# sigma0-dev/polymath

Hardware: AMD Instinct MI355X
Metric: prove_constraints_per_sec (higher is better)
Workload: dtype u32; 1 GPU; 2^20-100-constraint synthetic R1CS (random A*B=C gates), bls12_381, n=2^21, transcript=merlin; msm_pairs_per_proof=29359963, parallelism=one GPU

## Files before the change

polymath_amd/api.py:

```python
import ctypes as ct
import os

import numpy as np

HERE = os.path.dirname(os.path.abspath(__file__))
LIB_PATH = os.environ.get("POLYMATH_HIP_LIB") or os.path.join(HERE, "libpolymath_hip.so")

PM_BLS12_381, PM_BN254 = 0, 1
CURVE_IDS = {"bls12_381": PM_BLS12_381, "bn254": PM_BN254}
FQ_LIMBS64 = {PM_BLS12_381: 6, PM_BN254: 4}

STATUS = {0: "PM_OK", 1: "PM_ERR_INVALID_ARG", 2: "PM_ERR_LEN_MISMATCH", 3: "PM_ERR_DOMAIN_TOO_LARGE",
          4: "PM_ERR_REMAINDER_NONZERO", 5: "PM_ERR_DEGREE_BOUND", 6: "PM_ERR_HIP", 7: "PM_ERR_NO_DEVICE",
          8: "PM_ERR_STATE", 9: "PM_ERR_COMM"}
(X_POWERS, X_POWERS_Y_ALPHA, X_POWERS_Y_GAMMA, X_POWERS_Y_GAMMA_Z, X_POWERS_ZH_BY_Y_ALPHA,
 UJ_WJ_LCS_BY_Y_ALPHA) = range(6)
G1_OK, G1_BAD_FLAGS, G1_COORD_GE_P, G1_NOT_ON_CURVE, G1_NOT_IN_SUBGROUP, G1_NONCANONICAL_INF, G1_INF_SIGN = range(7)
G1_BYTES = {PM_BLS12_381: 48, PM_BN254: 32}
PROOF_BYTES = {PM_BLS12_381: 176, PM_BN254: 128}
VERIFY_REJECTED, VERIFY_ACCEPTED, VERIFY_MALFORMED = range(3)
VERIFY_TIMING_SLOTS = {"decode": 0, "terms": 1, "tree": 2, "host_glue": 3, "host_pairing": 4, "device_total": 7}
TIMING_SLOTS = ["witness_map", "ntt", "poly", "msm_sort", "msm_accumulate", "msm_reduce", "msm_total", "phase"]

u64p = ct.POINTER(ct.c_uint64)
# ... 242 lines not shown


def layout_indices(n, shard_count, shard_rank, coefficients=True):
    L = load_library()
    out = np.zeros(n // shard_count, dtype=np.uint64)
    st = L.pm_layout_indices(n, shard_count, shard_rank, int(coefficients), _p(out))
    if st:
        raise PolymathError(st, "pm_layout_indices")
    return out


class Comm:

    def __init__(self, handle, keep=None):
        self.L, self.h, self._keep = load_library(), handle, keep

    @classmethod
    def local_group(cls, world, serialize=False):
        L = load_library()
        arr = (ct.c_void_p * world)()
        st = L.pm_comm_local_create(world, arr)
        if st:
            raise PolymathError(st, "pm_comm_local_create")
        if serialize:
            st = L.pm_comm_local_set_serialize(ct.c_void_p(arr[0]), 1)
            if st:
                raise PolymathError(st, "pm_comm_local_set_serialize")
        return [cls(ct.c_void_p(arr[r])) for r in range(world)]

    @staticmethod
    def rccl_unique_id():
        L = load_library()
        buf = ct.create_string_buffer(128)
        st = L.pm_comm_rccl_unique_id(buf)
        if st:
            raise PolymathError(st, "pm_comm_rccl_unique_id (librccl not loadable?)")
        return buf.raw

    @classmethod
    def rccl(cls, unique_id, rank, world, device):
        L = load_library()
        h = ct.c_void_p()
        st = L.pm_comm_rccl_create(ct.c_char_p(unique_id), rank, world, device, ct.byref(h))
        if st:
            raise PolymathError(st, "pm_comm_rccl_create")
        return cls(h)

    @property
    def rank(self):
        return self.L.pm_comm_rank(self.h)

    @property
    def world(self):
        return self.L.pm_comm_world(self.h)

    def busy_ms(self, reset=True):
        return float(self.L.pm_comm_busy_ms(self.h, int(reset)))

    @property
    def kind(self):
        return self.L.pm_comm_kind(self.h).decode()

    @property
    def failed(self):
        return bool(self.L.pm_comm_failed(self.h))

    def last_error(self):
        return self.L.pm_comm_last_error(self.h).decode()

    def set_timeout_ms(self, ms):
        st = self.L.pm_comm_set_timeout_ms(self.h, int(ms))
        if st:
            raise PolymathError(st, "pm_comm_set_timeout_ms")

    def abort(self, why="aborted by the host"):
        self.L.pm_comm_abort(self.h, why.encode())

    def all_gather(self, arr):
        arr = np.ascontiguousarray(arr)
        out = np.zeros((self.world,) + arr.shape, dtype=arr.dtype)
        st = self.L.pm_comm_all_gather(self.h, arr.ctypes.data_as(ct.c_void_p), out.ctypes.data_as(ct.c_void_p), arr.nbytes)
        if st:
            raise PolymathError(st, self.L.pm_comm_last_error(self.h).decode())
        return out

    def all_to_all_device(self, d_send, d_recv, bytes_per_peer, stream=None):
        st = self.L.pm_comm_all_to_all(self.h, ct.c_void_p(d_send), ct.c_void_p(d_recv), bytes_per_peer, ct.c_void_p(stream or 0))
        if st:
            raise PolymathError(st, self.L.pm_comm_last_error(self.h).decode())

    def all_gather_device(self, d_send, d_recv, nbytes, stream=None):
        st = self.L.pm_comm_all_gather_device(self.h, ct.c_void_p(d_send), ct.c_void_p(d_recv), nbytes, ct.c_void_p(stream or 0))
        if st:
            raise PolymathError(st, self.L.pm_comm_last_error(self.h).decode())

    def close(self):
        if getattr(self, "h", None):
            self.L.pm_comm_destroy(self.h)
            self.h = None


class Context:

    def __init__(self, device=0):
        self.L = load_library()
        h = ct.c_void_p()
        st = self.L.pm_ctx_create(device, ct.byref(h))
        if st:
            raise PolymathError(st, "pm_ctx_create(device=%d)" % device)
        self.h = h
        self.device = device

    def close(self):
        if getattr(self, "h", None):
            self.L.pm_ctx_destroy(self.h)
            self.h = None

    def __del__(self):
        try:
            self.close()
        except Exception:
            pass

    def check(self, st):
        if st:
            raise PolymathError(st, self.L.pm_last_error(self.h).decode())

    def set_comm(self, comm):
        self.comm = comm
        self.check(self.L.pm_ctx_set_comm(self.h, comm.h if comm is not None else None))

    def set_option(self, name, value):
        key = OPTIONS[name] if isinstance(name, str) else int(name)
        if key == OPTIONS["tables"] and isinstance(value, str):
            value = TABLES_MODES[value]
        self.check(self.L.pm_ctx_set_option(self.h, key, int(value)))

    def get_option(self, name):
        key = OPTIONS[name] if isinstance(name, str) else int(name)
        v = ct.c_longlong(0)
        self.check(self.L.pm_ctx_get_option(self.h, key, ct.byref(v)))
        return int(v.value)

    def selftest_field(self, products_per_field=4096, seed=1):
        bad = (ct.c_uint64 * 4)()
        self.check(self.L.pm_selftest_field(self.h, products_per_field, seed, bad))
        return dict(zip(("bls12_381_fr", "bn254_fr", "bls12_381_fq", "bn254_fq"), (int(v) for v in bad)))

    def timings(self):
        arr = (ct.c_double * len(TIMING_SLOTS))()
        self.L.pm_last_timings(self.h, arr, len(TIMING_SLOTS))
        return dict(zip(TIMING_SLOTS, list(arr)))

    def ntt(self, curve, data, log_n, inverse=False):
        data = _c(data).copy()
        self.check(self.L.pm_ntt(self.h, CURVE_IDS[curve], _p(data), log_n, int(inverse)))
        return data

    def ntt_device(self, curve, dptr, log_n, inverse=False):
        self.check(self.L.pm_ntt_device(self.h, CURVE_IDS[curve], ct.c_void_p(dptr), log_n, int(inverse)))

    def msm(self, curve, bases, scalars):
        cid = CURVE_IDS[curve]
        bases, scalars = _c(bases), _c(scalars)
        out = np.zeros(2 * FQ_LIMBS64[cid], dtype=np.uint64)
        inf = ct.c_int(0)
        self.check(self.L.pm_msm_g1(self.h, cid, bases.ctypes.data_as(ct.c_void_p), max(bases.strides[0], 16 * FQ_LIMBS64[cid]) if bases.ndim > 1 else 16 * FQ_LIMBS64[cid],
                                    _p(scalars), scalars.shape[0], _p(out), ct.byref(inf)))
        return out, inf.value

    def g1_sum(self, curve, pts, infs=None):
        return g1_sum(curve, pts, infs)


class Bases:

    def __init__(self, ctx, curve, handle):
        self.ctx, self.curve, self.cid, self.h = ctx, curve, CURVE_IDS[curve], handle

    @classmethod
    def upload(cls, ctx, curve, bases):
        bases = _c(bases)
        h = ct.c_void_p()
        ctx.check(ctx.L.pm_bases_upload(ctx.h, CURVE_IDS[curve], bases.ctypes.data_as(ct.c_void_p), max(bases.strides[0], 16 * FQ_LIMBS64[CURVE_IDS[curve]]),
                                        bases.shape[0], ct.byref(h)))
        return cls(ctx, curve, h)

    @classmethod
    def multiples(cls, ctx, curve, length):
        h = ct.c_void_p()
        ctx.check(ctx.L.pm_bases_generate_multiples(ctx.h, CURVE_IDS[curve], length, ct.byref(h)))
        return cls(ctx, curve, h)

    def precompute(self):
        self.ctx.check(self.ctx.L.pm_bases_precompute(self.ctx.h, self.h))
        return self

    def __len__(self):
        return int(self.ctx.L.pm_bases_len(self.h))

    def download(self, offset=0, length=None):
        if length is None:
            length = len(self) - offset
        out = np.zeros((length, 2 * FQ_LIMBS64[self.cid]), dtype=np.uint64)
        self.ctx.check(self.ctx.L.pm_bases_download(self.ctx.h, self.h, offset, length, _p(out)))
        return out

    def msm(self, scalars, offset=0, length=None, device_ptr=None):
        out = np.zeros(2 * FQ_LIMBS64[self.cid], dtype=np.uint64)
        inf = ct.c_int(0)
        if device_ptr is not None:
            st = self.ctx.L.pm_msm_g1_resident(self.ctx.h, self.h, offset, ct.c_void_p(device_ptr), 1, length, _p(out), ct.byref(inf))
        else:
            scalars = _c(scalars)
            length = scalars.shape[0] if length is None else length
            st = self.ctx.L.pm_msm_g1_resident(self.ctx.h, self.h, offset, scalars.ctypes.data_as(ct.c_void_p), 0, length,
                                               _p(out), ct.byref(inf))
        self.ctx.check(st)
        return out, inf.value

    def free(self):
        if self.h:
            self.ctx.L.pm_bases_free(self.h)
            self.h = None

    def __del__(self):
        try:
            self.free()
        except Exception:
            pass


class CsrArrays:

    def __init__(self, rowptr, col, val):
        self.rowptr = np.ascontiguousarray(rowptr, dtype=np.uint64)
        self.col = np.ascontiguousarray(col if len(col) else [0], dtype=np.uint32)
        self.val = _c(val) if len(val) else np.zeros((1, 4), dtype=np.uint64)
        self.struct = PmCsr(len(self.rowptr) - 1, _p(self.rowptr), self.col.ctypes.data_as(u32p), _p(self.val))


class ProvingKey:

    def __init__(self, ctx, curve, handle, csrs):
        self.ctx, self.curve, self.cid, self.h, self._csrs = ctx, curve, CURVE_IDS[curve], handle, csrs
        n, m0, sigma = ct.c_uint64(), ct.c_uint64(), ct.c_uint64()
        omega = np.zeros(4, dtype=np.uint64)
        lens = np.zeros(6, dtype=np.uint64)
        ctx.check(ctx.L.pm_pk_info(self.h, ct.byref(n), ct.byref(m0), ct.byref(sigma), _p(omega), _p(lens)))
        self.n, self.m0, self.sigma, self.omega_limbs = n.value, m0.value, sigma.value, omega
        self.base_lens = [int(v) for v in lens]
        self.nq = FQ_LIMBS64[self.cid]

    @classmethod
    def generate(cls, ctx, curve, m0, mw, nr, a, b, c, x_trapdoor, z_trapdoor, shard_rank=0, shard_count=1, layout="pairs"):
        h = ct.c_void_p()
        ctx.check(ctx.L.pm_pk_generate_sharded(ctx.h, CURVE_IDS[curve], m0, mw, nr, ct.byref(a.struct), ct.byref(b.struct),
                                               ct.byref(c.struct), _p(_c(x_trapdoor)), _p(_c(z_trapdoor)), shard_rank, shard_count,
                                               LAYOUTS[layout], ct.byref(h)))
        pk = cls(ctx, curve, h, (a, b, c))
        pk.shard_rank, pk.shard_count, pk.layout = shard_rank, shard_count, LAYOUTS[layout]
        return pk

    @classmethod
    def load(cls, ctx, curve, n, m0, mw, nr, sigma, a, b, c, base_arrays, shard_rank=0, shard_count=1, layout="pairs"):
        arrs = [_c(x) for x in base_arrays]
        BA = (PmBaseArray * 6)()
        for k, x in enumerate(arrs):
            BA[k] = PmBaseArray(x.ctypes.data_as(ct.c_void_p), x.shape[0], x.strides[0])
        h = ct.c_void_p()
        ctx.check(ctx.L.pm_pk_load_sharded(ctx.h, CURVE_IDS[curve], n, m0, mw, nr, sigma, ct.byref(a.struct), ct.byref(b.struct),
                                           ct.byref(c.struct), BA, shard_rank, shard_count, LAYOUTS[layout], ct.byref(h)))
        pk = cls(ctx, curve, h, (a, b, c))
        pk.shard_rank, pk.shard_count, pk.layout = shard_rank, shard_count, LAYOUTS[layout]
        return pk

    @classmethod
    def load_bytes(cls, ctx, curve, data, validate=True, shard_rank=0, shard_count=1, layout="pairs"):
        keep, addr, nbytes = _byte_view(data)
        h = ct.c_void_p()
        ctx.check(ctx.L.pm_pk_load_bytes(ctx.h, CURVE_IDS[curve], ct.c_void_p(addr), nbytes, int(bool(validate)), shard_rank, shard_count,
                                         LAYOUTS[layout], ct.byref(h)))
        del keep
        pk = cls(ctx, curve, h, None)
        pk.shard_rank, pk.shard_count, pk.layout = shard_rank, shard_count, LAYOUTS[layout]
        return pk

    def view(self, ctx):
        v = ProvingKey.__new__(ProvingKey)
        v.__dict__.update(self.__dict__)
        v.ctx, v._view = ctx, True
        return v

    def msm_plan(self, which):
        pairs, win, bits, tb = ct.c_uint64(), ct.c_uint(), ct.c_uint(), ct.c_int()
        self.ctx.check(self.ctx.L.pm_pk_msm_plan(self.h, which, ct.byref(pairs), ct.byref(win), ct.byref(bits), ct.byref(tb)))
        return pairs.value, win.value, bits.value, bool(tb.value)

    def msm_pieces(self, which):
        n = ct.c_size_t(0)
        self.ctx.check(self.ctx.L.pm_pk_msm_pieces(self.h, which, None, None, 0, ct.byref(n)))
        lo, cnt = np.zeros(n.value, dtype=np.uint64), np.zeros(n.value, dtype=np.uint64)
        self.ctx.check(self.ctx.L.pm_pk_msm_pieces(self.h, which, _p(lo), _p(cnt), n.value, ct.byref(n)))
        return [(int(a), int(b)) for a, b in zip(lo, cnt)]

    def msm_windows(self, which):
# ... 92 lines not shown
```

polymath_amd/csrc/api.hip:

```cpp
#include <algorithm>
#include <atomic>
#include <cstdlib>
#include <cstring>
#include <exception>
#include <memory>
#include <new>
#include <thread>

#include "internal.h"
#include "comm.h"
#include "fq28.cuh"
#include "../host/hashes.hpp"

using namespace pm;

extern "C" void pm_host_keccak_f1600(uint64_t state[25]) { pmhost::keccak_f1600(state); }

int pm::host_threads_env() {
    static const int env_threads = [] { const char *e = getenv("PM_HOST_THREADS"); return e ? std::max(1, atoi(e)) : 0; }();
    return env_threads;
}

template <class F>
static void parallel_chunks(uint64_t count, F body) {
// ... 4 lines not shown
    if (env_threads) T = (unsigned)env_threads;
    if (T == 1) { body((uint64_t)0, count, 0u); return; }
    std::vector<std::thread> th;
    std::vector<std::exception_ptr> errs(T);
    auto guarded_body = [&](uint64_t lo, uint64_t hi, unsigned t) {
        try { body(lo, hi, t); } catch (...) { errs[t] = std::current_exception(); }
    };
    for (unsigned t = 1; t < T; ++t) {
        try {
            th.emplace_back([=, &guarded_body] { guarded_body(count * t / T, count * (t + 1) / T, t); });
        } catch (const std::system_error &) {
            guarded_body(count * t / T, count * (t + 1) / T, t);
        }
    }
    guarded_body((uint64_t)0, count / T, 0u);
    for (auto &x : th) x.join();
    for (auto &e : errs)
        if (e) std::rethrow_exception(e);
}

template <class C>
static void repack_bases(const void *src, size_t stride, size_t len, Affine<C> *dst) {
    const size_t PT = sizeof(Affine<C>);
    const uint8_t *s = (const uint8_t *)src;
    for (size_t i = 0; i < len; ++i) {
        memcpy(&dst[i], s + i * stride, PT);
        if (stride > PT && s[i * stride + PT] != 0) dst[i] = Affine<C>::infinity();
    }
}

#define PM_DISPATCH(curve, CALL_BLS, CALL_BN) \
    ((curve) == PM_BLS12_381 ? (CALL_BLS) : (curve) == PM_BN254 ? (CALL_BN) : (int)PM_ERR_INVALID_ARG)

static int set_device(pm_ctx *ctx) {
    PM_HIP(ctx, hipSetDevice(ctx->device));
    return PM_OK;
}

extern "C" int pm_device_count(void) {
    int n = 0;
    if (hipGetDeviceCount(&n) != hipSuccess) return 0;
    return n;
}

struct OptionSpec { const char *env; long long def, lo, hi; };
static const OptionSpec OPTION_SPECS[PM_NUM_OPTIONS] = {
     {"PM_MSM_OVERLAP", 1, 0, 1},
     {"PM_NTT_OVERLAP", 1, 0, 1},
     {"PM_TABLES", PM_TABLES_AUTO, PM_TABLES_OFF, PM_TABLES_NO_WIDE},
     {"PM_MSM_MAX_PIECE_LOG", 27, 4, 27},
     {"PM_MAX_SEG_LOG", 0, 0, 40},
     {"PM_INFLIGHT_CONTEXTS", 1, 1, 64},
     {"PM_MSM_SEG", 0, 0, 1 << 20},
     {"PM_TABLE_C", 0, 0, 24},
     {"PM_WIRE_CHUNK_LOG", 20, 4, 24},
};
static void options_defaults(pm_options *o) {
    for (int k = 0; k < PM_NUM_OPTIONS; ++k) {
        long long v = OPTION_SPECS[k].def;
        if (const char *e = getenv(OPTION_SPECS[k].env)) {
            if (k == PM_OPT_TABLES) v = e[0] == 'w' ? PM_TABLES_WIDE : e[0] == '0' ? PM_TABLES_OFF : PM_TABLES_AUTO;
            else v = atoll(e);
            if (v < OPTION_SPECS[k].lo || v > OPTION_SPECS[k].hi) v = OPTION_SPECS[k].def;
        }
        o->v[k] = v;
    }
    if (o->v[PM_OPT_TABLES] == PM_TABLES_AUTO) {
        const char *e = getenv("PM_WIDE");
        if (e && e[0] == '0') o->v[PM_OPT_TABLES] = PM_TABLES_NO_WIDE;
    }
}

extern "C" int pm_ctx_set_option(pm_ctx *ctx, int option, long long value) {
    if (!ctx || option < 0 || option >= PM_NUM_OPTIONS) return PM_ERR_INVALID_ARG;
    if (value < OPTION_SPECS[option].lo || value > OPTION_SPECS[option].hi) return PM_ERR_INVALID_ARG;
    ctx->opt.v[option] = value;
    if (ctx->aux) ctx->aux->opt.v[option] = value;
    return PM_OK;
}
extern "C" int pm_ctx_get_option(const pm_ctx *ctx, int option, long long *value) {
    if (!ctx || !value || option < 0 || option >= PM_NUM_OPTIONS) return PM_ERR_INVALID_ARG;
    *value = ctx->opt.v[option];
    return PM_OK;
}

extern "C" int pm_ctx_create(int device, pm_ctx **out) {
    if (!out) return PM_ERR_INVALID_ARG;
    *out = nullptr;
    int n = 0;
    if (hipGetDeviceCount(&n) != hipSuccess || n <= 0) return PM_ERR_NO_DEVICE;
    if (device < 0 || device >= n) return PM_ERR_INVALID_ARG;
    pm_ctx *ctx = new (std::nothrow) pm_ctx();
    if (!ctx) return PM_ERR_INVALID_ARG;
    ctx->device = device;
    options_defaults(&ctx->opt);
    ctx->pk = nullptr;
    ctx->phase = 0;
    ctx->aux = nullptr;
    ctx->comm = nullptr;
    ctx->tw_clock = 0;
    ctx->shard_roots_n = 0; ctx->shard_roots_N = 0; ctx->shard_roots_curve = -1;
    ctx->ntt_lds_attr[0] = ctx->ntt_lds_attr[1] = false;
    ctx->h_pinned = nullptr;
    ctx->msm_async = 0;
    ctx->keep_timings = false;
    ctx->lazy_timings = false;
    timing_reset(ctx);
    if (hipSetDevice(device) != hipSuccess || hipStreamCreateWithFlags(&ctx->stream, hipStreamNonBlocking) != hipSuccess) {
        delete ctx;
        return PM_ERR_HIP;
    }
    if (hipEventCreateWithFlags(&ctx->ev_sc_a, hipEventDisableTiming) != hipSuccess) {
        (void)hipStreamDestroy(ctx->stream);
        delete ctx;
        return PM_ERR_HIP;
    }
    *out = ctx;
    return PM_OK;
}

extern "C" void pm_ctx_destroy(pm_ctx *ctx) {
    if (!ctx) return;
    if (ctx->aux) pm_ctx_destroy(ctx->aux);
    (void)hipSetDevice(ctx->device);
    (void)hipStreamSynchronize(ctx->stream);
    timing_flush(ctx);
    MsmWorkspace &m = ctx->msm;
    for (DevBuf *b : {&m.set.sorted, &m.set.counts, &m.set.bucket_off, &m.set.task_off, &m.set.tasks, &m.set.partials, &m.set.task_cnt}) b->release();
    for (DevBuf *b : {&m.digits, &m.cursor, &m.wsum,
                      &m.region, &m.sub, &m.digits2, &m.len_bins, &m.block_cnt, &m.hot, &ctx->scratch, &ctx->flags, &ctx->xw, &ctx->ue, &ctx->we, &ctx->u, &ctx->w,
                      &ctx->wit_u, &ctx->u2, &ctx->sc_a, &ctx->sc_c, &ctx->quotient, &ctx->ztail, &ctx->ra, &ctx->sh_a, &ctx->sh_b, &ctx->sh_c, &ctx->halo,
                      &ctx->shard_roots, &ctx->ntt_tmp})
        b->release();
    for (auto &b : ctx->lvl) b.release();
    for (auto &b : ctx->fb_table) b.release();
    for (auto &t : ctx->tw) { t.fwd.release(); t.inv.release(); t.fwd_int.release(); t.inv_int.release(); }
    if (ctx->h_pinned) (void)hipHostFree(ctx->h_pinned);
    for (auto &t : ctx->pending_timers) { (void)hipEventDestroy(t.a); (void)hipEventDestroy(t.b); }
    for (hipEvent_t e : ctx->event_pool) (void)hipEventDestroy(e);
    (void)hipEventDestroy(ctx->ev_sc_a);
    (void)hipStreamDestroy(ctx->stream);
    delete ctx;
}

extern "C" const char *pm_last_error(const pm_ctx *ctx) { return ctx ? ctx->err.c_str() : "null context"; }

extern "C" int pm_last_timings(pm_ctx *ctx, double *ms_out, int n_slots) {
    if (!ctx || !ms_out) return PM_ERR_INVALID_ARG;
    if (!ctx->pending_timers.empty()) {
        if (hipSetDevice(ctx->device) != hipSuccess) return PM_ERR_HIP;
        timing_flush_now(ctx);
    }
    for (int i = 0; i < n_slots; ++i) ms_out[i] = i < T_NUM_SLOTS ? ctx->timing_ms[i] : 0.0;
    return PM_OK;
}

template <class C>
static int ntt_host(pm_ctx *ctx, uint64_t *data, unsigned log_n, int inverse) {
    typedef Fp<typename C::FrP> Fr;
    if (log_n > (unsigned)C::TWO_ADICITY) return PM_ERR_DOMAIN_TOO_LARGE;
    size_t bytes = sizeof(Fr) << log_n;
    PM_HIP(ctx, ctx->scratch.reserve(bytes));
    PM_HIP(ctx, hipMemcpyAsync(ctx->scratch.p, data, bytes, hipMemcpyHostToDevice, ctx->stream));
    timing_reset(ctx);
    PM_TRY(ntt_run<C>(ctx, ctx->scratch.as<Fr>(), log_n, inverse != 0));
    PM_HIP(ctx, hipMemcpyAsync(data, ctx->scratch.p, bytes, hipMemcpyDeviceToHost, ctx->stream));
    PM_HIP(ctx, hipStreamSynchronize(ctx->stream));
    timing_flush(ctx);
    return PM_OK;
}

extern "C" int pm_ntt(pm_ctx *ctx, int curve, uint64_t *data, unsigned log_n, int inverse) {
    if (!ctx || !data) return PM_ERR_INVALID_ARG;
    PM_TRY(set_device(ctx));
    return PM_DISPATCH(curve, ntt_host<BlsCurve>(ctx, data, log_n, inverse), ntt_host<BnCurve>(ctx, data, log_n, inverse));
}

template <class C>
static int ntt_dev(pm_ctx *ctx, uint64_t *d, unsigned log_n, int inverse) {
    timing_reset(ctx);
    PM_TRY(ntt_run<C>(ctx, (Fp<typename C::FrP> *)d, log_n, inverse != 0));
    PM_HIP(ctx, hipStreamSynchronize(ctx->stream));
    timing_flush(ctx);
    return PM_OK;
}

extern "C" int pm_ntt_device(pm_ctx *ctx, int curve, uint64_t *d_data, unsigned log_n, int inverse) {
    if (!ctx || !d_data) return PM_ERR_INVALID_ARG;
    PM_TRY(set_device(ctx));
    return PM_DISPATCH(curve, ntt_dev<BlsCurve>(ctx, d_data, log_n, inverse), ntt_dev<BnCurve>(ctx, d_data, log_n, inverse));
}

struct BasesDeleter {
    void operator()(pm_bases *b) const {
        if (!b) return;
        (void)hipSetDevice(b->device);
        if (b->d_points) (void)hipFree(b->d_points);
        if (b->d_inf) (void)hipFree(b->d_inf);
        if (b->d_table) (void)hipFree(b->d_table);
        delete b;
    }
};
typedef std::unique_ptr<pm_bases, BasesDeleter> BasesPtr;

template <class C>
static int bases_upload_impl(pm_ctx *ctx, const void *bases, size_t stride, size_t len, pm_bases **out) {
    if (stride < sizeof(Affine<C>)) return PM_ERR_INVALID_ARG;
    BasesPtr b(new pm_bases{C::ID, ctx->device, len, nullptr});
    if (len) {
        std::vector<Affine<C>> packed(len);
        repack_bases<C>(bases, stride, len, packed.data());
        PM_HIP(ctx, hipMalloc(&b->d_points, len * sizeof(Affine<C>)));
        PM_HIP(ctx, hipMemcpy(b->d_points, packed.data(), len * sizeof(Affine<C>), hipMemcpyHostToDevice));
        PM_TRY(bases_convert<C>(ctx, (Affine<C> *)b->d_points, len, true));
        PM_HIP(ctx, hipStreamSynchronize(ctx->stream));
    }
    *out = b.release();
    return PM_OK;
}

extern "C" int pm_bases_upload(pm_ctx *ctx, int curve, const void *bases, size_t base_stride, size_t len, pm_bases **out) {
    if (!ctx || !out || (len && !bases)) return PM_ERR_INVALID_ARG;
    PM_TRY(set_device(ctx));
    return PM_DISPATCH(curve, bases_upload_impl<BlsCurve>(ctx, bases, base_stride, len, out),
                       bases_upload_impl<BnCurve>(ctx, bases, base_stride, len, out));
}

template <class C>
static int bases_multiples_impl(pm_ctx *ctx, size_t len, pm_bases **out) {
    BasesPtr b(new pm_bases{C::ID, ctx->device, len, nullptr});
    if (len) {
        PM_HIP(ctx, hipMalloc(&b->d_points, len * sizeof(Affine<C>)));
        PM_TRY(bases_generate_multiples<C>(ctx, len, (Affine<C> *)b->d_points));
    }
    *out = b.release();
    return PM_OK;
}

extern "C" int pm_bases_generate_multiples(pm_ctx *ctx, int curve, size_t len, pm_bases **out) {
    if (!ctx || !out) return PM_ERR_INVALID_ARG;
    PM_TRY(set_device(ctx));
    return PM_DISPATCH(curve, bases_multiples_impl<BlsCurve>(ctx, len, out), bases_multiples_impl<BnCurve>(ctx, len, out));
}

template <class C>
static int download_points(pm_ctx *ctx, const void *d_src, size_t len, uint64_t *out_xy) {
    if (!len) return PM_OK;
    PM_HIP(ctx, ctx->scratch.reserve(len * sizeof(Affine<C>)));
    PM_HIP(ctx, hipMemcpyAsync(ctx->scratch.p, d_src, len * sizeof(Affine<C>), hipMemcpyDeviceToDevice, ctx->stream));
    PM_TRY(bases_convert<C>(ctx, ctx->scratch.as<Affine<C>>(), len, false));
    PM_HIP(ctx, hipMemcpyAsync(out_xy, ctx->scratch.p, len * sizeof(Affine<C>), hipMemcpyDeviceToHost, ctx->stream));
    PM_HIP(ctx, hipStreamSynchronize(ctx->stream));
    return PM_OK;
}

extern "C" int pm_bases_download(pm_ctx *ctx, const pm_bases *b, size_t offset, size_t len, uint64_t *out_xy) {
    if (!ctx || !b || !out_xy || offset + len > b->len) return PM_ERR_INVALID_ARG;
    PM_TRY(set_device(ctx));
    size_t pt = b->curve == PM_BLS12_381 ? sizeof(Affine<BlsCurve>) : sizeof(Affine<BnCurve>);
    const void *src = (const uint8_t *)b->d_points + offset * pt;
    return PM_DISPATCH(b->curve, download_points<BlsCurve>(ctx, src, len, out_xy), download_points<BnCurve>(ctx, src, len, out_xy));
}

template <class C>
static int bases_precompute_impl(pm_ctx *ctx, pm_bases *b) {
    if (b->tables.c || !b->len) return PM_OK;
    MsmTables tb = tables_plan(b->len, 1, b->len, (unsigned)C::FrP::BITS, (unsigned)ctx->opt.v[PM_OPT_TABLE_WINDOW_BITS]);
    if (!tb.c) return PM_OK;
    void *d_table = nullptr, *d_flags = nullptr;
    int st = PM_OK;
    if (hipMalloc(&d_table, b->len * tb.nwin * sizeof(TablePoint<C>)) != hipSuccess || hipMalloc(&d_flags, b->len) != hipSuccess) {
        ctx->err = "pm_bases_precompute: out of device memory for the window tables";
        st = PM_ERR_HIP;
    }
    if (st == PM_OK) st = infinity_flags<C>(ctx, (const Affine<C> *)b->d_points, b->len, (unsigned char *)d_flags);
    if (st == PM_OK) st = tables_build<C>(ctx, (const Affine<C> *)b->d_points, (TablePoint<C> *)d_table, b->len, tb);
    if (st != PM_OK) {
        if (d_table) (void)hipFree(d_table);
        if (d_flags) (void)hipFree(d_flags);
        return st;
    }
    b->d_table = d_table;
    b->d_inf = d_flags;
    tb.inf = (const unsigned char *)d_flags;
    tb.table = d_table;
    b->tables = tb;
    return PM_OK;
}

extern "C" int pm_bases_precompute(pm_ctx *ctx, pm_bases *b) {
    if (!ctx || !b) return PM_ERR_INVALID_ARG;
    PM_TRY(set_device(ctx));
    return PM_DISPATCH(b->curve, bases_precompute_impl<BlsCurve>(ctx, b), bases_precompute_impl<BnCurve>(ctx, b));
}

extern "C" size_t pm_bases_len(const pm_bases *b) { return b ? b->len : 0; }

extern "C" void pm_bases_free(pm_bases *b) { BasesDeleter()(b); }

template <class C>
static int msm_resident_impl(pm_ctx *ctx, const pm_bases *bases, size_t off, const uint64_t *scalars, int on_device,
                             size_t len, uint64_t *out_xy, int *out_inf) {
    typedef Fp<typename C::FrP> Fr;
    const Fr *d_sc = (const Fr *)scalars;
    if (!on_device && len) {
        PM_HIP(ctx, ctx->scratch.reserve(len * sizeof(Fr)));
// ... 819 lines not shown
```

polymath_amd/csrc/internal.h:

```cpp
#pragma once
#include <hip/hip_runtime.h>
#include <stdint.h>
#include <stdlib.h>

#include <chrono>
#include <condition_variable>
#include <cstdio>
#include <functional>
#include <mutex>
#include <string>
#include <thread>
#include <vector>

#include "../../include/polymath_hip.h"
#include "../host/layout.hpp"
#include "ec.cuh"

namespace pm {

struct pm_error_sink {
    std::string msg;
};

#define PM_HIP(ctx, expr)                                                                        \
    do {                                                                                         \
        hipError_t _e = (expr);                                                                  \
        if (_e != hipSuccess) {                                                                  \
            (ctx)->err = std::string(#expr) + ": " + hipGetErrorString(_e) + " @" + __FILE__ + ":" + \
                         std::to_string(__LINE__);                                               \
            return PM_ERR_HIP;                                                                   \
        }                                                                                        \
    } while (0)

#define PM_TRY(expr)                  \
    do {                              \
        int _s = (expr);              \
        if (_s != PM_OK) return _s;   \
    } while (0)

struct DevBuf {
    void *p = nullptr;
    size_t bytes = 0;
    hipError_t reserve(size_t need) {
        if (need <= bytes) return hipSuccess;
        if (p) {
            hipError_t e = hipFree(p);
            if (e != hipSuccess) return e;
            p = nullptr;
            bytes = 0;
        }
        size_t want = need + need / 8;
        hipError_t e = hipMalloc(&p, want);
        if (e != hipSuccess) {
            e = hipMalloc(&p, need);
            want = need;
        }
        if (e == hipSuccess) bytes = want;
        return e;
    }
    void release() {
        if (p) (void)hipFree(p);
        p = nullptr;
        bytes = 0;
    }
    template <class T>
    T *as() const { return (T *)p; }
};

enum TimingSlot {
    T_WITNESS_MAP = 0,
    T_NTT = 1,
    T_POLY = 2,
    T_MSM_SORT = 3,
    T_MSM_ACCUMULATE = 4,
    T_MSM_REDUCE = 5,
    T_MSM_TOTAL = 6,
    T_PHASE = 7,
    T_NUM_SLOTS = 8
};

struct MsmSet {
    DevBuf sorted, counts, bucket_off, task_off, tasks, partials, task_cnt;
};
struct MsmWorkspace {
    MsmSet set;
    DevBuf digits, cursor, wsum, region, sub, digits2, len_bins, block_cnt, hot;
};

struct MsmTables {
    unsigned c = 0, nwin = 0;
    unsigned off[33] = {0};
    unsigned char width[32] = {0};
    size_t stride = 0;
    size_t base_index = 0;
    const unsigned char *inf = nullptr;
    const void *table = nullptr;
    bool wide = false;
};

struct TwiddleCache {
    int curve = -1;
    unsigned log_n = 0;
    unsigned long long stamp = 0;
    DevBuf fwd, inv;
    DevBuf fwd_int, inv_int;
};

}

struct pm_bases {
    int curve;
    int device;
    size_t len;
    void *d_points;
    void *d_inf;
    void *d_table;
    pm::MsmTables tables;
};

struct pm_pk {
    int curve, device;
    uint64_t n, m0, mw, nr, sigma;
    unsigned log_n;
    uint64_t omega[4];
    int shard_rank, shard_count;
    uint64_t *d_rowptr[3];
    uint32_t *d_col[3];
    uint64_t *d_val[3];
    uint64_t nnz[3];
    void *d_bases;
    uint64_t base_len[PM_NUM_BASE_VECS];
    uint64_t seg_off[PM_NUM_BASE_VECS];
    uint64_t total_points;
    uint64_t res_lo[3], res_hi[3], res_dev_off[3];
    uint64_t msm_lo[3], msm_len[3];
    int layout;
    std::vector<pmlayout::Piece> pieces[3];
    uint64_t res_cnt[3];
    std::vector<pmlayout::Segment> segs;
    uint64_t max_seg;
    uint64_t max_piece = (uint64_t)1 << 27;
    struct SegRef { uint64_t a, b; uint32_t rank, idx; };
    std::vector<SegRef> all_segs;
    size_t seg_slots;
    void *d_segs;
    void *d_all_segs = nullptr;
    pm::MsmTables tables[3];
    void *d_tab[3], *d_tab_inf[3];
};

struct pm_worker {
    std::thread th;
    std::mutex mu;
    std::condition_variable cv;
    std::function<void()> job;
    bool has_job = false, done = true, stop = false;
    bool submit(std::function<void()> fn) {
        std::unique_lock<std::mutex> lk(mu);
        if (!th.joinable()) {
            try {
                th = std::thread([this] {
                    std::unique_lock<std::mutex> l(mu);
                    for (;;) {
                        cv.wait(l, [this] { return has_job || stop; });
                        if (stop) return;
                        std::function<void()> f = std::move(job);
                        has_job = false;
                        l.unlock();
                        f();
                        l.lock();
                        done = true;
                        cv.notify_all();
                    }
                });
            } catch (const std::system_error &) {
                return false;
            }
        }
        job = std::move(fn);
        has_job = true;
        done = false;
        cv.notify_all();
        return true;
    }
    void wait() {
        std::unique_lock<std::mutex> lk(mu);
        cv.wait(lk, [this] { return done; });
    }
    ~pm_worker() {
        {
            std::unique_lock<std::mutex> lk(mu);
            cv.wait(lk, [this] { return done; });
            stop = true;
            cv.notify_all();
        }
        if (th.joinable()) th.join();
    }
};

struct pm_options {
    long long v[PM_NUM_OPTIONS];
};

struct PendingTimer {
    int slot;
    hipEvent_t a, b;
};

struct pm_ctx {
    int device;
    pm_options opt;
    std::vector<PendingTimer> pending_timers;
    std::vector<hipEvent_t> event_pool;
    hipStream_t stream;
    std::string err;
    double timing_ms[pm::T_NUM_SLOTS];
    hipEvent_t ev_sc_a;
    pm::MsmWorkspace msm;
    pm::TwiddleCache tw[8];
    unsigned long long tw_clock;
    pm::DevBuf scratch, flags, ntt_tmp;
    void *h_pinned;
    int msm_async;
    bool ntt_lds_attr[2];
    pm_comm *comm;
    pm_worker worker;
    pm_ctx *aux;
    pm::DevBuf fb_table[2];
    const pm_pk *pk;
    int phase;
    std::vector<uint8_t> seg_all;
    uint64_t x1_host[4];
    uint64_t ra_host[8];
    bool keep_timings;
    bool lazy_timings;
    pm::DevBuf xw, ue, we, u, w, wit_u, u2, sc_a, sc_c, quotient, ztail, lvl[6], ra;
    pm::DevBuf sh_a, sh_b, sh_c, halo, shard_roots;
    uint64_t shard_roots_n;
    uint32_t shard_roots_N;
    int shard_roots_curve;
};

namespace pm {

struct HostProfile {
    bool on;
    const char *phase;
    int rank;
    std::chrono::steady_clock::time_point t0, last;
    std::vector<std::pair<const char *, double>> parts;
    HostProfile(const char *ph, int r) : phase(ph), rank(r) {
        static const bool enabled = [] { const char *e = getenv("PM_PROFILE_HOST"); return e && e[0] == '1'; }();
        on = enabled;
        if (on) t0 = last = std::chrono::steady_clock::now();
    }
    void mark(const char *label) {
        if (!on) return;
        const auto now = std::chrono::steady_clock::now();
        parts.emplace_back(label, std::chrono::duration<double, std::milli>(now - last).count());
        last = now;
    }
    ~HostProfile() {
        if (!on) return;
        std::string line = std::string("[pm host rank ") + std::to_string(rank) + "] " + phase + ":";
        char buf[96];
        for (auto &p : parts) { snprintf(buf, sizeof buf, " %s=%.3f", p.first, p.second); line += buf; }
        snprintf(buf, sizeof buf, " | total=%.3f ms\n", std::chrono::duration<double, std::milli>(last - t0).count());
        line += buf;
        fputs(line.c_str(), stderr);
    }
};

int host_threads_env();

template <class C>
int ntt_run(pm_ctx *ctx, Fp<typename C::FrP> *d_data, unsigned log_n, bool inverse);
template <class C>
int twiddles_get(pm_ctx *ctx, unsigned log_n, bool inv_dir, const Fp<typename C::FrP> **out);

template <class C>
int msm_run(pm_ctx *ctx, const Affine<C> *d_bases, const Fp<typename C::FrP> *d_scalars, size_t len,
            Affine<C> *h_out, int *h_inf, const MsmTables *tables = nullptr);

template <class C>
int msm_begin(pm_ctx *ctx, const Affine<C> *d_bases, const Fp<typename C::FrP> *d_scalars, size_t len, const MsmTables *tables);
template <class C>
int msm_end(pm_ctx *ctx, Affine<C> *h_out, int *h_inf);
template <class C>
int msm_resident_begin(pm_ctx *ctx, const pm_pk *pk, int which, const Fp<typename C::FrP> *d_scalars, uint64_t lo = 0, uint64_t count = 0);
template <class C>
int msm_resident_end(pm_ctx *ctx, uint64_t *out_xy, int *out_inf);

template <class C>
int reduce_two_level(pm_ctx *ctx, size_t NB, XYZZ<C> **out, unsigned nsets = 1, size_t bucket0 = 0);

constexpr unsigned SORT_REGION_BITS = 15, SORT_MAX_REGIONS = 1024;

struct WideSets {
    size_t wide_b, narrow_b;
    unsigned n_wide, n_narrow;
    size_t total() const { return n_wide * wide_b + n_narrow * narrow_b; }
};
inline WideSets wide_sets(unsigned nwin, unsigned c) {
    WideSets s;
    s.wide_b = (size_t)1 << (c - 1);
    const bool halve = 256 % nwin != 0 && (s.wide_b >> 1) >= ((size_t)1 << SORT_REGION_BITS);
    s.narrow_b = halve ? s.wide_b >> 1 : s.wide_b;
    s.n_wide = halve ? 256 % nwin : nwin;
    s.n_narrow = nwin - s.n_wide;
    return s;
}

inline size_t msm_max_piece(const pm_ctx *ctx) {
    const long long lg = ctx->opt.v[PM_OPT_MSM_MAX_PIECE_LOG];
    return (size_t)1 << (lg < 4 ? 4 : lg > 27 ? 27 : lg);
}

void msm_plan_query(size_t len, unsigned scalar_bits, unsigned *nwin, unsigned *c);
MsmTables tables_plan(size_t total_pairs, unsigned n_msm, size_t resident_points, unsigned scalar_bits, unsigned force_c = 0);
MsmTables wide_plan(size_t piece, unsigned force_c = 0);
template <class C>
struct TablePoint;
template <class C>
int tables_build(pm_ctx *ctx, const Affine<C> *d_points, TablePoint<C> *d_table, size_t count, const MsmTables &t);
template <class C>
int infinity_flags(pm_ctx *ctx, const Affine<C> *d_points, size_t count, unsigned char *d_flags);

template <class C>
int bases_generate_multiples(pm_ctx *ctx, size_t len, Affine<C> *d_out);

template <class C>
int fixed_base_batch(pm_ctx *ctx, const Fp<typename C::FrP> *d_scalars, size_t len, Affine<C> *d_out);

template <class C>
int bases_convert(pm_ctx *ctx, Affine<C> *d_points, size_t len, bool to_internal);

template <class C>
int g1_decode_device(pm_ctx *ctx, const uint8_t *d_in, size_t count, bool validate, Affine<C> *d_out, uint8_t *d_status,
                     unsigned long long *d_first_bad, uint64_t base_index);
template <class C>
int g1_encode_device(pm_ctx *ctx, const Affine<C> *d_pts, size_t count, uint8_t *d_out);
const char *g1_status_text(int curve, int status);
struct WireLayout {
    size_t vk_len = 0;
    uint64_t n = 0, vk_m0 = 0, sigma = 0, omega[4] = {0, 0, 0, 0};
    uint64_t m0 = 0, mw = 0, nr = 0;
    std::vector<uint64_t> rowptr[3], val[3];
    std::vector<uint32_t> col[3];
    uint64_t vec_off[PM_NUM_BASE_VECS] = {0}, vec_len[PM_NUM_BASE_VECS] = {0};
};
template <class C>
int pk_wire_parse(const uint8_t *data, size_t len, WireLayout &out, std::string &err);

template <class C>
int lcs_scalars(pm_ctx *ctx, const pm_pk *pk, const Fp<typename C::FrP> &x, const Fp<typename C::FrP> &omega, const Fp<typename C::FrP> &kscale,
                const Fp<typename C::FrP> &y_gamma, const Fp<typename C::FrP> &y_to_minus_alpha, DevBuf &lagrange, DevBuf &work,
                Fp<typename C::FrP> *d_lcs);

template <class C>
int powers_fill(pm_ctx *ctx, Fp<typename C::FrP> *d_out, size_t count, const Fp<typename C::FrP> &scale,
                const Fp<typename C::FrP> &x);

template <class C>
int msm_resident(pm_ctx *ctx, const pm_pk *pk, int which, const Fp<typename C::FrP> *d_scalars, uint64_t *out_xy, int *out_inf);

template <class C>
int prove_phase1_impl(pm_ctx *ctx, const pm_pk *pk, const uint64_t *x, const uint64_t *w, const uint64_t *r_a,
                      uint64_t *a_xy, int *a_inf, uint64_t *c_xy, int *c_inf, bool assignment_on_device);
template <class C>
int prove_phase2_impl(pm_ctx *ctx, const uint64_t *x1, uint64_t *u_at_x1);
template <class C>
int prove_phase3_impl(pm_ctx *ctx, const uint64_t *x1, const uint64_t *x2, const uint64_t *a_at_x1,
                      const uint64_t *c_at_x1, uint64_t *d_xy, int *d_inf);

template <class C>
int prove_phase1_sharded(pm_ctx *ctx, const pm_pk *pk, const uint64_t *x, const uint64_t *w, const uint64_t *r_a, uint64_t *a_xy, int *a_inf,
                         uint64_t *c_xy, int *c_inf, bool assignment_on_device);
template <class C>
int prove_phase2_sharded(pm_ctx *ctx, const uint64_t *x1, uint64_t *u_at_x1);
template <class C>
int prove_phase3_sharded(pm_ctx *ctx, const uint64_t *x1, const uint64_t *x2, const uint64_t *a_at_x1, const uint64_t *c_at_x1, uint64_t *d_xy,
                         int *d_inf);

inline pm_ctx *ctx_aux(pm_ctx *ctx) {
    if (!ctx->aux && pm_ctx_create(ctx->device, &ctx->aux) != PM_OK) ctx->aux = nullptr;
    if (ctx->aux) ctx->aux->opt = ctx->opt;
    return ctx->aux;
}

constexpr size_t PINNED_SLOTS_BYTES = 4096, PINNED_STAGE_BYTES = 32768;
constexpr size_t PINNED_MSM_SUM = 0,
                 PINNED_MSM_POINT = 1024,
                 PINNED_MSM_INF = 2048,
                 PINNED_REMAINDER = 3072,
                 PINNED_FLAGS = PINNED_SLOTS_BYTES;
template <class T>
inline T *pinned_slot(pm_ctx *ctx, size_t offset) { return (T *)((uint8_t *)ctx->h_pinned + offset); }
inline void *ctx_pinned(pm_ctx *ctx) {
    if (!ctx->h_pinned && hipHostMalloc(&ctx->h_pinned, PINNED_SLOTS_BYTES + PINNED_STAGE_BYTES, hipHostMallocDefault) != hipSuccess) ctx->h_pinned = nullptr;
    return ctx->h_pinned;
}

inline void timing_reset(pm_ctx *ctx) {
    for (int i = 0; i < T_NUM_SLOTS; ++i) ctx->timing_ms[i] = 0;
    for (auto &t : ctx->pending_timers) { ctx->event_pool.push_back(t.a); ctx->event_pool.push_back(t.b); }
    ctx->pending_timers.clear();
}

struct StageTimer {
    pm_ctx *ctx;
    int slot;
    hipEvent_t a, b;
    bool ok;
    static bool take(pm_ctx *c, hipEvent_t *e) {
        if (!c->event_pool.empty()) { *e = c->event_pool.back(); c->event_pool.pop_back(); return true; }
        return hipEventCreate(e) == hipSuccess;
    }
    hipStream_t stream;
    StageTimer(pm_ctx *c, int s, hipStream_t on = nullptr) : ctx(c), slot(s), ok(false), stream(on ? on : c->stream) {
        if (!take(c, &a)) return;
        if (!take(c, &b)) { c->event_pool.push_back(a); return; }
        ok = hipEventRecord(a, stream) == hipSuccess;
        if (!ok) { c->event_pool.push_back(a); c->event_pool.push_back(b); }
    }
    void stop() {
        if (!ok) return;
        ok = false;
        (void)hipEventRecord(b, stream);
        ctx->pending_timers.push_back(PendingTimer{slot, a, b});
// ... 37 lines not shown
```

polymath_amd/csrc/msm.hip:

```cpp
#include <cstdlib>
#include <cstring>

#include "internal.h"
#include "fq28.cuh"

namespace pm {

constexpr uint32_t DIGIT_NONE = 0xFFFFFFFFu;

struct MsmPlan {
    unsigned c, nwin, nbuckets;
    unsigned seg;
    size_t len;
    unsigned chunk, nchunks;
    size_t max_tasks;
};

static MsmPlan make_plan(size_t len, unsigned scalar_bits, unsigned task_len = 0) {
    MsmPlan p;
    p.len = len;
    double best = 1e300;
    unsigned bc = 4;
    for (unsigned c = 4; c <= 16; ++c) {
        unsigned w = (scalar_bits + 1 + c - 1) / c;
        double cost = (double)w * ((double)len + 6.0 * (double)(1u << (c - 1)));
        if (cost < best) { best = cost; bc = c; }
    }
    p.c = bc;
    p.nwin = (scalar_bits + 1 + bc - 1) / bc;
    p.nbuckets = 1u << (bc - 1);
    size_t avg = len / p.nbuckets + 1;
    size_t seg = 2 * avg;
    if (seg < 64) seg = 64;
    p.seg = (unsigned)seg;
    p.chunk = 1u << 15;
    if (len < p.chunk) p.chunk = (unsigned)(len ? len : 1);
    p.nchunks = (unsigned)((len + p.chunk - 1) / p.chunk);
    if (task_len) p.seg = task_len;
    p.max_tasks = (size_t)p.nwin * p.nbuckets + ((size_t)p.nwin * len) / p.seg + 1;
    return p;
}

void msm_plan_query(size_t len, unsigned scalar_bits, unsigned *nwin, unsigned *c) {
    MsmPlan p = make_plan(len ? len : 1, scalar_bits);
    *nwin = p.nwin;
    *c = p.c;
}

template <class C>
__global__ void k_digits(const Fp<typename C::FrP> *scalars, const Affine<C> *bases, uint32_t *digits, size_t len,
                         unsigned c, unsigned nwin) {
    typedef typename C::FrP P;
    size_t i = (size_t)blockIdx.x * blockDim.x + threadIdx.x;
    if (i >= len) return;
    Fp<P> k = from_mont<P>(scalars[i]);
    const uint32_t *bx = (const uint32_t *)&bases[i];
    uint32_t any = 0;
#pragma unroll
    for (int t = 0; t < 2 * C::FqP::N; ++t) any |= bx[t];
    const bool skip = (any == 0);
    uint32_t carry = 0;
    const uint32_t half = 1u << (c - 1), full = 1u << c, mask = full - 1;
    for (unsigned w = 0; w < nwin; ++w) {
        unsigned lo = w * c, limb = lo >> 5, off = lo & 31;
        uint32_t v = 0;
        if (limb < (unsigned)P::N) {
            uint64_t two = k.l[limb];
            if (limb + 1 < (unsigned)P::N) two |= (uint64_t)k.l[limb + 1] << 32;
            v = (uint32_t)(two >> off) & mask;
        }
        uint32_t d = v + carry;
        uint32_t out;
        if (d > half) {
            uint32_t m = full - d;
            out = m ? (((m - 1) << 1) | 1u) : DIGIT_NONE;
            carry = 1;
        } else {
            out = d ? ((d - 1) << 1) : DIGIT_NONE;
            carry = 0;
        }
        digits[(size_t)w * len + i] = skip ? DIGIT_NONE : out;
    }
}

__global__ __launch_bounds__(1024) void k_hist(const uint32_t *digits, uint32_t *counts, size_t len, unsigned chunk,
                                               unsigned nbuckets) {
    extern __shared__ __attribute__((aligned(16))) unsigned char smem_raw[];
    uint32_t *h = (uint32_t *)smem_raw;
    const unsigned w = blockIdx.y;
    for (unsigned b = threadIdx.x; b < nbuckets; b += blockDim.x) h[b] = 0;
    __syncthreads();
    size_t lo = (size_t)blockIdx.x * chunk, hi = lo + chunk;
    if (hi > len) hi = len;
    const uint32_t *d = digits + (size_t)w * len;
    for (size_t i = lo + threadIdx.x; i < hi; i += blockDim.x) {
        uint32_t v = d[i];
        if (v != DIGIT_NONE) atomicAdd(&h[v >> 1], 1u);
    }
    __syncthreads();
    uint32_t *cw = counts + (size_t)w * nbuckets;
    for (unsigned b = threadIdx.x; b < nbuckets; b += blockDim.x) {
        uint32_t v = h[b];
        if (v) atomicAdd(&cw[b], v);
    }
}

constexpr unsigned SCAN_PER = 16, SCAN_TILE = 256 * SCAN_PER;

__global__ __launch_bounds__(256) void k_scan_tiles(const uint32_t *counts, uint32_t *bucket_off, uint32_t *task_off,
                                                    uint32_t *tile_tot, size_t G, unsigned seg) {
    __shared__ uint32_t s_a[256], s_b[256];
    const unsigned tid = threadIdx.x;
    const size_t base = (size_t)blockIdx.x * SCAN_TILE + (size_t)tid * SCAN_PER;
    uint32_t c[SCAN_PER], nt[SCAN_PER];
    uint32_t sa = 0, sb = 0;
#pragma unroll
    for (unsigned k = 0; k < SCAN_PER; ++k) {
        c[k] = base + k < G ? counts[base + k] : 0u;
        nt[k] = (c[k] + seg - 1) / seg;
        sa += c[k];
        sb += nt[k];
    }
    s_a[tid] = sa;
    s_b[tid] = sb;
    __syncthreads();
    for (unsigned off = 1; off < 256; off <<= 1) {
        uint32_t va = 0, vb = 0;
        if (tid >= off) { va = s_a[tid - off]; vb = s_b[tid - off]; }
        __syncthreads();
        s_a[tid] += va;
        s_b[tid] += vb;
        __syncthreads();
    }
    uint32_t ra = s_a[tid] - sa, rb = s_b[tid] - sb;
#pragma unroll
    for (unsigned k = 0; k < SCAN_PER; ++k) {
        if (base + k < G) { bucket_off[base + k] = ra; task_off[base + k] = rb; }
        ra += c[k];
        rb += nt[k];
    }
    if (tid == 255) { tile_tot[2 * blockIdx.x] = s_a[255]; tile_tot[2 * blockIdx.x + 1] = s_b[255]; }
}

__global__ __launch_bounds__(1024) void k_scan_totals(uint32_t *tile_tot, unsigned ntiles, uint32_t *bucket_off,
                                                      uint32_t *task_off, size_t G) {
    __shared__ uint32_t s_a[1024], s_b[1024];
    const unsigned tid = threadIdx.x;
    uint32_t carry_a = 0, carry_b = 0;
    for (unsigned base = 0; base < ntiles; base += 1024) {
        unsigned i = base + tid;
        uint32_t a = i < ntiles ? tile_tot[2 * i] : 0u, b = i < ntiles ? tile_tot[2 * i + 1] : 0u;
        s_a[tid] = a;
        s_b[tid] = b;
        __syncthreads();
        for (unsigned off = 1; off < 1024; off <<= 1) {
            uint32_t va = 0, vb = 0;
            if (tid >= off) { va = s_a[tid - off]; vb = s_b[tid - off]; }
            __syncthreads();
            s_a[tid] += va;
            s_b[tid] += vb;
            __syncthreads();
        }
        if (i < ntiles) { tile_tot[2 * i] = carry_a + s_a[tid] - a; tile_tot[2 * i + 1] = carry_b + s_b[tid] - b; }
        carry_a += s_a[1023];
        carry_b += s_b[1023];
        __syncthreads();
    }
    if (tid == 0) { bucket_off[G] = carry_a; task_off[G] = carry_b; }
}

__global__ __launch_bounds__(256) void k_scan_add(uint32_t *bucket_off, uint32_t *task_off, const uint32_t *tile_tot, size_t G) {
    const size_t base = (size_t)blockIdx.x * SCAN_TILE + (size_t)threadIdx.x * SCAN_PER;
    const uint32_t oa = tile_tot[2 * blockIdx.x], ob = tile_tot[2 * blockIdx.x + 1];
#pragma unroll
    for (unsigned k = 0; k < SCAN_PER; ++k)
        if (base + k < G) { bucket_off[base + k] += oa; task_off[base + k] += ob; }
}

__global__ __launch_bounds__(1024) void k_scatter(const uint32_t *digits, const uint32_t *bucket_off, uint32_t *cursor,
                                                  uint32_t *sorted, size_t len, unsigned chunk, unsigned nbuckets) {
    extern __shared__ __attribute__((aligned(16))) unsigned char smem_raw[];
    uint32_t *h = (uint32_t *)smem_raw;
    const unsigned w = blockIdx.y;
    for (unsigned b = threadIdx.x; b < nbuckets; b += blockDim.x) h[b] = 0;
    __syncthreads();
    size_t lo = (size_t)blockIdx.x * chunk, hi = lo + chunk;
    if (hi > len) hi = len;
    const uint32_t *d = digits + (size_t)w * len;
    for (size_t i = lo + threadIdx.x; i < hi; i += blockDim.x) {
        uint32_t v = d[i];
        if (v != DIGIT_NONE) atomicAdd(&h[v >> 1], 1u);
    }
    __syncthreads();
    const size_t gbase = (size_t)w * nbuckets;
    for (unsigned b = threadIdx.x; b < nbuckets; b += blockDim.x) {
        uint32_t v = h[b];
        if (v) h[b] = bucket_off[gbase + b] + atomicAdd(&cursor[gbase + b], v);
    }
    __syncthreads();
    for (size_t i = lo + threadIdx.x; i < hi; i += blockDim.x) {
        uint32_t v = d[i];
        if (v != DIGIT_NONE) {
            uint32_t pos = atomicAdd(&h[v >> 1], 1u);
            sorted[pos] = ((uint32_t)i << 1) | (v & 1u);
        }
    }
}

constexpr unsigned TASK_MAX_BINS = 8192;

template <bool SCATTER>
__global__ __launch_bounds__(1024) void k_task_bins(const uint32_t *counts, const uint32_t *bucket_off, const uint32_t *task_off, size_t G,
                                                    unsigned seg, unsigned lshift, unsigned nbins, uint32_t *len_cnt, const uint32_t *len_off,
                                                    uint32_t *len_cursor, uint4 *tasks) {
    extern __shared__ __attribute__((aligned(16))) unsigned char smem_raw[];
    uint32_t *h = (uint32_t *)smem_raw;
    for (unsigned b = threadIdx.x; b < nbins; b += blockDim.x) h[b] = 0;
    __syncthreads();
    const size_t g = (size_t)blockIdx.x * blockDim.x + threadIdx.x;
    uint32_t t0 = 0, n = 0, rank_full = 0, rank_last = 0, cnt = 0;
    unsigned bin = 0;
    if (g < G) {
        t0 = task_off[g];
        n = task_off[g + 1] - t0;
        if (n) {
            cnt = counts[g];
            const uint32_t L = cnt - (n - 1) * seg;
            bin = (seg - L) >> lshift;
            if (n > 1) rank_full = atomicAdd(&h[0], n - 1);
            rank_last = atomicAdd(&h[bin], 1u);
        }
    }
    __syncthreads();
    if (!SCATTER) {
        for (unsigned b = threadIdx.x; b < nbins; b += blockDim.x) {
            const uint32_t v = h[b];
            if (v) atomicAdd(&len_cnt[b], v);
        }
    } else {
        for (unsigned b = threadIdx.x; b < nbins; b += blockDim.x) {
            const uint32_t v = h[b];
            if (v) h[b] = len_off[b] + atomicAdd(&len_cursor[b], v);
        }
        __syncthreads();
        if (n) {
            const uint32_t at = h[0] + rank_full, first = bucket_off[g];
            for (uint32_t k = 0; k + 1 < n; ++k)
                tasks[at + k] = make_uint4(t0 + k, first + k * seg, first + (k + 1) * seg, 0u);
            tasks[h[bin] + rank_last] = make_uint4(t0 + n - 1, first + (n - 1) * seg, first + cnt, 0u);
        }
    }
}

template <class C, bool TABLE>
__device__ __forceinline__ void accumulate_task(const uint32_t *sorted, const uint4 d, const void *points, XYZZ<C> *partials) {
    typedef typename C::FqRR RR;
    XYZZ28<C> acc;
    acc.X = acc.Y = acc.ZZ = acc.ZZZ = f28_zero<RR>();
    uint4 quad = make_uint4(0u, 0u, 0u, 0u);
    uint32_t quad_at = 0xffffffffu;
    for (uint32_t e = d.y; e < d.z; ++e) {
        if ((e & ~3u) != quad_at) {
            quad_at = e & ~3u;
            quad = *(const uint4 *)(sorted + quad_at);
        }
        const unsigned q = e & 3u;
        const uint32_t v = q == 0 ? quad.x : q == 1 ? quad.y : q == 2 ? quad.z : quad.w;
        const bool neg = (v & 1u) != 0;
        if (TABLE) {
            const TablePoint<C> tp = ((const TablePoint<C> *)points)[v >> 1];
            F28<RR> x2, y2;
#pragma unroll
            for (int i = 0; i < RR::N; ++i) { x2.l[i] = tp.x[i]; y2.l[i] = tp.y[i]; }
            if (!xyzz28_madd_limbs<C>(acc, x2, y2, neg)) acc = xyzz28_madd_exceptional<C>(acc, table_point_to_affine<C>(tp), neg);
        } else {
            const Affine<C> p = ((const Affine<C> *)points)[v >> 1];
            if (!xyzz28_madd<C>(acc, p, neg)) acc = xyzz28_madd_exceptional<C>(acc, p, neg);
        }
    }
    partials[d.x] = xyzz28_store<C>(acc);
}

template <class C, bool TABLE>
__global__ __launch_bounds__(128) void k_accumulate(const uint32_t *sorted, const uint32_t *task_off, const uint4 *tasks,
                                                    const void *points, XYZZ<C> *partials, size_t G, uint32_t *ticket) {
    const uint32_t total = task_off[G];
    const unsigned lane = threadIdx.x & 63u;
    for (;;) {
        uint32_t base = 0;
        if (lane == 0) base = atomicAdd(ticket, 64u);
        base = __builtin_amdgcn_readfirstlane(base);
        if (base >= total) break;
        const uint32_t i = base + lane;
        if (i < total) accumulate_task<C, TABLE>(sorted, tasks[i], points, partials);
    }
}

constexpr unsigned RED_K = 4;

template <class C>
__device__ __forceinline__ void lds_tree_sum(XYZZ28<C> *sh) {
    __syncthreads();
    for (unsigned off = blockDim.x >> 1; off > 0; off >>= 1) {
        if (threadIdx.x < off) {
            const XYZZ28<C> b = sh[threadIdx.x + off];
            xyzz28_add_into_full<C>(&sh[threadIdx.x], b);
        }
        __syncthreads();
    }
}

constexpr uint32_t FOLD_MIN = 8, FOLD_BLOCK_MIN = 1024;

__global__ void k_task_counts(const uint32_t *task_off, size_t G, uint32_t *task_cnt, uint32_t *hot_a, uint32_t *hot_b,
                              uint32_t *hot_counts , uint32_t cap) {
    size_t g = (size_t)blockIdx.x * blockDim.x + threadIdx.x;
    if (g >= G) return;
    const uint32_t n = task_off[g + 1] - task_off[g];
    task_cnt[g] = n;
    if (n > FOLD_BLOCK_MIN) {
        const uint32_t i = atomicAdd(&hot_counts[0], 1u);
        if (i < cap) hot_a[i] = (uint32_t)g;
    } else if (n > FOLD_MIN) {
        const uint32_t i = atomicAdd(&hot_counts[1], 1u);
        if (i < cap) hot_b[i] = (uint32_t)g;
    }
}

template <class C, unsigned LANES>
__global__ __launch_bounds__(256) __attribute__((amdgpu_waves_per_eu(2, 2))) void k_task_fold(XYZZ<C> *partials, const uint32_t *task_off, uint32_t *task_cnt,
                                                   const uint32_t *hot, const uint32_t *hot_count, uint32_t cap) {
    extern __shared__ __attribute__((aligned(16))) unsigned char smem_raw[];
    XYZZ28<C> *sh = (XYZZ28<C> *)smem_raw;
    typedef typename C::FqRR RR;
    uint32_t listed = *hot_count;
    if (listed > cap) listed = cap;
    constexpr unsigned GROUPS = 256 / LANES;
    const unsigned group = threadIdx.x / LANES, lane = threadIdx.x % LANES;
    for (uint32_t h0 = blockIdx.x * GROUPS; h0 < listed; h0 += gridDim.x * GROUPS) {
        const uint32_t h = h0 + group;
        XYZZ28<C> *acc = &sh[threadIdx.x];
        acc->X = acc->Y = acc->ZZ = acc->ZZZ = f28_zero<RR>();
        uint32_t first = 0, n = 0;
        if (h < listed) {
            first = task_off[hot[h]];
            n = task_off[hot[h] + 1] - first;
            for (uint32_t i = lane; i < n; i += LANES) xyzz28_add_into_full<C>(acc, xyzz28_load<C>(partials[first + i]));
        }
        __syncthreads();
        for (unsigned off = LANES >> 1; off > 0; off >>= 1) {
            if (lane < off) {
                const XYZZ28<C> b = sh[threadIdx.x + off];
                xyzz28_add_into_full<C>(&sh[threadIdx.x], b);
            }
            __syncthreads();
        }
        if (h < listed && lane == 0) {
            partials[first] = xyzz28_store<C>(sh[threadIdx.x]);
            task_cnt[hot[h]] = 1;
        }
        __syncthreads();
    }
}

template <class C>
__global__ __launch_bounds__(256) __attribute__((amdgpu_waves_per_eu(2, 2))) void k_bucket_reduce(const XYZZ<C> *partials, const uint32_t *task_off, const uint32_t *task_cnt, unsigned nbuckets,
                                                       unsigned lanes_per_window, unsigned bpw, XYZZ<C> *out) {
    extern __shared__ __attribute__((aligned(16))) unsigned char smem_raw[];
    XYZZ28<C> *sh = (XYZZ28<C> *)smem_raw;
    typedef typename C::FqRR RR;
    const unsigned w = blockIdx.x / bpw, bw = blockIdx.x % bpw;
    const unsigned j = bw * blockDim.x + threadIdx.x;
    XYZZ28<C> run;
    run.X = run.Y = run.ZZ = run.ZZZ = f28_zero<RR>();
    XYZZ28<C> *acc = &sh[threadIdx.x];
    *acc = run;
    if (j < lanes_per_window) {
        const size_t gbase = (size_t)w * nbuckets + (size_t)j * RED_K;
        for (int i = (int)RED_K - 1; i >= 0; --i) {
            if ((size_t)j * RED_K + i >= nbuckets) continue;
            for (uint32_t q = task_off[gbase + i], qe = q + task_cnt[gbase + i]; q < qe; ++q) xyzz28_add_full<C>(run, xyzz28_load<C>(partials[q]));
            xyzz28_add_into_full<C>(acc, run);
        }
        const uint32_t s = j * RED_K;
        if (s) {
            XYZZ28<C> m = run;
            for (int b = 30 - __clz((int)s); b >= 0; --b) {
                xyzz28_dbl<C>(m);
                if ((s >> b) & 1) xyzz28_add_full<C>(m, run);
            }
            xyzz28_add_into_full<C>(acc, m);
        }
    }
    lds_tree_sum<C>(sh);
    if (threadIdx.x == 0) out[blockIdx.x] = xyzz28_store<C>(sh[0]);
}

template <class C>
__global__ __launch_bounds__(64) __attribute__((amdgpu_waves_per_eu(2, 2))) void k_sum_parts(const XYZZ<C> *parts, unsigned count, XYZZ<C> *out) {
    __shared__ XYZZ28<C> sh[64];
    typedef typename C::FqRR RR;
    XYZZ28<C> *acc = &sh[threadIdx.x];
    acc->X = acc->Y = acc->ZZ = acc->ZZZ = f28_zero<RR>();
    for (unsigned i = threadIdx.x; i < count; i += 64) xyzz28_add_into_full<C>(acc, xyzz28_load<C>(parts[(size_t)blockIdx.x * count + i]));
    lds_tree_sum<C>(sh);
    if (threadIdx.x == 0) out[blockIdx.x] = xyzz28_store<C>(sh[0]);
}

constexpr unsigned LO_BITS = SORT_REGION_BITS;

__device__ __forceinline__ uint32_t block_inclusive_scan(uint32_t v, uint32_t *wt) {
    const unsigned lane = threadIdx.x & 63, wave = threadIdx.x >> 6;
#pragma unroll
    for (unsigned o = 1; o < 64; o <<= 1) {
        const uint32_t n = __shfl_up(v, o, 64);
        if (lane >= o) v += n;
    }
    if (lane == 63) wt[wave] = v;
    __syncthreads();
    if (wave == 0) {
        uint32_t w = lane < (blockDim.x >> 6) ? wt[lane] : 0u;
#pragma unroll
        for (unsigned o = 1; o < 16; o <<= 1) {
            const uint32_t n = __shfl_up(w, o, 64);
            if (lane >= o) w += n;
        }
        wt[lane] = w;
    }
    __syncthreads();
    if (wave) v += wt[wave - 1];
    return v;
}

template <class P>
__device__ __forceinline__ Fp<P> canon_scalar(const Fp<P> *scalars, const unsigned char *inf, size_t i) {
    Fp<P> k = from_mont<P>(scalars[i]);
    if (inf[i]) k = Fp<P>::zero();
    return k;
}

__host__ __device__ constexpr unsigned win_width(unsigned nwin, unsigned w) { return 256 / nwin + (w < 256 % nwin ? 1u : 0u); }
__host__ __device__ constexpr unsigned win_off(unsigned nwin, unsigned w) { return w * (256 / nwin) + (w < 256 % nwin ? w : 256 % nwin); }
__host__ __device__ constexpr uint32_t win_base(unsigned nwin, unsigned w, uint32_t wide_b, uint32_t narrow_b) {
    return w <= 256 % nwin ? w * wide_b : (256 % nwin) * wide_b + (w - 256 % nwin) * narrow_b;
}

template <class P>
__device__ __forceinline__ bool digit_at(const Fp<P> &k, unsigned lo, unsigned c, uint32_t &carry, uint32_t &bucket, uint32_t &neg) {
    const uint32_t half = 1u << (c - 1), full = 1u << c, mask = full - 1;
    const unsigned limb = lo >> 5, off = lo & 31;
    uint32_t v = 0;
    if (limb < (unsigned)P::N) {
        uint64_t two = k.l[limb];
        if (limb + 1 < (unsigned)P::N) two |= (uint64_t)k.l[limb + 1] << 32;
        v = (uint32_t)(two >> off) & mask;
    }
    const uint32_t d = v + carry;
    const bool over = d > half;
    const uint32_t m = over ? full - d : d;
    carry = over ? 1u : 0u;
    neg = carry;
    bucket = m - 1;
    return m != 0;
}

template <class P, unsigned NWIN>
__global__ __launch_bounds__(1024) void k_tbl_count(const Fp<P> *scalars, const unsigned char *inf, size_t len, unsigned regions,
                                                   uint32_t *block_cnt, uint32_t win_buckets, uint32_t narrow_buckets) {
    __shared__ uint32_t cnt[SORT_MAX_REGIONS];
    for (unsigned r = threadIdx.x; r < regions; r += blockDim.x) cnt[r] = 0;
    __syncthreads();
    const size_t i = (size_t)blockIdx.x * blockDim.x + threadIdx.x;
    if (i < len) {
        const Fp<P> k = canon_scalar<P>(scalars, inf, i);
        uint32_t carry = 0, b, neg;
#pragma unroll
        for (unsigned w = 0; w < NWIN; ++w)
            if (digit_at<P>(k, win_off(NWIN, w), win_width(NWIN, w), carry, b, neg)) atomicAdd(&cnt[(b + win_base(NWIN, w, win_buckets, narrow_buckets)) >> LO_BITS], 1u);
    }
    __syncthreads();
    for (unsigned r = threadIdx.x; r < regions; r += blockDim.x) block_cnt[(size_t)blockIdx.x * regions + r] = cnt[r];
}

struct BlockScanShape { unsigned G, span, rows, per; };
static BlockScanShape block_scan_shape(unsigned nblocks, unsigned regions) {
    BlockScanShape h;
    h.rows = 1024 / regions < 16 ? 1024 / regions : 16;
    if (h.rows < 1) h.rows = 1;
    h.G = (nblocks + 15) / 16 < 256 ? (nblocks + 15) / 16 : 256;
    if (h.G < 1) h.G = 1;
    h.span = (nblocks + h.G - 1) / h.G;
    h.per = (h.span + h.rows - 1) / h.rows;
    return h;
}
__device__ __forceinline__ void block_scan_range(unsigned g, unsigned j, BlockScanShape h, unsigned nblocks, unsigned &lo, unsigned &hi) {
    const unsigned end = (g + 1) * h.span < nblocks ? (g + 1) * h.span : nblocks;
    lo = g * h.span + j * h.per;
    hi = lo + h.per < end ? lo + h.per : end;
}
__global__ __launch_bounds__(1024) void k_block_sums(const uint32_t *block_cnt, unsigned nblocks, unsigned regions, BlockScanShape h, uint32_t *partial) {
    __shared__ uint32_t s[1024];
    const unsigned t = threadIdx.x, j = t / regions, r = t % regions;
    if (j < h.rows) {
        unsigned lo, hi;
        block_scan_range(blockIdx.x, j, h, nblocks, lo, hi);
        uint32_t sum = 0;
        for (unsigned b = lo; b < hi; ++b) sum += block_cnt[(size_t)b * regions + r];
        s[t] = sum;
    }
    __syncthreads();
    if (t < regions) {
        uint32_t tot = 0;
        for (unsigned jj = 0; jj < h.rows; ++jj) tot += s[jj * regions + t];
        partial[(size_t)blockIdx.x * regions + t] = tot;
    }
}
__global__ __launch_bounds__(1024) void k_block_offsets(uint32_t *block_cnt, unsigned nblocks, unsigned regions, BlockScanShape h, const uint32_t *partial,
                                                        uint32_t *region_count) {
    __shared__ uint32_t s[1024], base[1024];
    const unsigned t = threadIdx.x, j = t / regions, r = t % regions, g = blockIdx.x;
    if (j < h.rows) {
        uint32_t acc = 0;
        for (unsigned q = j; q < g; q += h.rows) acc += partial[(size_t)q * regions + r];
        s[t] = acc;
    }
    __syncthreads();
    if (t < regions) {
        uint32_t tot = 0;
        for (unsigned jj = 0; jj < h.rows; ++jj) tot += s[jj * regions + t];
        base[t] = tot;
    }
    __syncthreads();
    unsigned lo = 0, hi = 0;
    if (j < h.rows) {
        block_scan_range(g, j, h, nblocks, lo, hi);
        uint32_t sum = 0;
        for (unsigned b = lo; b < hi; ++b) sum += block_cnt[(size_t)b * regions + r];
        s[t] = sum;
    }
    __syncthreads();
    if (j < h.rows) {
        uint32_t run = base[r];
        for (unsigned jj = 0; jj < j; ++jj) run += s[jj * regions + r];
        for (unsigned b = lo; b < hi; ++b) {
            const uint32_t v = block_cnt[(size_t)b * regions + r];
            block_cnt[(size_t)b * regions + r] = run;
            run += v;
        }
    }
    if (g == gridDim.x - 1 && t < regions) {
        uint32_t tot = base[t];
        for (unsigned jj = 0; jj < h.rows; ++jj) tot += s[jj * regions + t];
        region_count[t] = tot;
    }
}

__global__ __launch_bounds__(1024) void k_region_offsets(const uint32_t *region_count, uint32_t *region_off, uint32_t *region_cursor,
                                                         unsigned regions) {
    __shared__ uint32_t s[1024];
    const unsigned t = threadIdx.x;
    uint32_t v = t < regions ? region_count[t] : 0u;
    s[t] = v;
    __syncthreads();
    for (unsigned off = 1; off < 1024; off <<= 1) {
        uint32_t a = t >= off ? s[t - off] : 0u;
        __syncthreads();
        s[t] += a;
        __syncthreads();
    }
    if (t < regions) { region_off[t] = s[t] - v; region_cursor[t] = 0; }
    if (t == 1023) region_off[regions] = s[1023];
}

template <class P, unsigned NWIN>
__global__ __launch_bounds__(1024) void k_tbl_partition(const Fp<P> *scalars, const unsigned char *inf, size_t len,
                                                       unsigned regions, const uint32_t *region_off, const uint32_t *block_off, size_t tbl_stride, size_t base_index, uint16_t *keys,
                                                       uint32_t *vals, uint32_t win_buckets, uint32_t narrow_buckets) {
    extern __shared__ __attribute__((aligned(16))) unsigned char smem_raw[];
    uint32_t *cnt = (uint32_t *)smem_raw, *delta = cnt + SORT_MAX_REGIONS;
    uint32_t *st_val = delta + 1024, *st_key = st_val + (size_t)blockDim.x * NWIN;
    __shared__ uint32_t tot, wt[64];
    const unsigned t = threadIdx.x, BD = blockDim.x;
    for (unsigned r = t; r < regions; r += BD) cnt[r] = 0;
    __syncthreads();
    const size_t i = (size_t)blockIdx.x * BD + t;
    uint32_t rank[NWIN];
    Fp<P> k = Fp<P>::zero();
    if (i < len) {
        k = canon_scalar<P>(scalars, inf, i);
        uint32_t carry = 0, b, neg;
#pragma unroll
        for (unsigned w = 0; w < NWIN; ++w)
            if (digit_at<P>(k, win_off(NWIN, w), win_width(NWIN, w), carry, b, neg)) rank[w] = atomicAdd(&cnt[(b + win_base(NWIN, w, win_buckets, narrow_buckets)) >> LO_BITS], 1u);
    }
    __syncthreads();
    {
        const uint32_t c = t < regions ? cnt[t] : 0u;
        const uint32_t incl = block_inclusive_scan(c, wt);
        if (t < regions) {
            const uint32_t ex = incl - c;
            cnt[t] = ex;
            delta[t] = region_off[t] + block_off[(size_t)blockIdx.x * regions + t] - ex;
        }
        if (t == BD - 1) tot = incl;
    }
    __syncthreads();
    if (i < len) {
        uint32_t carry = 0, b, neg;
#pragma unroll
        for (unsigned w = 0; w < NWIN; ++w)
            if (digit_at<P>(k, win_off(NWIN, w), win_width(NWIN, w), carry, b, neg)) {
                b += win_base(NWIN, w, win_buckets, narrow_buckets);
                const uint32_t rg = b >> LO_BITS, slot = cnt[rg] + rank[w];
                st_key[slot] = (rg << 16) | (b & ((1u << LO_BITS) - 1));
                st_val[slot] = (uint32_t)(((size_t)w * tbl_stride + base_index + i) << 1) | neg;
            }
    }
    __syncthreads();
    const uint32_t total = tot;
    for (uint32_t s = t; s < total; s += BD) {
        const uint32_t kv = st_key[s], pos = delta[kv >> 16] + s;
        keys[pos] = (uint16_t)kv;
        vals[pos] = st_val[s];
    }
}

enum { RS_HIST = 0, RS_MID = 1, RS_FINAL = 2 };
constexpr unsigned ST_MAX_BINS_HIST = 256;
constexpr unsigned RS_CHUNK_LOG = 15, RS_PER_LANE = (1u << RS_CHUNK_LOG) / 1024;

template <int MODE>
__global__ __launch_bounds__(1024) void k_region_pass(const uint16_t *keys, const uint32_t *vals, const uint32_t *seg_off,
                                                      unsigned nseg, unsigned bin_shift, unsigned nbins, unsigned chunk,
                                                      uint32_t *counts, const uint32_t *out_off, uint32_t *cursor,
                                                      uint32_t *sorted, uint16_t * , uint32_t * ) {
    static_assert(MODE == RS_HIST || MODE == RS_FINAL, "the middle level runs staged (k_region_pass_staged<RS_MID>)");
    extern __shared__ __attribute__((aligned(16))) unsigned char smem_raw[];
    uint32_t *h = (uint32_t *)smem_raw;
    const uint32_t total = seg_off[nseg];
    const uint32_t lo = blockIdx.x * chunk;
    if (lo >= total) return;
    uint32_t hi = lo + chunk;
    if (hi > total) hi = total;
    unsigned ra = 0, rb = nseg;
    while (rb - ra > 1) {
        unsigned mid = (ra + rb) >> 1;
        if (seg_off[mid] <= lo) ra = mid; else rb = mid;
    }
    for (unsigned r = ra; r < nseg; ++r) {
        const uint32_t s0 = seg_off[r] > lo ? seg_off[r] : lo;
        const uint32_t s1 = seg_off[r + 1] < hi ? seg_off[r + 1] : hi;
        if (s0 >= hi) break;
        if (s0 >= s1) continue;
        for (unsigned b = threadIdx.x; b < nbins; b += blockDim.x) h[b] = 0;
        __syncthreads();
        const size_t gbase = (size_t)r * nbins;
        if (MODE == RS_HIST) {
            for (uint32_t e = s0 + threadIdx.x; e < s1; e += blockDim.x) atomicAdd(&h[keys[e] >> bin_shift], 1u);
            __syncthreads();
            for (unsigned b = threadIdx.x; b < nbins; b += blockDim.x) {
                uint32_t v = h[b];
                if (v) atomicAdd(&counts[gbase + b], v);
            }
        } else {
            uint32_t rank[RS_PER_LANE];
            uint16_t key[RS_PER_LANE];
#pragma unroll
            for (unsigned q = 0; q < RS_PER_LANE; ++q) {
                const uint32_t e = s0 + q * blockDim.x + threadIdx.x;
                if (e < s1) {
                    key[q] = keys[e];
                    rank[q] = atomicAdd(&h[key[q] >> bin_shift], 1u);
                }
            }
            __syncthreads();
            for (unsigned b = threadIdx.x; b < nbins; b += blockDim.x) {
                uint32_t v = h[b];
                if (v) h[b] = out_off[gbase + b] + atomicAdd(&cursor[gbase + b], v);
            }
            __syncthreads();
#pragma unroll
            for (unsigned q = 0; q < RS_PER_LANE; ++q) {
                const uint32_t e = s0 + q * blockDim.x + threadIdx.x;
                if (e < s1) sorted[h[key[q] >> bin_shift] + rank[q]] = vals[e];
            }
        }
        __syncthreads();
    }
}

__global__ __launch_bounds__(1024) void k_hist_small(const uint16_t *keys, const uint32_t *seg_off, unsigned nseg, unsigned bin_shift,
                                                     unsigned nbins, unsigned chunk, uint32_t *counts) {
    __shared__ uint32_t h[16][ST_MAX_BINS_HIST];
    const uint32_t total = seg_off[nseg];
    const uint32_t lo = blockIdx.x * chunk;
    if (lo >= total) return;
    uint32_t hi = lo + chunk;
    if (hi > total) hi = total;
    unsigned ra = 0, rb = nseg;
    while (rb - ra > 1) {
        unsigned mid = (ra + rb) >> 1;
        if (seg_off[mid] <= lo) ra = mid; else rb = mid;
    }
    const unsigned wave = threadIdx.x >> 6;
    for (unsigned r = ra; r < nseg; ++r) {
        const uint32_t s0 = seg_off[r] > lo ? seg_off[r] : lo;
        const uint32_t s1 = seg_off[r + 1] < hi ? seg_off[r + 1] : hi;
        if (s0 >= hi) break;
        if (s0 >= s1) continue;
        for (unsigned b = threadIdx.x; b < 16 * ST_MAX_BINS_HIST; b += blockDim.x) (&h[0][0])[b] = 0;
        __syncthreads();
        const uint32_t b0 = (s0 + 7u) & ~7u, b1 = s1 & ~7u;
        if (b0 < b1) {
            for (uint32_t e = s0 + threadIdx.x; e < b0; e += blockDim.x) atomicAdd(&h[wave][keys[e] >> bin_shift], 1u);
            for (uint32_t e = b0 + threadIdx.x * 8u; e < b1; e += blockDim.x * 8u) {
                const uint4 v = *(const uint4 *)(keys + e);
                const uint32_t w4[4] = {v.x, v.y, v.z, v.w};
#pragma unroll
                for (int q = 0; q < 4; ++q) {
                    atomicAdd(&h[wave][(w4[q] & 0xffffu) >> bin_shift], 1u);
                    atomicAdd(&h[wave][(w4[q] >> 16) >> bin_shift], 1u);
                }
            }
            for (uint32_t e = b1 + threadIdx.x; e < s1; e += blockDim.x) atomicAdd(&h[wave][keys[e] >> bin_shift], 1u);
// ... 50 lines not shown
            uint32_t kw[ST_PER_LANE / 2], vw[ST_PER_LANE];
#pragma unroll
            for (unsigned g = 0; g < ST_PER_LANE / 8; ++g) {
                const uint4 kv = *(const uint4 *)(keys + e0 + 8 * g);
                kw[4 * g] = kv.x; kw[4 * g + 1] = kv.y; kw[4 * g + 2] = kv.z; kw[4 * g + 3] = kv.w;
            }
#pragma unroll
            for (unsigned g = 0; g < ST_PER_LANE / 4; ++g) {
                const uint4 va = *(const uint4 *)(vals + e0 + 4 * g);
                vw[4 * g] = va.x; vw[4 * g + 1] = va.y; vw[4 * g + 2] = va.z; vw[4 * g + 3] = va.w;
            }
#pragma unroll
            for (unsigned q = 0; q < ST_PER_LANE; ++q) {
                const uint32_t e = e0 + q;
                key[q] = (uint16_t)(kw[q >> 1] >> (16 * (q & 1)));
                val[q] = vw[q];
                if (e >= s0 && e < s1) {
                    vm |= 1u << q;
                    rank[q] = atomicAdd(&h[key[q] >> bin_shift], 1u);
                }
            }
        }
        __syncthreads();
        {
            const uint32_t c = t < nbins ? h[t] : 0u;
            const uint32_t incl = block_inclusive_scan(c, wt);
            if (t < nbins) {
                const uint32_t ex = incl - c;
                const size_t g = (size_t)r * nbins + t;
                const uint32_t gpos = c ? out_off[g] + atomicAdd(&cursor[g], c) : 0u;
                delta[t] = gpos - ex;
                h[t] = ex;
            }
        }
        __syncthreads();
#pragma unroll
        for (unsigned q = 0; q < ST_PER_LANE; ++q) {
            if ((vm >> q) & 1u) {
                const uint32_t slot = h[key[q] >> bin_shift] + rank[q];
                st_key[slot] = key[q];
                st_val[slot] = val[q];
            }
        }
        __syncthreads();
        for (uint32_t i = t; i < cnt; i += ST_THREADS) {
            const uint16_t k = st_key[i];
            const uint32_t pos = delta[k >> bin_shift] + i;
            if (MODE == RS_FINAL) {
                sorted[pos] = st_val[i];
            } else {
                keys_out[pos] = k & low_mask;
                vals_out[pos] = st_val[i];
            }
        }
        __syncthreads();
    }
}

__global__ __launch_bounds__(1024) void k_scan_small(const uint32_t *cnt, uint32_t *off, uint32_t *zero, unsigned n) {
    __shared__ uint32_t s[1024];
    __shared__ uint32_t carry;
    const unsigned t = threadIdx.x;
    if (t == 0) carry = 0;
    __syncthreads();
    for (unsigned base = 0; base < n; base += 1024) {
        const unsigned i = base + t;
        const uint32_t v = i < n ? cnt[i] : 0u;
        s[t] = v;
        __syncthreads();
        for (unsigned o = 1; o < 1024; o <<= 1) {
            uint32_t a = t >= o ? s[t - o] : 0u;
            __syncthreads();
            s[t] += a;
            __syncthreads();
        }
        if (i < n) { off[i] = carry + s[t] - v; zero[i] = 0; }
        __syncthreads();
        if (t == 1023) carry += s[1023];
        __syncthreads();
    }
    if (t == 0) off[n] = carry;
}

struct BucketPlan {
    bool tables, wide;
    unsigned nwin, c;
    size_t len, E;
    size_t NB1, NBn, NB;
    unsigned n_wide_sets, n_narrow_sets;
    uint32_t win_buckets, narrow_buckets;
    size_t seg, max_tasks;
    unsigned chunk, nchunks;
    unsigned lo_buckets, regions, pbd;
    size_t plds, keys_bytes;
    bool two_level;
    unsigned red_lanes, red_block, bpw;
    unsigned nsums;
    unsigned char width[64];
};

constexpr unsigned PARTITION_LANES = 512, PARTITION_WIDE_LANES = 1024, PARTITION_WIDE_FROM = 512;

static int bucket_plan(const MsmTables *tb, size_t len, unsigned scalar_bits, long long task_len, BucketPlan &p) {
    p = BucketPlan();
    p.len = len;
    p.tables = tb && tb->c;
    if (!p.tables) {
        const MsmPlan w = make_plan(len, scalar_bits, task_len > 0 ? (unsigned)task_len : 0u);
        p.nwin = w.nwin; p.c = w.c; p.seg = w.seg; p.max_tasks = w.max_tasks; p.chunk = w.chunk; p.nchunks = w.nchunks;
        p.NB1 = w.nbuckets;
        p.n_wide_sets = w.nwin;
        for (unsigned i = 0; i < w.nwin; ++i) p.width[i] = (unsigned char)w.c;
    } else {
        p.wide = tb->wide;
        p.nwin = tb->nwin; p.c = tb->c;
        if (p.nwin < 10 || p.nwin > 32) return PM_ERR_INVALID_ARG;
        for (unsigned w = 0; w < p.nwin; ++w)
            if (tb->off[w] != win_off(p.nwin, w) || tb->width[w] != win_width(p.nwin, w)) return PM_ERR_INVALID_ARG;
        p.NB1 = (size_t)1 << (p.c - 1);
        p.n_wide_sets = 1;
        if (p.wide) {
            const WideSets s = wide_sets(p.nwin, p.c);
            p.NBn = s.narrow_b; p.n_wide_sets = s.n_wide; p.n_narrow_sets = s.n_narrow;
            p.win_buckets = (uint32_t)p.NB1; p.narrow_buckets = (uint32_t)p.NBn;
            for (unsigned w = 0; w < p.nwin; ++w) p.width[w] = tb->width[w];
        }
    }
    p.NB = p.n_wide_sets * p.NB1 + p.n_narrow_sets * p.NBn;
    p.E = (size_t)p.nwin * len;
    p.nsums = p.n_wide_sets + p.n_narrow_sets;
    p.red_lanes = (unsigned)((p.NB1 + RED_K - 1) / RED_K);
    p.red_block = 64;
    while (p.red_block < p.red_lanes && p.red_block < 256) p.red_block <<= 1;
    p.bpw = (p.red_lanes + p.red_block - 1) / p.red_block;
    if (!p.tables) return PM_OK;

    p.lo_buckets = (unsigned)(p.NB < ((size_t)1 << LO_BITS) ? p.NB : ((size_t)1 << LO_BITS));
    p.regions = (unsigned)(p.NB / p.lo_buckets);
    if ((size_t)p.regions * p.lo_buckets != p.NB) return PM_ERR_INVALID_ARG;
    p.pbd = p.regions >= PARTITION_WIDE_FROM ? PARTITION_WIDE_LANES : p.nwin <= 16 ? PARTITION_LANES : 256;
    if (p.regions > p.pbd || p.regions > SORT_MAX_REGIONS) return PM_ERR_INVALID_ARG;
    p.plds = 2 * SORT_MAX_REGIONS * 4 + (size_t)p.pbd * p.nwin * 8;
    p.two_level = p.NB1 >= 4096;
    if (p.wide && !p.two_level) return PM_ERR_INVALID_ARG;
    p.seg = 2 * (p.E / p.NB + 1);
    if (p.seg < 64) p.seg = 64;
    if (task_len > 0) p.seg = (size_t)task_len;
    p.max_tasks = p.NB + p.E / p.seg + 1;
    p.keys_bytes = (p.E * 2 + 15) & ~(size_t)15;
    return PM_OK;
}


template <class C>
static int reserve_set(pm_ctx *ctx, MsmSet &S, const BucketPlan &p) {
    PM_HIP(ctx, S.sorted.reserve(p.E * 4 + 16));
    PM_HIP(ctx, S.counts.reserve(2 * p.NB * 4));
    PM_HIP(ctx, S.bucket_off.reserve((p.NB + 1) * 4));
    PM_HIP(ctx, S.task_off.reserve((p.NB + 1) * 4));
    PM_HIP(ctx, S.partials.reserve(p.max_tasks * sizeof(XYZZ<C>)));
    PM_HIP(ctx, S.task_cnt.reserve(p.NB * 4));
    PM_HIP(ctx, ctx->msm.cursor.reserve(((p.NB + SCAN_TILE - 1) / SCAN_TILE + 1) * 8));
    return PM_OK;
}

static int bucket_scan(pm_ctx *ctx, MsmSet &S, const BucketPlan &p) {
    uint32_t *tile_tot = ctx->msm.cursor.as<uint32_t>(), *bucket_off = S.bucket_off.as<uint32_t>(), *task_off = S.task_off.as<uint32_t>();
    const unsigned ntiles = (unsigned)((p.NB + SCAN_TILE - 1) / SCAN_TILE);
    hipLaunchKernelGGL(k_scan_tiles, dim3(ntiles), dim3(256), 0, ctx->stream, S.counts.as<uint32_t>(), bucket_off, task_off, tile_tot, p.NB,
                       (unsigned)p.seg);
    PM_HIP(ctx, hipGetLastError());
    hipLaunchKernelGGL(k_scan_totals, dim3(1), dim3(1024), 0, ctx->stream, tile_tot, ntiles, bucket_off, task_off, p.NB);
    PM_HIP(ctx, hipGetLastError());
    hipLaunchKernelGGL(k_scan_add, dim3(ntiles), dim3(256), 0, ctx->stream, bucket_off, task_off, tile_tot, p.NB);
    PM_HIP(ctx, hipGetLastError());
    return PM_OK;
}

template <class C>
static int fold_hot_buckets(pm_ctx *ctx, MsmSet &S, const BucketPlan &p) {
    MsmWorkspace &ws = ctx->msm;
    const size_t G = p.NB;
    size_t cap = p.max_tasks > G ? p.max_tasks - G + 1 : 1;
    cap = cap / FOLD_MIN + 1;
    PM_HIP(ctx, ws.hot.reserve((2 * cap + 2) * 4));
    uint32_t *hot_counts = ws.hot.as<uint32_t>(), *hot_a = hot_counts + 2, *hot_b = hot_a + cap;
    PM_HIP(ctx, hipMemsetAsync(hot_counts, 0, 8, ctx->stream));
    hipLaunchKernelGGL(k_task_counts, dim3((unsigned)((G + 255) / 256)), dim3(256), 0, ctx->stream, S.task_off.as<uint32_t>(), G,
                       S.task_cnt.as<uint32_t>(), hot_a, hot_b, hot_counts, (uint32_t)cap);
    PM_HIP(ctx, hipGetLastError());
    hipLaunchKernelGGL((k_task_fold<C, 256>), dim3(256), dim3(256), 256 * sizeof(XYZZ28<C>), ctx->stream, S.partials.as<XYZZ<C>>(),
                       S.task_off.as<uint32_t>(), S.task_cnt.as<uint32_t>(), hot_a, hot_counts, (uint32_t)cap);
    PM_HIP(ctx, hipGetLastError());
    hipLaunchKernelGGL((k_task_fold<C, 64>), dim3(1024), dim3(256), 256 * sizeof(XYZZ28<C>), ctx->stream, S.partials.as<XYZZ<C>>(),
                       S.task_off.as<uint32_t>(), S.task_cnt.as<uint32_t>(), hot_b, hot_counts + 1, (uint32_t)cap);
    PM_HIP(ctx, hipGetLastError());
    return PM_OK;
}

static int task_order(pm_ctx *ctx, MsmSet &S, const BucketPlan &p) {
    MsmWorkspace &ws = ctx->msm;
    const size_t G = p.NB, seg = p.seg;
    const uint32_t *counts = S.counts.as<uint32_t>();
    unsigned lshift = 0;
    while (((seg - 1) >> lshift) + 1 > TASK_MAX_BINS) ++lshift;
    const unsigned nbins = (unsigned)(((seg - 1) >> lshift) + 1);
    PM_HIP(ctx, S.tasks.reserve(p.max_tasks * sizeof(uint4)));
    PM_HIP(ctx, ws.len_bins.reserve((3 * (size_t)nbins + 5) * 4));
    uint32_t *ticket = ws.len_bins.as<uint32_t>(), *len_cnt = ticket + 1, *len_off = len_cnt + nbins, *len_cursor = len_off + nbins + 1;
    PM_HIP(ctx, hipMemsetAsync(ticket, 0, ((size_t)nbins + 1) * 4, ctx->stream));
    const unsigned blocks = (unsigned)((G + 1023) / 1024);
    hipLaunchKernelGGL(k_task_bins<false>, dim3(blocks), dim3(1024), nbins * 4, ctx->stream, counts, S.bucket_off.as<uint32_t>(),
                       S.task_off.as<uint32_t>(), G, (unsigned)seg, lshift, nbins, len_cnt, (const uint32_t *)nullptr, (uint32_t *)nullptr,
                       (uint4 *)nullptr);
    PM_HIP(ctx, hipGetLastError());
    hipLaunchKernelGGL(k_scan_small, dim3(1), dim3(1024), 0, ctx->stream, len_cnt, len_off, len_cursor, nbins);
    PM_HIP(ctx, hipGetLastError());
    hipLaunchKernelGGL(k_task_bins<true>, dim3(blocks), dim3(1024), nbins * 4, ctx->stream, counts, S.bucket_off.as<uint32_t>(),
                       S.task_off.as<uint32_t>(), G, (unsigned)seg, lshift, nbins, (uint32_t *)nullptr, len_off, len_cursor,
                       S.tasks.as<uint4>());
    PM_HIP(ctx, hipGetLastError());
    return PM_OK;
}

template <class C, bool TABLE>
static int accumulate(pm_ctx *ctx, MsmSet &S, const BucketPlan &p, const void *points) {
    int per_cu = 0, cus = 0;
    PM_HIP(ctx, hipOccupancyMaxActiveBlocksPerMultiprocessor(&per_cu, (const void *)k_accumulate<C, TABLE>, 128, 0));
    PM_HIP(ctx, hipDeviceGetAttribute(&cus, hipDeviceAttributeMultiprocessorCount, ctx->device));
    size_t blocks = (size_t)(per_cu > 0 ? per_cu : 1) * (size_t)(cus > 0 ? cus : 1);
    if (blocks > (p.max_tasks + 127) / 128) blocks = (p.max_tasks + 127) / 128;
    hipLaunchKernelGGL((k_accumulate<C, TABLE>), dim3((unsigned)blocks), dim3(128), 0, ctx->stream, S.sorted.as<uint32_t>(),
                       S.task_off.as<uint32_t>(), S.tasks.as<uint4>(), points, S.partials.as<XYZZ<C>>(), p.NB, ctx->msm.len_bins.as<uint32_t>());
    PM_HIP(ctx, hipGetLastError());
    return PM_OK;
}

template <class C>
static int reduce_single_level(pm_ctx *ctx, MsmSet &S, const BucketPlan &p, XYZZ<C> **out) {
    const unsigned sets = p.n_wide_sets;
    PM_HIP(ctx, ctx->msm.wsum.reserve(((size_t)sets * p.bpw + sets) * sizeof(XYZZ<C>)));
    XYZZ<C> *parts = ctx->msm.wsum.as<XYZZ<C>>(), *sums = parts + (size_t)sets * p.bpw;
    hipLaunchKernelGGL(k_bucket_reduce<C>, dim3(sets * p.bpw), dim3(p.red_block), p.red_block * sizeof(XYZZ28<C>), ctx->stream,
                       S.partials.as<XYZZ<C>>(), S.task_off.as<uint32_t>(), S.task_cnt.as<uint32_t>(), (unsigned)p.NB1, p.red_lanes, p.bpw, parts);
    PM_HIP(ctx, hipGetLastError());
    hipLaunchKernelGGL(k_sum_parts<C>, dim3(sets), dim3(64), 0, ctx->stream, parts, p.bpw, sums);
    PM_HIP(ctx, hipGetLastError());
    *out = sums;
    return PM_OK;
}

template <class C>
static XYZZ<C> host_horner(const XYZZ<C> *sums , unsigned nsums, const unsigned char *width) {
    XYZZ<C> acc = XYZZ<C>::identity();
    for (int w = (int)nsums - 1; w >= 0; --w) {
        for (unsigned k = 0; k < width[w]; ++k) acc = xyzz_dbl<C>(acc);
        acc = xyzz_add<C>(acc, xyzz_internal_to_std<C>(sums[w]));
    }
    return acc;
}
template <class C>
static void host_finish(const XYZZ<C> &acc, Affine<C> *out, int *inf) {
    *inf = acc.is_identity() ? 1 : 0;
    *out = xyzz_to_affine<C>(acc);
}

template <class C>
static int sort_windows(pm_ctx *ctx, MsmSet &S, const BucketPlan &p, const Affine<C> *d_bases, const Fp<typename C::FrP> *d_scalars) {
    MsmWorkspace &ws = ctx->msm;
    PM_HIP(ctx, ws.digits.reserve(p.E * 4));
    uint32_t *counts = S.counts.as<uint32_t>(), *cursor = counts + p.NB, *digits = ws.digits.as<uint32_t>();
    const unsigned nbuckets = (unsigned)p.NB1;
    PM_HIP(ctx, hipMemsetAsync(counts, 0, 2 * p.NB * 4, ctx->stream));
    hipLaunchKernelGGL(k_digits<C>, dim3((unsigned)((p.len + 255) / 256)), dim3(256), 0, ctx->stream, d_scalars, d_bases, digits, p.len, p.c, p.nwin);
    PM_HIP(ctx, hipGetLastError());
    const size_t lds = (size_t)nbuckets * 4;
    if (lds > 48 * 1024) {
        PM_HIP(ctx, hipFuncSetAttribute((const void *)k_hist, hipFuncAttributeMaxDynamicSharedMemorySize, (int)lds));
        PM_HIP(ctx, hipFuncSetAttribute((const void *)k_scatter, hipFuncAttributeMaxDynamicSharedMemorySize, (int)lds));
    }
    hipLaunchKernelGGL(k_hist, dim3(p.nchunks, p.nwin), dim3(1024), lds, ctx->stream, digits, counts, p.len, p.chunk, nbuckets);
    PM_HIP(ctx, hipGetLastError());
    PM_TRY(bucket_scan(ctx, S, p));
    hipLaunchKernelGGL(k_scatter, dim3(p.nchunks, p.nwin), dim3(1024), lds, ctx->stream, digits, S.bucket_off.as<uint32_t>(), cursor,
                       S.sorted.as<uint32_t>(), p.len, p.chunk, nbuckets);
    PM_HIP(ctx, hipGetLastError());
    return PM_OK;
}

struct SortBuffers {
    uint16_t *keys;
    uint32_t *vals, *region_count, *region_off, *region_cursor;
};

template <class P, unsigned NWIN = 10>
static int sort_first_level(pm_ctx *ctx, const BucketPlan &p, const MsmTables &tb, const Fp<P> *d_scalars, const SortBuffers &b) {
    if (p.nwin != NWIN) {
        if constexpr (NWIN < 32) return sort_first_level<P, NWIN + 1>(ctx, p, tb, d_scalars, b);
        return PM_ERR_INVALID_ARG;
    }
    hipStream_t st = ctx->stream;
    const unsigned char *inf = tb.inf + tb.base_index;
    const unsigned pblocks = (unsigned)((p.len + p.pbd - 1) / p.pbd);
    const BlockScanShape bsh = block_scan_shape(pblocks, p.regions);
    PM_HIP(ctx, ctx->msm.block_cnt.reserve(((size_t)pblocks + bsh.G) * p.regions * 4));
    uint32_t *block_cnt = ctx->msm.block_cnt.as<uint32_t>(), *block_partial = block_cnt + (size_t)pblocks * p.regions;
    PM_HIP(ctx, hipMemsetAsync(b.region_count, 0, (size_t)p.regions * 4, st));
    hipLaunchKernelGGL((k_tbl_count<P, NWIN>), dim3(pblocks), dim3(p.pbd), 0, st, d_scalars, inf, p.len, p.regions, block_cnt, p.win_buckets,
                       p.narrow_buckets);
    hipLaunchKernelGGL(k_block_sums, dim3(bsh.G), dim3(1024), 0, st, block_cnt, pblocks, p.regions, bsh, block_partial);
    hipLaunchKernelGGL(k_block_offsets, dim3(bsh.G), dim3(1024), 0, st, block_cnt, pblocks, p.regions, bsh, block_partial, b.region_count);
    hipLaunchKernelGGL(k_region_offsets, dim3(1), dim3(1024), 0, st, b.region_count, b.region_off, b.region_cursor, p.regions);
    PM_HIP(ctx, hipFuncSetAttribute((const void *)k_tbl_partition<P, NWIN>, hipFuncAttributeMaxDynamicSharedMemorySize, (int)p.plds));
    hipLaunchKernelGGL((k_tbl_partition<P, NWIN>), dim3(pblocks), dim3(p.pbd), p.plds, st, d_scalars, inf, p.len, p.regions, b.region_off, block_cnt,
                       p.wide ? (size_t)0 : tb.stride, tb.base_index, b.keys, b.vals, p.win_buckets, p.narrow_buckets);
    PM_HIP(ctx, hipGetLastError());
    return PM_OK;
}

constexpr unsigned SUB_BINS = 128, FIN_BINS = 256, FIN_BITS = 8;

static int sort_three_levels(pm_ctx *ctx, MsmSet &S, const BucketPlan &p, const SortBuffers &b) {
    MsmWorkspace &ws = ctx->msm;
    hipStream_t st = ctx->stream;
    const unsigned nsub = p.regions * SUB_BINS, chunk = 1u << RS_CHUNK_LOG;
    PM_HIP(ctx, ws.sub.reserve((3 * (size_t)nsub + 4) * 4));
    PM_HIP(ctx, ws.digits2.reserve(p.keys_bytes + p.E * 4 + 128));
    uint32_t *counts = S.counts.as<uint32_t>(), *cursor = counts + p.NB;
    uint32_t *sub_count = ws.sub.as<uint32_t>(), *sub_off = sub_count + nsub, *sub_cursor = sub_off + nsub + 1;
    uint16_t *keys2 = (uint16_t *)ws.digits2.p;
    uint32_t *vals2 = (uint32_t *)((uint8_t *)ws.digits2.p + p.keys_bytes);
    const unsigned sblocks = (unsigned)((p.E + chunk - 1) / chunk), stblocks = (unsigned)((p.E + ST_CHUNK - 1) / ST_CHUNK);
    PM_HIP(ctx, hipMemsetAsync(sub_count, 0, (size_t)nsub * 4, st));
    hipLaunchKernelGGL(k_hist_small, dim3(sblocks), dim3(1024), 0, st, b.keys, b.region_off, p.regions, FIN_BITS, SUB_BINS, chunk, sub_count);
    PM_HIP(ctx, hipGetLastError());
    hipLaunchKernelGGL(k_scan_small, dim3(1), dim3(1024), 0, st, sub_count, sub_off, sub_cursor, nsub);
    PM_HIP(ctx, hipGetLastError());
    hipLaunchKernelGGL(k_region_pass_staged<RS_MID>, dim3(stblocks), dim3(ST_THREADS), 0, st, b.keys, b.vals, b.region_off, p.regions,
                       FIN_BITS, SUB_BINS, sub_off, sub_cursor, (uint32_t *)nullptr, keys2, vals2);
    PM_HIP(ctx, hipGetLastError());
    hipLaunchKernelGGL(k_hist_small, dim3(sblocks), dim3(1024), 0, st, keys2, sub_off, nsub, 0u, FIN_BINS, chunk, counts);
    PM_HIP(ctx, hipGetLastError());
    PM_TRY(bucket_scan(ctx, S, p));
    hipLaunchKernelGGL(k_region_pass_staged<RS_FINAL>, dim3(stblocks), dim3(ST_THREADS), 0, st, keys2, vals2, sub_off, nsub, 0u,
                       FIN_BINS, S.bucket_off.as<uint32_t>(), cursor, S.sorted.as<uint32_t>(), (uint16_t *)nullptr, (uint32_t *)nullptr);
    PM_HIP(ctx, hipGetLastError());
    return PM_OK;
}

static int sort_one_region(pm_ctx *ctx, MsmSet &S, const BucketPlan &p, const SortBuffers &b) {
    hipStream_t st = ctx->stream;
    const unsigned chunk = 1u << RS_CHUNK_LOG, sblocks = (unsigned)((p.E + chunk - 1) / chunk);
    const size_t lds = (size_t)p.lo_buckets * 4;
    uint32_t *counts = S.counts.as<uint32_t>(), *cursor = counts + p.NB;
    hipLaunchKernelGGL(k_region_pass<RS_HIST>, dim3(sblocks), dim3(1024), lds, st, b.keys, b.vals, b.region_off, p.regions, 0u,
                       p.lo_buckets, chunk, counts, (const uint32_t *)nullptr, (uint32_t *)nullptr, (uint32_t *)nullptr,
                       (uint16_t *)nullptr, (uint32_t *)nullptr);
    PM_HIP(ctx, hipGetLastError());
    PM_TRY(bucket_scan(ctx, S, p));
    hipLaunchKernelGGL(k_region_pass<RS_FINAL>, dim3(sblocks), dim3(1024), lds, st, b.keys, b.vals, b.region_off, p.regions, 0u,
                       p.lo_buckets, chunk, (uint32_t *)nullptr, S.bucket_off.as<uint32_t>(), cursor, S.sorted.as<uint32_t>(),
                       (uint16_t *)nullptr, (uint32_t *)nullptr);
    PM_HIP(ctx, hipGetLastError());
    return PM_OK;
}

template <class C>
static int sort_tables(pm_ctx *ctx, MsmSet &S, const BucketPlan &p, const MsmTables &tb, const Fp<typename C::FrP> *d_scalars) {
    MsmWorkspace &ws = ctx->msm;
    PM_HIP(ctx, ws.digits.reserve(p.keys_bytes + p.E * 4 + 128));
    PM_HIP(ctx, ws.region.reserve((3 * (size_t)p.regions + 4) * 4));
    SortBuffers b;
    b.keys = (uint16_t *)ws.digits.p;
    b.vals = (uint32_t *)((uint8_t *)ws.digits.p + p.keys_bytes);
    b.region_count = ws.region.as<uint32_t>();
    b.region_off = b.region_count + p.regions;
    b.region_cursor = b.region_off + p.regions + 1;
    PM_HIP(ctx, hipMemsetAsync(S.counts.as<uint32_t>(), 0, 2 * p.NB * 4, ctx->stream));
    PM_TRY((sort_first_level<typename C::FrP>(ctx, p, tb, d_scalars, b)));
    return p.lo_buckets == (1u << LO_BITS) ? sort_three_levels(ctx, S, p, b) : sort_one_region(ctx, S, p, b);
}

template <class C>
static int msm_enqueue(pm_ctx *ctx, const BucketPlan &p, const MsmTables *tb, const Affine<C> *d_bases, const Fp<typename C::FrP> *d_scalars,
                       XYZZ<C> *h_sums) {
    MsmSet &S = ctx->msm.set;
    if (p.wide && !d_bases) return PM_ERR_INVALID_ARG;
    PM_TRY(reserve_set<C>(ctx, S, p));
    {
        StageTimer t(ctx, T_MSM_SORT);
        PM_TRY(p.tables ? sort_tables<C>(ctx, S, p, *tb, d_scalars) : sort_windows<C>(ctx, S, p, d_bases, d_scalars));
        PM_TRY(task_order(ctx, S, p));
    }
    {
        StageTimer t(ctx, T_MSM_ACCUMULATE);
        if (p.tables && !p.wide) PM_TRY((accumulate<C, true>(ctx, S, p, tb->table)));
        else PM_TRY((accumulate<C, false>(ctx, S, p, (const void *)d_bases)));
    }
    StageTimer t(ctx, T_MSM_REDUCE);
    PM_TRY(fold_hot_buckets<C>(ctx, S, p));
    XYZZ<C> *d_sums = nullptr;
    if (!p.two_level) {
        PM_TRY(reduce_single_level<C>(ctx, S, p, &d_sums));
    } else {
        PM_TRY(reduce_two_level<C>(ctx, p.NB1, &d_sums, p.n_wide_sets));
    }
    PM_HIP(ctx, hipMemcpyAsync(h_sums, d_sums, p.n_wide_sets * sizeof(XYZZ<C>), hipMemcpyDeviceToHost, ctx->stream));
    if (p.n_narrow_sets) {
        PM_TRY(reduce_two_level<C>(ctx, p.NBn, &d_sums, p.n_narrow_sets, (size_t)p.n_wide_sets * p.NB1));
        PM_HIP(ctx, hipMemcpyAsync(h_sums + p.n_wide_sets, d_sums, p.n_narrow_sets * sizeof(XYZZ<C>), hipMemcpyDeviceToHost, ctx->stream));
    }
    return PM_OK;
}

template <class C>
int msm_run(pm_ctx *ctx, const Affine<C> *d_bases, const Fp<typename C::FrP> *d_scalars, size_t len, Affine<C> *h_out,
            int *h_inf, const MsmTables *tables) {
    const bool tbl = tables && tables->c;
    const size_t max_piece = msm_max_piece(ctx);
    XYZZ<C> acc = XYZZ<C>::identity();
    std::vector<XYZZ<C>> sums;
    for (size_t off = 0; off < len; off += max_piece) {
        StageTimer t_total(ctx, T_MSM_TOTAL);
        const size_t cnt = len - off < max_piece ? len - off : max_piece;
        MsmTables tb;
        if (tbl) {
            tb = *tables;
            tb.base_index += off;
        }
        BucketPlan p;
        PM_TRY(bucket_plan(tbl ? &tb : nullptr, cnt, (unsigned)C::FrP::BITS, ctx->opt.v[PM_OPT_MSM_TASK_LEN], p));
        sums.resize(p.nsums);
        PM_TRY(msm_enqueue<C>(ctx, p, tbl ? &tb : nullptr, tbl ? d_bases : d_bases + off, d_scalars + off, sums.data()));
        PM_HIP(ctx, hipStreamSynchronize(ctx->stream));
        acc = xyzz_add<C>(acc, host_horner<C>(sums.data(), p.nsums, p.width));
    }
    host_finish<C>(acc, h_out, h_inf);
    return PM_OK;
}

template <class C>
int msm_begin(pm_ctx *ctx, const Affine<C> *d_bases, const Fp<typename C::FrP> *d_scalars, size_t len, const MsmTables *tables) {
    ctx->msm_async = 0;
    const bool tbl = tables && tables->c && !tables->wide;
    if (!ctx_pinned(ctx)) { ctx->err = "pinned result slot allocation failed"; return PM_ERR_HIP; }
    if (len == 0 || !tbl || len > msm_max_piece(ctx)) {
        PM_TRY(msm_run<C>(ctx, d_bases, d_scalars, len, pinned_slot<Affine<C>>(ctx, PINNED_MSM_POINT), pinned_slot<int>(ctx, PINNED_MSM_INF), tables));
        ctx->msm_async = 2;
        return PM_OK;
    }
    StageTimer t_total(ctx, T_MSM_TOTAL);
    BucketPlan p;
    PM_TRY(bucket_plan(tables, len, (unsigned)C::FrP::BITS, ctx->opt.v[PM_OPT_MSM_TASK_LEN], p));
    PM_TRY(msm_enqueue<C>(ctx, p, tables, d_bases, d_scalars, pinned_slot<XYZZ<C>>(ctx, PINNED_MSM_SUM)));
    ctx->msm_async = 1;
    return PM_OK;
}

template <class C>
int msm_end(pm_ctx *ctx, Affine<C> *h_out, int *h_inf) {
    if (ctx->msm_async == 2) {
        *h_out = *pinned_slot<const Affine<C>>(ctx, PINNED_MSM_POINT);
        *h_inf = *pinned_slot<const int>(ctx, PINNED_MSM_INF);
    } else if (ctx->msm_async == 1) {
        PM_HIP(ctx, hipStreamSynchronize(ctx->stream));
        const unsigned char width0 = 0;
        host_finish<C>(host_horner<C>(pinned_slot<const XYZZ<C>>(ctx, PINNED_MSM_SUM), 1, &width0), h_out, h_inf);
    } else {
        return PM_ERR_STATE;
    }
    ctx->msm_async = 0;
    return PM_OK;
}

template int msm_begin<BlsCurve>(pm_ctx *, const Affine<BlsCurve> *, const Fp<BlsFrP> *, size_t, const MsmTables *);
template int msm_begin<BnCurve>(pm_ctx *, const Affine<BnCurve> *, const Fp<BnFrP> *, size_t, const MsmTables *);
template int msm_end<BlsCurve>(pm_ctx *, Affine<BlsCurve> *, int *);
template int msm_end<BnCurve>(pm_ctx *, Affine<BnCurve> *, int *);
template int msm_run<BlsCurve>(pm_ctx *, const Affine<BlsCurve> *, const Fp<BlsFrP> *, size_t, Affine<BlsCurve> *, int *, const MsmTables *);
template int msm_run<BnCurve>(pm_ctx *, const Affine<BnCurve> *, const Fp<BnFrP> *, size_t, Affine<BnCurve> *, int *, const MsmTables *);

}
```

polymath_amd/csrc/ntt.hip:

```cpp
#include <cstring>
#include <type_traits>

#include "internal.h"
#include "fq28.cuh"

namespace pm {

template <class P>
struct PowTable {
    Fp<P> w[33];
};

template <class RR>
struct alignas(8) Tw28 {
    uint32_t l[RR::N];
};

template <class P, class RR>
__global__ void k_twiddles(Fp<P> *out, Fp<P> *out_int, Tw28<RR> *out28, size_t count, PowTable<P> tab, unsigned nbits) {
    size_t j = (size_t)blockIdx.x * blockDim.x + threadIdx.x;
    if (j >= count) return;
    Fp<P> acc = Fp<P>::one();
    for (unsigned k = 0; k < nbits; ++k)
        if ((j >> k) & 1) acc = mul<P>(acc, tab.w[k]);
// ... 232 lines not shown
            stage(std::true_type{});
        else
            stage(std::false_type{});
        __syncthreads();
    }
}

template <class P, class RR>
__device__ __forceinline__ void l28_emit(const F28<RR> &v, Fp<P> *dst, const F28<RR> &scale28, int do_scale, bool short_pass) {
    Fp<P> out;
    if (do_scale)
        l28_pack_canonical<RR>(l28_canonical<RR, 0>(f28_mul<RR>(v, scale28)), out.l);
    else if (short_pass)
        l28_pack_canonical<RR>(l28_canonical<RR, 4>(f28_weak_norm<RR>(v)), out.l);
    else
        l28_pack_canonical<RR>(l28_canonical<RR, 5>(f28_weak_norm<RR>(v)), out.l);
    *dst = out;
}

template <class P, class RR, unsigned TH>
__global__ __launch_bounds__(TH) __attribute__((amdgpu_waves_per_eu(4, 4))) void k_ntt_pass28(const Fp<P> *a, Fp<P> *dst, const Tw28<RR> *tw, unsigned log_n, unsigned s0, unsigned ns,
                                                             unsigned log_cols, Fp<P> scale_int, int do_scale, int pair_stages) {
    extern __shared__ __attribute__((aligned(16))) unsigned char smem_raw[];
    uint32_t *t = (uint32_t *)smem_raw;
    constexpr unsigned tile = L28_EPL * TH;
    const unsigned cols = 1u << log_cols;
    const size_t lo_groups = ((size_t)1 << s0) >> log_cols, g = blockIdx.x;
    const size_t hi = g / lo_groups, lo0 = (g % lo_groups) << log_cols, base = (hi << (s0 + ns)) + lo0;
    for (unsigned e8 = threadIdx.x; e8 < tile; e8 += L28_EPL * TH) {
        Fp<P> v[L28_EPL];
#pragma unroll
        for (unsigned q = 0; q < L28_EPL; ++q) {
            const unsigned e = e8 + q * TH, r = e >> log_cols, c = e & (cols - 1);
            if (e < tile) v[q] = a[base + ((size_t)r << s0) + c];
        }
#pragma unroll
        for (unsigned q = 0; q < L28_EPL; ++q) {
            const unsigned e = e8 + q * TH;
            if (e < tile) l28_store<RR, tile>(t, e, f28_unpack<RR>(v[q].l));
        }
    }
    __syncthreads();
    l28_stages<P, RR, false, TH>(t, tw, log_n, s0, ns, log_cols, lo0, pair_stages != 0);
    const F28<RR> sc = f28_unpack<RR>(scale_int.l);
    for (unsigned e = threadIdx.x; e < tile; e += TH) {
        const unsigned r = e >> log_cols, c = e & (cols - 1);
        l28_emit<P, RR>(l28_load<RR, tile>(t, e), &dst[base + ((size_t)r << s0) + c], sc, do_scale, ns <= 7);
    }
}

template <class P, class RR, unsigned TH>
__global__ __launch_bounds__(TH) __attribute__((amdgpu_waves_per_eu(4, 4))) void k_ntt_first_pass28(const Fp<P> *src, Fp<P> *dst, const Tw28<RR> *tw, unsigned log_n, unsigned ns,
                                                                   unsigned log_cols, int pair_stages) {
    extern __shared__ __attribute__((aligned(16))) unsigned char smem_raw[];
    uint32_t *t = (uint32_t *)smem_raw;
    constexpr unsigned tile = L28_EPL * TH;
    const unsigned cols = 1u << log_cols, rows = 1u << ns, H = log_n - ns, cm = cols - 1;
    const size_t g = blockIdx.x;
    for (unsigned e8 = threadIdx.x; e8 < tile; e8 += L28_EPL * TH) {
        Fp<P> v[L28_EPL];
#pragma unroll
        for (unsigned q = 0; q < L28_EPL; ++q) {
            const unsigned e = e8 + q * TH, rb = e >> log_cols, c = e & cm;
            if (e < tile) v[q] = src[((size_t)rb << H) + (g << log_cols) + c];
        }
#pragma unroll
        for (unsigned q = 0; q < L28_EPL; ++q) {
            const unsigned e = e8 + q * TH, rb = e >> log_cols, c = e & cm, r = __brev(rb) >> (32 - ns);
            if (e < tile) l28_store<RR, tile>(t, r * cols + ((c + r) & cm), f28_unpack<RR>(v[q].l));
        }
    }
    __syncthreads();
    l28_stages<P, RR, true, TH>(t, tw, log_n, 0, ns, log_cols, 0, pair_stages != 0);
    const F28<RR> none = f28_zero<RR>();
    for (unsigned e = threadIdx.x; e < tile; e += TH) {
        const unsigned c = e >> ns, r = e & (rows - 1);
        const size_t hi = __brevll((unsigned long long)((g << log_cols) + c)) >> (64 - H);
        l28_emit<P, RR>(l28_load<RR, tile>(t, r * cols + ((c + r) & cm)), &dst[(hi << ns) + r], none, 0, ns <= 7);
    }
}

template <class P>
__global__ void k_scale(Fp<P> *a, size_t n, Fp<P> s) {
    size_t i = (size_t)blockIdx.x * blockDim.x + threadIdx.x;
    if (i < n) a[i] = mul<P>(a[i], s);
}

static bool ntt_l28_domain(unsigned log_n) {
    const unsigned tile_log = log_n > 24 ? (unsigned)LOG_TILE + 1 : (unsigned)LOG_TILE;
    return log_n >= tile_log + 3;
}

template <class C>
static int twiddles_slot(pm_ctx *ctx, unsigned log_n, TwiddleCache **out) {
    typedef typename C::FrP P;
    typedef typename C::FrRR RR;
    typedef typename C::FrNttRR NttRR;
    typedef Fp<P> Fr;
    const int cid = C::ID;
    TwiddleCache *slot = nullptr;
    for (auto &t : ctx->tw)
        if (t.curve == cid && t.log_n == log_n) slot = &t;
    if (slot) slot->stamp = ++ctx->tw_clock;
    if (!slot) {
        slot = &ctx->tw[0];
        for (auto &t : ctx->tw)
            if (t.stamp < slot->stamp) slot = &t;
        slot->stamp = ++ctx->tw_clock;
        slot->curve = cid;
        slot->log_n = log_n;
        const bool l28 = ntt_l28_domain(log_n);
        size_t half = log_n ? ((size_t)1 << (log_n - 1)) : 1;
        const size_t int_bytes = half * (l28 ? sizeof(Tw28<NttRR>) : sizeof(Fr));
        PM_HIP(ctx, slot->fwd.reserve(half * sizeof(Fr)));
        PM_HIP(ctx, slot->inv.reserve(half * sizeof(Fr)));
        PM_HIP(ctx, slot->fwd_int.reserve(int_bytes));
        PM_HIP(ctx, slot->inv_int.reserve(int_bytes));
        Fr root;
        for (int i = 0; i < P::N; ++i) root.l[i] = C::ROOT_MONT[i];
        for (unsigned i = log_n; i < (unsigned)C::TWO_ADICITY; ++i) root = sqr<P>(root);
        Fr rinv = inverse<P>(root);
        for (int dir = 0; dir < 2; ++dir) {
            PowTable<P> tab;
            Fr w = dir ? rinv : root;
            for (unsigned k = 0; k < 33; ++k) {
                tab.w[k] = w;
                w = sqr<P>(w);
            }
            Fr *dst = dir ? slot->inv.as<Fr>() : slot->fwd.as<Fr>();
            DevBuf &ib = dir ? slot->inv_int : slot->fwd_int;
            unsigned blocks = (unsigned)((half + 255) / 256);
            if (l28)
                hipLaunchKernelGGL((k_twiddles<P, NttRR>), dim3(blocks), dim3(256), 0, ctx->stream, dst, (Fr *)nullptr, ib.as<Tw28<NttRR>>(), half,
                                   tab, log_n ? log_n - 1 : 0);
            else
                hipLaunchKernelGGL((k_twiddles<P, RR>), dim3(blocks), dim3(256), 0, ctx->stream, dst, ib.as<Fr>(), (Tw28<RR> *)nullptr, half, tab,
                                   log_n ? log_n - 1 : 0);
            PM_HIP(ctx, hipGetLastError());
        }
    }
    *out = slot;
    return PM_OK;
}

template <class C>
int twiddles_get(pm_ctx *ctx, unsigned log_n, bool inv_dir, const Fp<typename C::FrP> **out) {
    TwiddleCache *slot = nullptr;
    PM_TRY(twiddles_slot<C>(ctx, log_n, &slot));
    *out = inv_dir ? slot->inv.as<Fp<typename C::FrP>>() : slot->fwd.as<Fp<typename C::FrP>>();
    return PM_OK;
}

template <class C>
int ntt_run(pm_ctx *ctx, Fp<typename C::FrP> *d, unsigned log_n, bool inv_dir) {
    typedef typename C::FrP P;
    typedef Fp<P> Fr;
    if (log_n > (unsigned)C::TWO_ADICITY) return PM_ERR_DOMAIN_TOO_LARGE;
    if (log_n == 0) return PM_OK;
    StageTimer timer(ctx, T_NTT);
    const size_t n = (size_t)1 << log_n;
    TwiddleCache *slot = nullptr;
    PM_TRY(twiddles_slot<C>(ctx, log_n, &slot));
    const DevBuf &twb = inv_dir ? slot->inv_int : slot->fwd_int;
    const Fr *tw = twb.as<Fr>();
    const unsigned tile_log = log_n > 24 ? (unsigned)LOG_TILE + 1 : (unsigned)LOG_TILE;
    const Fr ninv = inv_dir ? inverse<P>(from_u64<P>((uint64_t)n)) : Fr::one();
    if (ntt_l28_domain(log_n)) {
        PM_HIP(ctx, ctx->ntt_tmp.reserve(n * sizeof(Fr)));
        Fr *tmp = ctx->ntt_tmp.as<Fr>();
        typedef typename C::FrNttRR RR;
        const Tw28<RR> *tw28 = twb.as<Tw28<RR>>();
        const unsigned p8 = (log_n + 7) / 8, p9 = (log_n + 8) / 9, npass = p9 < p8 ? p9 : p8;
        const unsigned ns_max = log_n / npass + (log_n % npass ? 1 : 0);
#ifndef PM_NTT_TH_SMALL_MAX_NS
#define PM_NTT_TH_SMALL_MAX_NS 8
#endif
        const bool small = ns_max <= PM_NTT_TH_SMALL_MAX_NS;
        const unsigned tile_log28 = small ? 10 : 11;
        if (!ctx->ntt_lds_attr[C::ID]) {
            PM_HIP(ctx, hipFuncSetAttribute((const void *)k_ntt_pass28<P, RR, 512>, hipFuncAttributeMaxDynamicSharedMemorySize, (int)(((size_t)1 << 11) * RR::N * 4)));
            PM_HIP(ctx, hipFuncSetAttribute((const void *)k_ntt_first_pass28<P, RR, 512>, hipFuncAttributeMaxDynamicSharedMemorySize, (int)(((size_t)1 << 11) * RR::N * 4)));
            ctx->ntt_lds_attr[C::ID] = true;
        }
        Fr scale_int;
        for (int i = 0; i < P::N; ++i) scale_int.l[i] = RR::STD2INT[i];
        scale_int = mul<P>(ninv, scale_int);
        const int pair_stages = 1;
        unsigned s0 = 0;
        for (unsigned k = 0; k < npass; ++k) {
            const unsigned ns = log_n / npass + (k < log_n % npass ? 1 : 0);
            unsigned log_cols = tile_log28 - ns;
            if (k && s0 < log_cols) return PM_ERR_STATE;
            const bool last = s0 + ns == log_n;
            if (k == 0) {
                const dim3 grid((unsigned)(n >> (ns + log_cols)));
                const size_t lds = ((size_t)1 << (ns + log_cols)) * RR::N * 4;
                if (small)
                    hipLaunchKernelGGL((k_ntt_first_pass28<P, RR, 256>), grid, dim3(256), lds, ctx->stream, (const Fr *)d, tmp, tw28, log_n, ns, log_cols, pair_stages);
                else
                    hipLaunchKernelGGL((k_ntt_first_pass28<P, RR, 512>), grid, dim3(512), lds, ctx->stream, (const Fr *)d, tmp, tw28, log_n, ns, log_cols, pair_stages);
            } else {
                if (s0 < log_cols) log_cols = s0;
                const dim3 grid((unsigned)(n >> (ns + log_cols)));
                const size_t lds = ((size_t)1 << (ns + log_cols)) * RR::N * 4;
                if (small)
                    hipLaunchKernelGGL((k_ntt_pass28<P, RR, 256>), grid, dim3(256), lds, ctx->stream, (const Fr *)tmp, last ? d : tmp, tw28, log_n, s0, ns,
                                       log_cols, scale_int, last && inv_dir ? 1 : 0, pair_stages);
                else
                    hipLaunchKernelGGL((k_ntt_pass28<P, RR, 512>), grid, dim3(512), lds, ctx->stream, (const Fr *)tmp, last ? d : tmp, tw28, log_n, s0, ns,
                                       log_cols, scale_int, last && inv_dir ? 1 : 0, pair_stages);
            }
            PM_HIP(ctx, hipGetLastError());
            s0 += ns;
        }
        return PM_OK;
    }
    hipLaunchKernelGGL(k_bitrev<P>, dim3((unsigned)((n + 255) / 256)), dim3(256), 0, ctx->stream, d, log_n);
    PM_HIP(ctx, hipGetLastError());
    unsigned s0 = 0;
    while (s0 < log_n) {
        unsigned ns = log_n - s0 < tile_log ? log_n - s0 : tile_log;
        unsigned log_cols = 11 - ns < 3 ? 11 - ns : 3;
        if (s0 < log_cols) log_cols = s0;
        size_t tiles = n >> (ns + log_cols);
        size_t lds = ((size_t)1 << (ns + log_cols)) * sizeof(Fr);
        hipLaunchKernelGGL((k_ntt_pass<P, typename C::FrRR>), dim3((unsigned)tiles), dim3(256), lds, ctx->stream, (const Fr *)d, d, tw, log_n, s0, ns,
                           log_cols, ninv, 0);
        PM_HIP(ctx, hipGetLastError());
        s0 += ns;
    }
    if (inv_dir) {
        hipLaunchKernelGGL(k_scale<P>, dim3((unsigned)((n + 255) / 256)), dim3(256), 0, ctx->stream, d, n, ninv);
        PM_HIP(ctx, hipGetLastError());
    }
    return PM_OK;
}

template int twiddles_get<BlsCurve>(pm_ctx *, unsigned, bool, const Fp<BlsFrP> **);
template int twiddles_get<BnCurve>(pm_ctx *, unsigned, bool, const Fp<BnFrP> **);
template int ntt_run<BlsCurve>(pm_ctx *, Fp<BlsFrP> *, unsigned, bool);
template int ntt_run<BnCurve>(pm_ctx *, Fp<BnFrP> *, unsigned, bool);

}
```

polymath_amd/csrc/prove.hip:

```cpp
#include <cstring>

#include <thread>

#include "internal.h"
#include "fq28.cuh"
#include "prove_common.cuh"

namespace pm {

template <class P>
__global__ void k_witness_rows(CsrDev A, CsrDev B, CsrDev Cm, const Fp<P> *xw, Fp<P> *ue, Fp<P> *we, Fp<P> *y,
                               uint64_t m0, uint64_t nr) {
    uint64_t r = (uint64_t)blockIdx.x * blockDim.x + threadIdx.x;
    if (r >= nr) return;
    Fp<P> az = csr_row_dot<P>(A.rowptr, A.col, A.val, xw, r);
    Fp<P> bz = csr_row_dot<P>(B.rowptr, B.col, B.val, xw, r);
    Fp<P> cz = csr_row_dot<P>(Cm.rowptr, Cm.col, Cm.val, xw, r);
    Fp<P> d = sub<P>(az, bz), d2 = sqr<P>(d);
    Fp<P> c4 = dbl<P>(dbl<P>(cz));
    y[m0 + r] = d2;
    ue[2 * m0 + r] = add<P>(az, bz);
    we[2 * m0 + r] = add<P>(c4, d2);
    ue[2 * m0 + nr + r] = d;
    we[2 * m0 + nr + r] = d2;
// ... 281 lines not shown
template <class P>
__global__ void k_div_top(const Fp<P> *in, uint64_t count, Fp<P> xp, Fp<P> *H) {
    if (threadIdx.x || blockIdx.x) return;
    Fp<P> acc = Fp<P>::zero();
    H[count] = acc;
    for (uint64_t k = count; k-- > 0;) {
        acc = add<P>(mul<P>(acc, xp), in[k]);
        H[k] = acc;
    }
}

template <class P>
__global__ void k_div_expandN(const Fp<P> *in, uint64_t count, Fp<P> xp, unsigned L, uint64_t nchunks, const Fp<P> *Hup,
                              Fp<P> *H) {
    uint64_t t = (uint64_t)blockIdx.x * blockDim.x + threadIdx.x;
    if (t >= nchunks) return;
    uint64_t lo = t * L, hi = lo + L;
    if (hi > count) hi = count;
    Fp<P> acc = Hup[t + 1];
    for (uint64_t k = hi; k-- > lo;) {
        acc = add<P>(mul<P>(acc, xp), in[k]);
        H[k] = acc;
    }
    if (t == nchunks - 1) H[count] = Fp<P>::zero();
}

template <class P>
__global__ void k_div_expand0(NumParams np, NumConsts<P> nc, NumMul28<typename Radix28<P>::RR> m28, const Fp<P> *u, const Fp<P> *wit_u, const Fp<P> *u2,
                              unsigned L, uint64_t nchunks, const Fp<P> *Hup, Fp<P> *q, unsigned *flags) {
    typedef typename Radix28<P>::RR RR;
    uint64_t t = (uint64_t)blockIdx.x * blockDim.x + threadIdx.x;
    if (t >= nchunks) return;
    uint64_t lo = t * L, hi = lo + L;
    if (hi > np.len) hi = np.len;
    F28<RR> acc = f28_unpack<RR>(Hup[t + 1].l);
    {
        const uint64_t s = np.sigma, n = np.n;
        const bool zeros = (lo >= 2 && hi <= 2 * s) || (lo >= 2 * s + 3 && hi <= 3 * s) || (lo >= 3 * s + n && hi <= 5 * s) ||
                           (lo >= 5 * s + n + 1 && hi <= 8 * s);
        if (zeros) {
            for (uint64_t k = hi; k-- > lo;) {
                acc = f28_mul<RR>(acc, m28.x1);
                Fp<P> out;
                f28_pack_reduced<RR>(acc, out.l);
                q[k - 1] = out;
            }
            return;
        }
    }
    for (uint64_t k = hi; k-- > lo;) {
        acc = f28_canonical_lazy<RR, 3>(horner28_step<P, RR>(acc, k, np, nc, m28, u, wit_u, u2));
        Fp<P> out;
        f28_pack_canonical<RR>(acc, out.l);
        if (k > 0) q[k - 1] = out;
        else if (!out.is_zero()) atomicOr(flags, 8u);
    }
}

template <class C>
int msm_resident(pm_ctx *ctx, const pm_pk *pk, int which, const Fp<typename C::FrP> *d_scalars, uint64_t *out_xy, int *out_inf) {
    const Affine<C> *bases = (const Affine<C> *)pk->d_bases + pk->res_dev_off[which];
    Affine<C> r;
    int inf = 1;
    if (pk->tables[which].c) {
        MsmTables tb = pk->tables[which];
        tb.base_index = 0;
        PM_TRY(msm_run<C>(ctx, tb.wide ? bases : (const Affine<C> *)nullptr, d_scalars, (size_t)pk->res_cnt[which], &r, &inf, &tb));
    } else {
        PM_TRY(msm_run<C>(ctx, bases, d_scalars, (size_t)pk->res_cnt[which], &r, &inf));
    }
    store_affine_host<C>(r, inf, out_xy, out_inf);
    return PM_OK;
}

template <class C>
int msm_resident_begin(pm_ctx *ctx, const pm_pk *pk, int which, const Fp<typename C::FrP> *d_scalars, uint64_t lo, uint64_t count) {
    const Affine<C> *bases = (const Affine<C> *)pk->d_bases + pk->res_dev_off[which];
    if (count == 0) { lo = 0; count = pk->res_cnt[which]; }
    if (lo + count > pk->res_cnt[which]) return PM_ERR_INVALID_ARG;
    if (pk->tables[which].c) {
        MsmTables tb = pk->tables[which];
        tb.base_index = (size_t)lo;
        return msm_begin<C>(ctx, tb.wide ? bases : (const Affine<C> *)nullptr, d_scalars + lo, (size_t)count, &tb);
    }
    return msm_begin<C>(ctx, bases + lo, d_scalars + lo, (size_t)count, (const MsmTables *)nullptr);
}
template <class C>
int msm_resident_end(pm_ctx *ctx, uint64_t *out_xy, int *out_inf) {
    Affine<C> r;
    int inf = 1;
    PM_TRY(msm_end<C>(ctx, &r, &inf));
    store_affine_host<C>(r, inf, out_xy, out_inf);
    return PM_OK;
}

template <class C>
static int msm_shard(pm_ctx *ctx, const pm_pk *pk, int which, const Fp<typename C::FrP> *d_scalars, uint64_t *out_xy,
                     int *out_inf) {
    return msm_resident<C>(ctx, pk, which, d_scalars + pk->res_lo[which], out_xy, out_inf);
}

template <class C>
int prove_phase1_impl(pm_ctx *ctx, const pm_pk *pk, const uint64_t *x, const uint64_t *w, const uint64_t *r_a,
                      uint64_t *a_xy, int *a_inf, uint64_t *c_xy, int *c_inf, bool assignment_on_device) {
    typedef typename C::FrP P;
    typedef Fp<P> Fr;
    const uint64_t n = pk->n, m0 = pk->m0, mw = pk->mw, nr = pk->nr;
    const uint64_t Lz = 2 * m0 + mw + nr;
    if (pk->log_n + 1 > (unsigned)C::TWO_ADICITY) return PM_ERR_DOMAIN_TOO_LARGE;
    hipStream_t st = ctx->stream;
    if (!ctx->keep_timings) timing_reset(ctx);
    ctx->pk = pk;
    ctx->phase = 0;
    TimingGuard timing_guard{ctx};
    StageTimer t_phase(ctx, T_PHASE);
    const uint64_t len_c = Lz + (n - 1) + (n + 1) + 3 + 2, len_a = n + 3;
    PM_HIP(ctx, ctx->xw.reserve((m0 + mw) * sizeof(Fr)));
    PM_HIP(ctx, ctx->ue.reserve(n * sizeof(Fr)));
    PM_HIP(ctx, ctx->we.reserve(n * sizeof(Fr)));
    PM_HIP(ctx, ctx->u.reserve(n * sizeof(Fr)));
    PM_HIP(ctx, ctx->w.reserve(n * sizeof(Fr)));
    PM_HIP(ctx, ctx->wit_u.reserve(n * sizeof(Fr)));
    PM_HIP(ctx, ctx->u2.reserve(2 * n * sizeof(Fr)));
    PM_HIP(ctx, ctx->sc_c.reserve(len_c * sizeof(Fr)));
    PM_HIP(ctx, ctx->sc_a.reserve(len_a * sizeof(Fr)));
    PM_HIP(ctx, ctx->ra.reserve(2 * sizeof(Fr)));
    PM_HIP(ctx, ctx->flags.reserve(64));
    Fr *xw = ctx->xw.as<Fr>(), *ue = ctx->ue.as<Fr>(), *we = ctx->we.as<Fr>(), *u = ctx->u.as<Fr>(), *wv = ctx->w.as<Fr>();
    Fr *wit_u = ctx->wit_u.as<Fr>(), *u2 = ctx->u2.as<Fr>(), *sc_c = ctx->sc_c.as<Fr>(), *sc_a = ctx->sc_a.as<Fr>();
    Fr *ra = ctx->ra.as<Fr>();
    unsigned *flags = ctx->flags.as<unsigned>();
    PM_HIP(ctx, hipMemsetAsync(flags, 0, 64, st));
    const hipMemcpyKind kind = assignment_on_device ? hipMemcpyDeviceToDevice : hipMemcpyHostToDevice;
    PM_HIP(ctx, hipMemcpyAsync(xw, x, m0 * sizeof(Fr), kind, st));
    if (mw) PM_HIP(ctx, hipMemcpyAsync(xw + m0, w, mw * sizeof(Fr), kind, st));
    PM_HIP(ctx, hipMemcpyAsync(ra, r_a, 2 * sizeof(Fr), hipMemcpyHostToDevice, st));
    memcpy(ctx->ra_host, r_a, 2 * sizeof(Fr));
    {
        StageTimer t(ctx, T_WITNESS_MAP);
        CsrDev A{pk->d_rowptr[0], pk->d_col[0], pk->d_val[0]}, B{pk->d_rowptr[1], pk->d_col[1], pk->d_val[1]},
            Cm{pk->d_rowptr[2], pk->d_col[2], pk->d_val[2]};
        Fr *ztail = sc_c;
        uint64_t head = n > m0 + mw ? n : m0 + mw;
        hipLaunchKernelGGL(k_witness_head<P>, dim3(nblk(head)), dim3(256), 0, st, xw, ue, we, ztail, m0, mw, nr, n);
        PM_HIP(ctx, hipGetLastError());
        if (nr) {
            hipLaunchKernelGGL(k_witness_rows<P>, dim3(nblk(nr)), dim3(256), 0, st, A, B, Cm, xw, ue, we, ztail + m0 + mw,
                               m0, nr);
            PM_HIP(ctx, hipGetLastError());
        }
        hipLaunchKernelGGL(k_check_sap<P>, dim3(nblk(n)), dim3(256), 0, st, ue, we, n, flags);
        PM_HIP(ctx, hipGetLastError());
    }
    PM_HIP(ctx, hipMemcpyAsync(u, ue, n * sizeof(Fr), hipMemcpyDeviceToDevice, st));
    PM_HIP(ctx, hipMemcpyAsync(wv, we, n * sizeof(Fr), hipMemcpyDeviceToDevice, st));
    PM_TRY(ntt_run<C>(ctx, u, pk->log_n, true));
    const bool overlap = ctx->opt.v[PM_OPT_MSM_OVERLAP] != 0;
    pm_ctx *const aux_ctx = overlap ? ctx_aux(ctx) : nullptr;
    int st_a = PM_OK;
    struct Joiner {
        pm_worker *w;
        bool pending;
        void join() { if (pending) { w->wait(); pending = false; } }
        ~Joiner() { join(); }
    } helper{&ctx->worker, false};
    bool a_early = aux_ctx != nullptr;
    if (a_early) {
        pm_ctx *aux = ctx->aux;
        hipLaunchKernelGGL(k_sc_a<P>, dim3(nblk(n)), dim3(256), 0, st, u, ra, sc_a, n);
        PM_HIP(ctx, hipGetLastError());
        PM_HIP(ctx, hipEventRecord(ctx->ev_sc_a, st));
        timing_reset_aux(ctx, aux);
        {
            helper.pending = ctx->worker.submit([&, aux] {
                if (hipSetDevice(aux->device) != hipSuccess || hipStreamWaitEvent(aux->stream, ctx->ev_sc_a, 0) != hipSuccess) {
                    st_a = PM_ERR_HIP;
                    aux->err = "helper stream setup failed";
                    return;
                }
                try {
                    st_a = msm_shard<C>(aux, pk, 0, sc_a, a_xy, a_inf);
                } catch (const std::exception &e) {
                    st_a = PM_ERR_STATE;
                    aux->err = e.what();
                }
                timing_flush(aux);
            });
            if (!helper.pending) a_early = false;
        }
    }
    PM_TRY(ntt_run<C>(ctx, wv, pk->log_n, true));
    if (2 * m0 <= 16 && pk->log_n >= 1) {
        const Fr *winv = nullptr;
        PM_TRY(twiddles_get<C>(ctx, pk->log_n, true, &winv));
        StageTimer t(ctx, T_NTT);
        hipLaunchKernelGGL(k_wit_u_sparse<P>, dim3(nblk(n)), dim3(256), 0, st, u, ue, winv, inverse<P>(from_u64<P>(n)), n,
                           (unsigned)(2 * m0), wit_u);
        PM_HIP(ctx, hipGetLastError());
    } else {
        hipLaunchKernelGGL(k_copy_zero_head<P>, dim3(nblk(n)), dim3(256), 0, st, ue, wit_u, n, 2 * m0);
        PM_HIP(ctx, hipGetLastError());
        PM_TRY(ntt_run<C>(ctx, wit_u, pk->log_n, true));
    }
    {
        const Fr *psi = nullptr, *psi_inv = nullptr;
        PM_TRY(twiddles_get<C>(ctx, pk->log_n + 1, false, &psi));
        PM_TRY(twiddles_get<C>(ctx, pk->log_n + 1, true, &psi_inv));
        PM_HIP(ctx, ctx->scratch.reserve(n * sizeof(Fr)));
        Fr *tmp = ctx->scratch.as<Fr>();
        hipLaunchKernelGGL(k_twist<P>, dim3(nblk(n)), dim3(256), 0, st, u, psi, tmp, n);
        PM_HIP(ctx, hipGetLastError());
        PM_TRY(ntt_run<C>(ctx, tmp, pk->log_n, false));
        hipLaunchKernelGGL(k_square<P>, dim3(nblk(n)), dim3(256), 0, st, tmp, n);
        PM_HIP(ctx, hipGetLastError());
        PM_TRY(ntt_run<C>(ctx, tmp, pk->log_n, true));
        Fr half = inverse<P>(from_u64<P>(2));
        hipLaunchKernelGGL(k_untwist_combine<P>, dim3(nblk(n)), dim3(256), 0, st, tmp, psi_inv, wv, u2, n, half);
        PM_HIP(ctx, hipGetLastError());
    }
    {
        StageTimer t(ctx, T_POLY);
        hipLaunchKernelGGL(k_phase1_scalars<P>, dim3(nblk(n + 1)), dim3(256), 0, st, u, u2, ra, sc_c + Lz, a_early ? (Fr *)nullptr : sc_a, n,
                           flags);
        PM_HIP(ctx, hipGetLastError());
    }
    if (!ctx_pinned(ctx)) { ctx->err = "pinned staging allocation failed"; return PM_ERR_HIP; }
    volatile unsigned *hflags_p = pinned_slot<volatile unsigned>(ctx, PINNED_FLAGS);
    *hflags_p = 0;
    PM_HIP(ctx, hipMemcpyAsync((void *)hflags_p, flags, 4, hipMemcpyDeviceToHost, st));
    if (a_early) {
        const int st_c = msm_shard<C>(ctx, pk, 1, sc_c, c_xy, c_inf);
        helper.join();
        timing_absorb_aux(ctx, ctx->aux);
        const hipError_t e_sync = hipStreamSynchronize(st);
        if (st_a != PM_OK && st_c != PM_OK) { ctx->err = ctx->aux->err; return st_a; }
        PM_HIP(ctx, e_sync);
        const unsigned hf = *hflags_p;
        if (hf & 1u) return PM_ERR_REMAINDER_NONZERO;
        if ((hf & 2u) || !(hf & 4u)) return PM_ERR_DEGREE_BOUND;
        if (st_a != PM_OK) { ctx->err = ctx->aux->err; return st_a; }
        PM_TRY(st_c);
    } else {
        const int s_a = msm_shard<C>(ctx, pk, 0, sc_a, a_xy, a_inf);
        const int s_c = s_a == PM_OK ? msm_shard<C>(ctx, pk, 1, sc_c, c_xy, c_inf) : (int)PM_OK;
        const hipError_t e_sync = hipStreamSynchronize(st);
        PM_TRY(s_a);
        PM_HIP(ctx, e_sync);
        const unsigned hf = *hflags_p;
        if (hf & 1u) return PM_ERR_REMAINDER_NONZERO;
        if ((hf & 2u) || !(hf & 4u)) return PM_ERR_DEGREE_BOUND;
        PM_TRY(s_c);
    }
    t_phase.stop();
    timing_flush(ctx);
    ctx->phase = 1;
    return PM_OK;
}

template <class C>
int prove_phase2_impl(pm_ctx *ctx, const uint64_t *x1_in, uint64_t *u_at_x1) {
    typedef typename C::FrP P;
    typedef Fp<P> Fr;
    if (ctx->phase < 1 || !ctx->pk) return PM_ERR_STATE;
    const uint64_t n = ctx->pk->n;
    hipStream_t st = ctx->stream;
    Fr x1 = load_fr<P>(x1_in);
    const unsigned L = 16;
    uint64_t lanes = (n + L - 1) / L;
    unsigned blocks = nblk(lanes);
    PM_HIP(ctx, ctx->scratch.reserve(((size_t)blocks + 1) * sizeof(Fr)));
    Fr *part = ctx->scratch.as<Fr>();
    hipLaunchKernelGGL(k_horner_partial<P>, dim3(blocks), dim3(256), 0, st, ctx->u.as<Fr>(), n, x1, L, part);
    PM_HIP(ctx, hipGetLastError());
    hipLaunchKernelGGL(k_sum_small<P>, dim3(1), dim3(256), 0, st, part, blocks, part + blocks);
    PM_HIP(ctx, hipGetLastError());
    PM_HIP(ctx, hipMemcpyAsync(u_at_x1, part + blocks, sizeof(Fr), hipMemcpyDeviceToHost, st));
    PM_HIP(ctx, hipStreamSynchronize(st));
    ctx->phase = 2;
    return PM_OK;
}

template <class C>
int prove_phase3_impl(pm_ctx *ctx, const uint64_t *x1_in, const uint64_t *x2_in, const uint64_t *a_in,
                      const uint64_t *c_in, uint64_t *d_xy, int *d_inf) {
    typedef typename C::FrP P;
    typedef Fp<P> Fr;
    if (ctx->phase < 1 || !ctx->pk) return PM_ERR_STATE;
    const pm_pk *pk = ctx->pk;
    hipStream_t st = ctx->stream;
    if (!ctx->keep_timings) timing_reset(ctx);
    TimingGuard timing_guard{ctx};
    StageTimer t_phase(ctx, T_PHASE);
    const uint64_t n = pk->n, sigma = pk->sigma;
    Fr x1 = load_fr<P>(x1_in), x2 = load_fr<P>(x2_in), a_at = load_fr<P>(a_in), c_at = load_fr<P>(c_in);
    Fr rah[2];
    memcpy(rah, ctx->ra_host, sizeof(rah));
    NumParams np{n, sigma, 8 * sigma + 2 * n - 1};
    const NumConsts<P> nc = make_num_consts<P>(x2, rah, a_at, c_at);
    const NumMul28<typename Radix28<P>::RR> m28 = make_num_mul28<P>(x1, nc);
    const unsigned L = 16;
    uint64_t cnt[8];
    cnt[0] = np.len;
    int levels = 0;
    while (cnt[levels] > 64 && levels < 6) {
        cnt[levels + 1] = (cnt[levels] + L - 1) / L;
        ++levels;
    }
    Fr *V[8] = {nullptr}, *H[8] = {nullptr};
    for (int l = 1; l <= levels; ++l) {
        PM_HIP(ctx, ctx->lvl[l - 1].reserve((2 * cnt[l] + 2) * sizeof(Fr)));
        V[l] = ctx->lvl[l - 1].as<Fr>();
        H[l] = V[l] + cnt[l];
    }
    PM_HIP(ctx, ctx->quotient.reserve((np.len + 1) * sizeof(Fr)));
    Fr *q = ctx->quotient.as<Fr>();
    unsigned *flags = ctx->flags.as<unsigned>();
    const Fr *u = ctx->u.as<Fr>(), *wit_u = ctx->wit_u.as<Fr>(), *u2 = ctx->u2.as<Fr>();
    {
        StageTimer t(ctx, T_POLY);
        PM_HIP(ctx, hipMemsetAsync(flags, 0, 64, st));
        Fr xp[8];
        xp[0] = x1;
        for (int l = 1; l <= levels; ++l) xp[l] = pow_u64<P>(xp[l - 1], L);
        if (levels == 0) {
            PM_HIP(ctx, ctx->lvl[0].reserve(2 * sizeof(Fr)));
            Fr *zero = ctx->lvl[0].as<Fr>();
            PM_HIP(ctx, hipMemsetAsync(zero, 0, 2 * sizeof(Fr), st));
            hipLaunchKernelGGL(k_div_expand0<P>, dim3(1), dim3(64), 0, st, np, nc, m28, u, wit_u, u2, (unsigned)np.len, (uint64_t)1,
                               zero, q, flags);
            PM_HIP(ctx, hipGetLastError());
        } else {
            hipLaunchKernelGGL(k_div_level0<P>, dim3(nblk(cnt[1])), dim3(256), 0, st, np, nc, m28, u, wit_u, u2, L, cnt[1], V[1]);
            PM_HIP(ctx, hipGetLastError());
            for (int l = 1; l < levels; ++l) {
                hipLaunchKernelGGL(k_div_levelN<P>, dim3(nblk(cnt[l + 1])), dim3(256), 0, st, V[l], cnt[l], xp[l], L,
                                   cnt[l + 1], V[l + 1]);
                PM_HIP(ctx, hipGetLastError());
            }
            hipLaunchKernelGGL(k_div_top<P>, dim3(1), dim3(64), 0, st, V[levels], cnt[levels], xp[levels], H[levels]);
            PM_HIP(ctx, hipGetLastError());
            for (int l = levels - 1; l >= 1; --l) {
                hipLaunchKernelGGL(k_div_expandN<P>, dim3(nblk(cnt[l + 1])), dim3(256), 0, st, V[l], cnt[l], xp[l], L,
                                   cnt[l + 1], H[l + 1], H[l]);
                PM_HIP(ctx, hipGetLastError());
// ... 34 lines not shown
```

Baseline: 18.20 million constraints/s.

## Fuse MSM scan/bin/count kernels and let NTT read from source buffer

Folds the length-histogram pass into the tile scan, with a last-arriving workgroup doing the totals and length-bin offsets. Hot-bucket listing moves into the task-binning kernel, and the two fold tiers become one launch. Region and sub-histogram memsets and offset kernels are removed, and repeated LDS attribute calls are cached. The proof path's NTT now reads directly from the witness buffers instead of copying first. Together these cut kernel launches, memsets and device-to-device copies, at the cost of inter-workgroup atomic completion logic that must be correct.

Result: no change. 18.23 million constraints/s (median of 6 runs) (+0.2%).

```diff
diff --git a/polymath_amd/api.py b/polymath_amd/api.py
--- a/polymath_amd/api.py
+++ b/polymath_amd/api.py
@@ -418,6 +418,11 @@
         self.L.pm_last_timings(self.h, arr, len(TIMING_SLOTS))
         return dict(zip(TIMING_SLOTS, list(arr)))
 
+    def msm_fold_counts(self):
+        arr = (ct.c_double * (len(TIMING_SLOTS) + 2))()
+        self.check(self.L.pm_last_timings(self.h, arr, len(TIMING_SLOTS) + 2))
+        return int(arr[len(TIMING_SLOTS)]), int(arr[len(TIMING_SLOTS) + 1])
+
     def ntt(self, curve, data, log_n, inverse=False):
         data = _c(data).copy()
         self.check(self.L.pm_ntt(self.h, CURVE_IDS[curve], _p(data), log_n, int(inverse)))
diff --git a/polymath_amd/csrc/api.hip b/polymath_amd/csrc/api.hip
--- a/polymath_amd/csrc/api.hip
+++ b/polymath_amd/csrc/api.hip
@@ -180,6 +180,14 @@
         timing_flush_now(ctx);
     }
     for (int i = 0; i < n_slots; ++i) ms_out[i] = i < T_NUM_SLOTS ? ctx->timing_ms[i] : 0.0;
+    if (n_slots > T_NUM_SLOTS && ctx->msm.set.hot_counts) {
+        uint32_t hot[2] = {0, 0};
+        if (hipSetDevice(ctx->device) != hipSuccess) return PM_ERR_HIP;
+        PM_HIP(ctx, hipMemcpyAsync(hot, ctx->msm.set.hot_counts, sizeof(hot), hipMemcpyDeviceToHost, ctx->stream));
+        PM_HIP(ctx, hipStreamSynchronize(ctx->stream));
+        ms_out[T_NUM_SLOTS] = hot[0];
+        if (n_slots > T_NUM_SLOTS + 1) ms_out[T_NUM_SLOTS + 1] = hot[1];
+    }
     return PM_OK;
 }
 
diff --git a/polymath_amd/csrc/internal.h b/polymath_amd/csrc/internal.h
--- a/polymath_amd/csrc/internal.h
+++ b/polymath_amd/csrc/internal.h
@@ -81,10 +81,14 @@
 
 struct MsmSet {
     DevBuf sorted, counts, bucket_off, task_off, tasks, partials, task_cnt;
+    const uint32_t *hot_counts = nullptr;
 };
 struct MsmWorkspace {
     MsmSet set;
     DevBuf digits, cursor, wsum, region, sub, digits2, len_bins, block_cnt, hot;
+    unsigned resident_blocks[2][2] = {};
+    size_t partition_lds[2][33] = {};
+    size_t hist_lds = 0;
 };
 
 struct MsmTables {
@@ -274,7 +278,7 @@
 int host_threads_env();
 
 template <class C>
-int ntt_run(pm_ctx *ctx, Fp<typename C::FrP> *d_data, unsigned log_n, bool inverse);
+int ntt_run(pm_ctx *ctx, Fp<typename C::FrP> *d_data, unsigned log_n, bool inverse, const Fp<typename C::FrP> *d_src = nullptr);
 template <class C>
 int twiddles_get(pm_ctx *ctx, unsigned log_n, bool inv_dir, const Fp<typename C::FrP> **out);
 
diff --git a/polymath_amd/csrc/msm.hip b/polymath_amd/csrc/msm.hip
--- a/polymath_amd/csrc/msm.hip
+++ b/polymath_amd/csrc/msm.hip
@@ -1,5 +1,6 @@
 #include <cstdlib>
 #include <cstring>
+#include <type_traits>
 
 #include "internal.h"
 #include "fq28.cuh"
@@ -105,12 +106,61 @@
     }
 }
 
+__device__ __forceinline__ uint32_t block_inclusive_scan(uint32_t v, uint32_t *wt) {
+    const unsigned lane = threadIdx.x & 63, wave = threadIdx.x >> 6;
+#pragma unroll
+    for (unsigned o = 1; o < 64; o <<= 1) {
+        const uint32_t n = __shfl_up(v, o, 64);
+        if (lane >= o) v += n;
+    }
+    if (lane == 63) wt[wave] = v;
+    __syncthreads();
+    if (wave == 0) {
+        uint32_t w = lane < (blockDim.x >> 6) ? wt[lane] : 0u;
+#pragma unroll
+        for (unsigned o = 1; o < 16; o <<= 1) {
+            const uint32_t n = __shfl_up(w, o, 64);
+            if (lane >= o) w += n;
+        }
+        wt[lane] = w;
+    }
+    __syncthreads();
+    if (wave) v += wt[wave - 1];
+    return v;
+}
+
+__device__ __forceinline__ bool last_workgroup_arrives(uint32_t *counter, uint32_t expected, uint32_t *flag ) {
+    asm volatile("s_waitcnt vmcnt(0)" ::: "memory");
+    __syncthreads();
+    if (threadIdx.x == 0) {
+        __builtin_amdgcn_fence(__ATOMIC_RELEASE, "agent");
+        asm volatile("s_waitcnt vmcnt(0)" ::: "memory");
+        const bool last = __hip_atomic_fetch_add(counter, 1u, __ATOMIC_RELAXED, __HIP_MEMORY_SCOPE_AGENT) + 1u == expected;
+        if (last) {
+            __builtin_amdgcn_fence(__ATOMIC_ACQUIRE, "agent");
+            asm volatile("s_waitcnt vmcnt(0)" ::: "memory");
+        }
+        *flag = last ? 1u : 0u;
+    }
+    __syncthreads();
+    return *flag != 0;
+}
+__device__ __forceinline__ uint32_t load_published(const uint32_t *p) { return __hip_atomic_load(p, __ATOMIC_RELAXED, __HIP_MEMORY_SCOPE_AGENT); }
+
+constexpr unsigned TASK_MAX_BINS = 8192;
+constexpr unsigned SUB_BINS = 128, FIN_BINS = 256, FIN_BITS = 8;
+constexpr unsigned CTL_TICKET = 0, CTL_ARRIVALS = 1, CTL_HOT = 2, CTL_LEN_CNT = 4, CTL_SUB_COUNT = CTL_LEN_CNT + TASK_MAX_BINS;
+
 constexpr unsigned SCAN_PER = 16, SCAN_TILE = 256 * SCAN_PER;
 
 __global__ __launch_bounds__(256) void k_scan_tiles(const uint32_t *counts, uint32_t *bucket_off, uint32_t *task_off,
-                                                    uint32_t *tile_tot, size_t G, unsigned seg) {
-    __shared__ uint32_t s_a[256], s_b[256];
+                                                    uint32_t *tile_tot, size_t G, unsigned seg, unsigned lshift, unsigned nbins,
+                                                    uint32_t *ctl, uint32_t *len_off, uint32_t *len_cursor) {
+    extern __shared__ __attribute__((aligned(16))) unsigned char smem_raw[];
+    uint32_t *h = (uint32_t *)smem_raw;
+    __shared__ uint32_t s_a[256], s_b[256], wt[64], flag;
     const unsigned tid = threadIdx.x;
+    for (unsigned b = tid; b < nbins; b += 256) h[b] = 0;
     const size_t base = (size_t)blockIdx.x * SCAN_TILE + (size_t)tid * SCAN_PER;
     uint32_t c[SCAN_PER], nt[SCAN_PER];
     uint32_t sa = 0, sb = 0;
@@ -124,6 +174,13 @@
     s_a[tid] = sa;
     s_b[tid] = sb;
     __syncthreads();
+#pragma unroll
+    for (unsigned k = 0; k < SCAN_PER; ++k)
+        if (nt[k]) {
+            const uint32_t L = c[k] - (nt[k] - 1) * seg;
+            if (nt[k] > 1) atomicAdd(&h[0], nt[k] - 1);
+            atomicAdd(&h[(seg - L) >> lshift], 1u);
+        }
     for (unsigned off = 1; off < 256; off <<= 1) {
         uint32_t va = 0, vb = 0;
         if (tid >= off) { va = s_a[tid - off]; vb = s_b[tid - off]; }
@@ -140,33 +197,40 @@
         rb += nt[k];
     }
     if (tid == 255) { tile_tot[2 * blockIdx.x] = s_a[255]; tile_tot[2 * blockIdx.x + 1] = s_b[255]; }
-}
-
-__global__ __launch_bounds__(1024) void k_scan_totals(uint32_t *tile_tot, unsigned ntiles, uint32_t *bucket_off,
-                                                      uint32_t *task_off, size_t G) {
-    __shared__ uint32_t s_a[1024], s_b[1024];
-    const unsigned tid = threadIdx.x;
+    uint32_t *len_cnt = ctl + CTL_LEN_CNT;
+    for (unsigned b = tid; b < nbins; b += 256) {
+        const uint32_t v = h[b];
+        if (v) atomicAdd(&len_cnt[b], v);
+    }
+    if (!last_workgroup_arrives(ctl + CTL_ARRIVALS, gridDim.x, &flag)) return;
+    const unsigned ntiles = gridDim.x;
     uint32_t carry_a = 0, carry_b = 0;
-    for (unsigned base = 0; base < ntiles; base += 1024) {
-        unsigned i = base + tid;
-        uint32_t a = i < ntiles ? tile_tot[2 * i] : 0u, b = i < ntiles ? tile_tot[2 * i + 1] : 0u;
-        s_a[tid] = a;
-        s_b[tid] = b;
-        __syncthreads();
-        for (unsigned off = 1; off < 1024; off <<= 1) {
-            uint32_t va = 0, vb = 0;
-            if (tid >= off) { va = s_a[tid - off]; vb = s_b[tid - off]; }
-            __syncthreads();
-            s_a[tid] += va;
-            s_b[tid] += vb;
-            __syncthreads();
-        }
-        if (i < ntiles) { tile_tot[2 * i] = carry_a + s_a[tid] - a; tile_tot[2 * i + 1] = carry_b + s_b[tid] - b; }
-        carry_a += s_a[1023];
-        carry_b += s_b[1023];
+    for (unsigned t0 = 0; t0 < ntiles; t0 += 256) {
+        const unsigned i = t0 + tid;
+        const uint32_t a = i < ntiles ? load_published(&tile_tot[2 * i]) : 0u, b = i < ntiles ? load_published(&tile_tot[2 * i + 1]) : 0u;
+        const uint32_t ia = block_inclusive_scan(a, wt);
+        __syncthreads();
+        const uint32_t ib = block_inclusive_scan(b, wt);
+        if (i < ntiles) { tile_tot[2 * i] = carry_a + ia - a; tile_tot[2 * i + 1] = carry_b + ib - b; }
+        if (tid == 255) { s_a[0] = ia; s_b[0] = ib; }
+        __syncthreads();
+        carry_a += s_a[0];
+        carry_b += s_b[0];
         __syncthreads();
     }
     if (tid == 0) { bucket_off[G] = carry_a; task_off[G] = carry_b; }
+    uint32_t carry = 0;
+    for (unsigned b0 = 0; b0 < nbins; b0 += 256) {
+        const unsigned i = b0 + tid;
+        const uint32_t v = i < nbins ? load_published(&len_cnt[i]) : 0u;
+        const uint32_t iv = block_inclusive_scan(v, wt);
+        if (i < nbins) { len_off[i] = carry + iv - v; len_cursor[i] = 0; }
+        if (tid == 255) s_a[0] = iv;
+        __syncthreads();
+        carry += s_a[0];
+        __syncthreads();
+    }
+    if (tid == 0) len_off[nbins] = carry;
 }
 
 __global__ __launch_bounds__(256) void k_scan_add(uint32_t *bucket_off, uint32_t *task_off, const uint32_t *tile_tot, size_t G) {
@@ -207,12 +271,12 @@
     }
 }
 
-constexpr unsigned TASK_MAX_BINS = 8192;
-
-template <bool SCATTER>
+constexpr uint32_t FOLD_MIN = 8, FOLD_BLOCK_MIN = 1024;
+
 __global__ __launch_bounds__(1024) void k_task_bins(const uint32_t *counts, const uint32_t *bucket_off, const uint32_t *task_off, size_t G,
-                                                    unsigned seg, unsigned lshift, unsigned nbins, uint32_t *len_cnt, const uint32_t *len_off,
-                                                    uint32_t *len_cursor, uint4 *tasks) {
+                                                    unsigned seg, unsigned lshift, unsigned nbins, const uint32_t *len_off,
+                                                    uint32_t *len_cursor, uint4 *tasks, uint32_t *task_cnt, uint32_t *hot_a, uint32_t *hot_b,
+                                                    uint32_t *hot_counts , uint32_t cap) {
     extern __shared__ __attribute__((aligned(16))) unsigned char smem_raw[];
     uint32_t *h = (uint32_t *)smem_raw;
     for (unsigned b = threadIdx.x; b < nbins; b += blockDim.x) h[b] = 0;
@@ -223,6 +287,7 @@
     if (g < G) {
         t0 = task_off[g];
         n = task_off[g + 1] - t0;
+        task_cnt[g] = n;
         if (n) {
             cnt = counts[g];
             const uint32_t L = cnt - (n - 1) * seg;
@@ -230,25 +295,25 @@
             if (n > 1) rank_full = atomicAdd(&h[0], n - 1);
             rank_last = atomicAdd(&h[bin], 1u);
         }
-    }
-    __syncthreads();
-    if (!SCATTER) {
-        for (unsigned b = threadIdx.x; b < nbins; b += blockDim.x) {
-            const uint32_t v = h[b];
-            if (v) atomicAdd(&len_cnt[b], v);
-        }
-    } else {
-        for (unsigned b = threadIdx.x; b < nbins; b += blockDim.x) {
-            const uint32_t v = h[b];
-            if (v) h[b] = len_off[b] + atomicAdd(&len_cursor[b], v);
-        }
-        __syncthreads();
-        if (n) {
-            const uint32_t at = h[0] + rank_full, first = bucket_off[g];
-            for (uint32_t k = 0; k + 1 < n; ++k)
-                tasks[at + k] = make_uint4(t0 + k, first + k * seg, first + (k + 1) * seg, 0u);
-            tasks[h[bin] + rank_last] = make_uint4(t0 + n - 1, first + (n - 1) * seg, first + cnt, 0u);
-        }
+        if (n > FOLD_BLOCK_MIN) {
+            const uint32_t i = atomicAdd(&hot_counts[0], 1u);
+            if (i < cap) hot_a[i] = (uint32_t)g;
+        } else if (n > FOLD_MIN) {
+            const uint32_t i = atomicAdd(&hot_counts[1], 1u);
+            if (i < cap) hot_b[i] = (uint32_t)g;
+        }
+    }
+    __syncthreads();
+    for (unsigned b = threadIdx.x; b < nbins; b += blockDim.x) {
+        const uint32_t v = h[b];
+        if (v) h[b] = len_off[b] + atomicAdd(&len_cursor[b], v);
+    }
+    __syncthreads();
+    if (n) {
+        const uint32_t at = h[0] + rank_full, first = bucket_off[g];
+        for (uint32_t k = 0; k + 1 < n; ++k)
+            tasks[at + k] = make_uint4(t0 + k, first + k * seg, first + (k + 1) * seg, 0u);
+        tasks[h[bin] + rank_last] = make_uint4(t0 + n - 1, first + (n - 1) * seg, first + cnt, 0u);
     }
 }
 
@@ -310,34 +375,15 @@
     }
 }
 
-constexpr uint32_t FOLD_MIN = 8, FOLD_BLOCK_MIN = 1024;
-
-__global__ void k_task_counts(const uint32_t *task_off, size_t G, uint32_t *task_cnt, uint32_t *hot_a, uint32_t *hot_b,
-                              uint32_t *hot_counts , uint32_t cap) {
-    size_t g = (size_t)blockIdx.x * blockDim.x + threadIdx.x;
-    if (g >= G) return;
-    const uint32_t n = task_off[g + 1] - task_off[g];
-    task_cnt[g] = n;
-    if (n > FOLD_BLOCK_MIN) {
-        const uint32_t i = atomicAdd(&hot_counts[0], 1u);
-        if (i < cap) hot_a[i] = (uint32_t)g;
-    } else if (n > FOLD_MIN) {
-        const uint32_t i = atomicAdd(&hot_counts[1], 1u);
-        if (i < cap) hot_b[i] = (uint32_t)g;
-    }
-}
+constexpr unsigned FOLD_BLOCKS_A = 256, FOLD_BLOCKS_B = 1024;
 
 template <class C, unsigned LANES>
-__global__ __launch_bounds__(256) __attribute__((amdgpu_waves_per_eu(2, 2))) void k_task_fold(XYZZ<C> *partials, const uint32_t *task_off, uint32_t *task_cnt,
-                                                   const uint32_t *hot, const uint32_t *hot_count, uint32_t cap) {
-    extern __shared__ __attribute__((aligned(16))) unsigned char smem_raw[];
-    XYZZ28<C> *sh = (XYZZ28<C> *)smem_raw;
+__device__ __forceinline__ void task_fold(XYZZ28<C> *sh, XYZZ<C> *partials, const uint32_t *task_off, uint32_t *task_cnt, const uint32_t *hot,
+                                          uint32_t listed, unsigned block, unsigned nblocks) {
     typedef typename C::FqRR RR;
-    uint32_t listed = *hot_count;
-    if (listed > cap) listed = cap;
     constexpr unsigned GROUPS = 256 / LANES;
     const unsigned group = threadIdx.x / LANES, lane = threadIdx.x % LANES;
-    for (uint32_t h0 = blockIdx.x * GROUPS; h0 < listed; h0 += gridDim.x * GROUPS) {
+    for (uint32_t h0 = block * GROUPS; h0 < listed; h0 += nblocks * GROUPS) {
         const uint32_t h = h0 + group;
         XYZZ28<C> *acc = &sh[threadIdx.x];
         acc->X = acc->Y = acc->ZZ = acc->ZZZ = f28_zero<RR>();
@@ -361,6 +407,19 @@
         }
         __syncthreads();
     }
+}
+
+template <class C>
+__global__ __launch_bounds__(256) __attribute__((amdgpu_waves_per_eu(2, 2))) void k_task_fold(XYZZ<C> *partials, const uint32_t *task_off, uint32_t *task_cnt,
+                                                   const uint32_t *hot_a, const uint32_t *hot_b, const uint32_t *hot_counts, uint32_t cap) {
+    extern __shared__ __attribute__((aligned(16))) unsigned char smem_raw[];
+    XYZZ28<C> *sh = (XYZZ28<C> *)smem_raw;
+    const bool tier_a = blockIdx.x < FOLD_BLOCKS_A;
+    uint32_t listed = hot_counts[tier_a ? 0 : 1];
+    if (listed > cap) listed = cap;
+    if (listed == 0) return;
+    if (tier_a) task_fold<C, 256>(sh, partials, task_off, task_cnt, hot_a, listed, blockIdx.x, FOLD_BLOCKS_A);
+    else task_fold<C, 64>(sh, partials, task_off, task_cnt, hot_b, listed, blockIdx.x - FOLD_BLOCKS_A, FOLD_BLOCKS_B);
 }
 
 template <class C>
@@ -409,29 +468,6 @@
 
 constexpr unsigned LO_BITS = SORT_REGION_BITS;
 
-__device__ __forceinline__ uint32_t block_inclusive_scan(uint32_t v, uint32_t *wt) {
-    const unsigned lane = threadIdx.x & 63, wave = threadIdx.x >> 6;
-#pragma unroll
-    for (unsigned o = 1; o < 64; o <<= 1) {
-        const uint32_t n = __shfl_up(v, o, 64);
-        if (lane >= o) v += n;
-    }
-    if (lane == 63) wt[wave] = v;
-    __syncthreads();
-    if (wave == 0) {
-        uint32_t w = lane < (blockDim.x >> 6) ? wt[lane] : 0u;
-#pragma unroll
-        for (unsigned o = 1; o < 16; o <<= 1) {
-            const uint32_t n = __shfl_up(w, o, 64);
-            if (lane >= o) w += n;
-        }
-        wt[lane] = w;
-    }
-    __syncthreads();
-    if (wave) v += wt[wave - 1];
-    return v;
-}
-
 template <class P>
 __device__ __forceinline__ Fp<P> canon_scalar(const Fp<P> *scalars, const unsigned char *inf, size_t i) {
     Fp<P> k = from_mont<P>(scalars[i]);
@@ -516,8 +552,8 @@
     }
 }
 __global__ __launch_bounds__(1024) void k_block_offsets(uint32_t *block_cnt, unsigned nblocks, unsigned regions, BlockScanShape h, const uint32_t *partial,
-                                                        uint32_t *region_count) {
-    __shared__ uint32_t s[1024], base[1024];
+                                                        uint32_t *region_off) {
+    __shared__ uint32_t s[1024], base[1024], wt[64];
     const unsigned t = threadIdx.x, j = t / regions, r = t % regions, g = blockIdx.x;
     if (j < h.rows) {
         uint32_t acc = 0;
@@ -548,28 +584,16 @@
             run += v;
         }
     }
-    if (g == gridDim.x - 1 && t < regions) {
-        uint32_t tot = base[t];
-        for (unsigned jj = 0; jj < h.rows; ++jj) tot += s[jj * regions + t];
-        region_count[t] = tot;
-    }
-}
-
-__global__ __launch_bounds__(1024) void k_region_offsets(const uint32_t *region_count, uint32_t *region_off, uint32_t *region_cursor,
-                                                         unsigned regions) {
-    __shared__ uint32_t s[1024];
-    const unsigned t = threadIdx.x;
-    uint32_t v = t < regions ? region_count[t] : 0u;
-    s[t] = v;
-    __syncthreads();
-    for (unsigned off = 1; off < 1024; off <<= 1) {
-        uint32_t a = t >= off ? s[t - off] : 0u;
-        __syncthreads();
-        s[t] += a;
-        __syncthreads();
-    }
-    if (t < regions) { region_off[t] = s[t] - v; region_cursor[t] = 0; }
-    if (t == 1023) region_off[regions] = s[1023];
+    if (g == gridDim.x - 1) {
+        uint32_t tot = 0;
+        if (t < regions) {
+            tot = base[t];
+            for (unsigned jj = 0; jj < h.rows; ++jj) tot += s[jj * regions + t];
+        }
+        const uint32_t incl = block_inclusive_scan(tot, wt);
+        if (t < regions) region_off[t] = incl - tot;
+        if (t == 1023) region_off[regions] = incl;
+    }
 }
 
 template <class P, unsigned NWIN>
@@ -926,86 +950,94 @@
 }
 
 
+static size_t ctl_words(const BucketPlan &p) { return CTL_SUB_COUNT + (p.tables ? (size_t)p.regions * SUB_BINS : 0); }
+static uint32_t *set_ctl(const MsmSet &S, const BucketPlan &p) { return S.counts.as<uint32_t>() + 2 * p.NB; }
+
 template <class C>
 static int reserve_set(pm_ctx *ctx, MsmSet &S, const BucketPlan &p) {
     PM_HIP(ctx, S.sorted.reserve(p.E * 4 + 16));
-    PM_HIP(ctx, S.counts.reserve(2 * p.NB * 4));
+    PM_HIP(ctx, S.counts.reserve((2 * p.NB + ctl_words(p)) * 4));
     PM_HIP(ctx, S.bucket_off.reserve((p.NB + 1) * 4));
     PM_HIP(ctx, S.task_off.reserve((p.NB + 1) * 4));
     PM_HIP(ctx, S.partials.reserve(p.max_tasks * sizeof(XYZZ<C>)));
     PM_HIP(ctx, S.task_cnt.reserve(p.NB * 4));
     PM_HIP(ctx, ctx->msm.cursor.reserve(((p.NB + SCAN_TILE - 1) / SCAN_TILE + 1) * 8));
-    return PM_OK;
+    S.hot_counts = set_ctl(S, p) + CTL_HOT;
+    return PM_OK;
+}
+
+static int clear_counters(pm_ctx *ctx, MsmSet &S, const BucketPlan &p) {
+    PM_HIP(ctx, hipMemsetAsync(S.counts.as<uint32_t>(), 0, (2 * p.NB + ctl_words(p)) * 4, ctx->stream));
+    return PM_OK;
+}
+
+struct TaskBins { unsigned lshift, nbins; };
+static TaskBins task_bins(const BucketPlan &p) {
+    TaskBins b{0, 0};
+    while (((p.seg - 1) >> b.lshift) + 1 > TASK_MAX_BINS) ++b.lshift;
+    b.nbins = (unsigned)(((p.seg - 1) >> b.lshift) + 1);
+    return b;
 }
 
 static int bucket_scan(pm_ctx *ctx, MsmSet &S, const BucketPlan &p) {
-    uint32_t *tile_tot = ctx->msm.cursor.as<uint32_t>(), *bucket_off = S.bucket_off.as<uint32_t>(), *task_off = S.task_off.as<uint32_t>();
+    MsmWorkspace &ws = ctx->msm;
+    uint32_t *tile_tot = ws.cursor.as<uint32_t>(), *bucket_off = S.bucket_off.as<uint32_t>(), *task_off = S.task_off.as<uint32_t>();
     const unsigned ntiles = (unsigned)((p.NB + SCAN_TILE - 1) / SCAN_TILE);
-    hipLaunchKernelGGL(k_scan_tiles, dim3(ntiles), dim3(256), 0, ctx->stream, S.counts.as<uint32_t>(), bucket_off, task_off, tile_tot, p.NB,
-                       (unsigned)p.seg);
-    PM_HIP(ctx, hipGetLastError());
-    hipLaunchKernelGGL(k_scan_totals, dim3(1), dim3(1024), 0, ctx->stream, tile_tot, ntiles, bucket_off, task_off, p.NB);
+    const TaskBins tb = task_bins(p);
+    PM_HIP(ctx, ws.len_bins.reserve((2 * (size_t)tb.nbins + 1) * 4));
+    uint32_t *len_off = ws.len_bins.as<uint32_t>(), *len_cursor = len_off + tb.nbins + 1;
+    hipLaunchKernelGGL(k_scan_tiles, dim3(ntiles), dim3(256), tb.nbins * 4, ctx->stream, S.counts.as<uint32_t>(), bucket_off, task_off, tile_tot, p.NB,
+                       (unsigned)p.seg, tb.lshift, tb.nbins, set_ctl(S, p), len_off, len_cursor);
     PM_HIP(ctx, hipGetLastError());
     hipLaunchKernelGGL(k_scan_add, dim3(ntiles), dim3(256), 0, ctx->stream, bucket_off, task_off, tile_tot, p.NB);
     PM_HIP(ctx, hipGetLastError());
     return PM_OK;
 }
 
+static size_t hot_cap(const BucketPlan &p) {
+    const size_t cap = p.max_tasks > p.NB ? p.max_tasks - p.NB + 1 : 1;
+    return cap / FOLD_MIN + 1;
+}
+
 template <class C>
 static int fold_hot_buckets(pm_ctx *ctx, MsmSet &S, const BucketPlan &p) {
-    MsmWorkspace &ws = ctx->msm;
-    const size_t G = p.NB;
-    size_t cap = p.max_tasks > G ? p.max_tasks - G + 1 : 1;
-    cap = cap / FOLD_MIN + 1;
-    PM_HIP(ctx, ws.hot.reserve((2 * cap + 2) * 4));
-    uint32_t *hot_counts = ws.hot.as<uint32_t>(), *hot_a = hot_counts + 2, *hot_b = hot_a + cap;
-    PM_HIP(ctx, hipMemsetAsync(hot_counts, 0, 8, ctx->stream));
-    hipLaunchKernelGGL(k_task_counts, dim3((unsigned)((G + 255) / 256)), dim3(256), 0, ctx->stream, S.task_off.as<uint32_t>(), G,
-                       S.task_cnt.as<uint32_t>(), hot_a, hot_b, hot_counts, (uint32_t)cap);
-    PM_HIP(ctx, hipGetLastError());
-    hipLaunchKernelGGL((k_task_fold<C, 256>), dim3(256), dim3(256), 256 * sizeof(XYZZ28<C>), ctx->stream, S.partials.as<XYZZ<C>>(),
-                       S.task_off.as<uint32_t>(), S.task_cnt.as<uint32_t>(), hot_a, hot_counts, (uint32_t)cap);
-    PM_HIP(ctx, hipGetLastError());
-    hipLaunchKernelGGL((k_task_fold<C, 64>), dim3(1024), dim3(256), 256 * sizeof(XYZZ28<C>), ctx->stream, S.partials.as<XYZZ<C>>(),
-                       S.task_off.as<uint32_t>(), S.task_cnt.as<uint32_t>(), hot_b, hot_counts + 1, (uint32_t)cap);
+    const size_t cap = hot_cap(p);
+    uint32_t *hot_a = ctx->msm.hot.as<uint32_t>(), *hot_b = hot_a + cap;
+    hipLaunchKernelGGL((k_task_fold<C>), dim3(FOLD_BLOCKS_A + FOLD_BLOCKS_B), dim3(256), 256 * sizeof(XYZZ28<C>), ctx->stream, S.partials.as<XYZZ<C>>(),
+                       S.task_off.as<uint32_t>(), S.task_cnt.as<uint32_t>(), hot_a, hot_b, set_ctl(S, p) + CTL_HOT, (uint32_t)cap);
     PM_HIP(ctx, hipGetLastError());
     return PM_OK;
 }
 
 static int task_order(pm_ctx *ctx, MsmSet &S, const BucketPlan &p) {
     MsmWorkspace &ws = ctx->msm;
-    const size_t G = p.NB, seg = p.seg;
-    const uint32_t *counts = S.counts.as<uint32_t>();
-    unsigned lshift = 0;
-    while (((seg - 1) >> lshift) + 1 > TASK_MAX_BINS) ++lshift;
-    const unsigned nbins = (unsigned)(((seg - 1) >> lshift) + 1);
+    const size_t G = p.NB, cap = hot_cap(p);
+    const TaskBins tb = task_bins(p);
     PM_HIP(ctx, S.tasks.reserve(p.max_tasks * sizeof(uint4)));
-    PM_HIP(ctx, ws.len_bins.reserve((3 * (size_t)nbins + 5) * 4));
-    uint32_t *ticket = ws.len_bins.as<uint32_t>(), *len_cnt = ticket + 1, *len_off = len_cnt + nbins, *len_cursor = len_off + nbins + 1;
-    PM_HIP(ctx, hipMemsetAsync(ticket, 0, ((size_t)nbins + 1) * 4, ctx->stream));
+    PM_HIP(ctx, ws.hot.reserve(2 * cap * 4));
+    uint32_t *len_off = ws.len_bins.as<uint32_t>(), *len_cursor = len_off + tb.nbins + 1, *ctl = set_ctl(S, p);
+    uint32_t *hot_a = ws.hot.as<uint32_t>(), *hot_b = hot_a + cap;
     const unsigned blocks = (unsigned)((G + 1023) / 1024);
-    hipLaunchKernelGGL(k_task_bins<false>, dim3(blocks), dim3(1024), nbins * 4, ctx->stream, counts, S.bucket_off.as<uint32_t>(),
-                       S.task_off.as<uint32_t>(), G, (unsigned)seg, lshift, nbins, len_cnt, (const uint32_t *)nullptr, (uint32_t *)nullptr,
-                       (uint4 *)nullptr);
-    PM_HIP(ctx, hipGetLastError());
-    hipLaunchKernelGGL(k_scan_small, dim3(1), dim3(1024), 0, ctx->stream, len_cnt, len_off, len_cursor, nbins);
-    PM_HIP(ctx, hipGetLastError());
-    hipLaunchKernelGGL(k_task_bins<true>, dim3(blocks), dim3(1024), nbins * 4, ctx->stream, counts, S.bucket_off.as<uint32_t>(),
-                       S.task_off.as<uint32_t>(), G, (unsigned)seg, lshift, nbins, (uint32_t *)nullptr, len_off, len_cursor,
-                       S.tasks.as<uint4>());
+    hipLaunchKernelGGL(k_task_bins, dim3(blocks), dim3(1024), tb.nbins * 4, ctx->stream, S.counts.as<uint32_t>(), S.bucket_off.as<uint32_t>(),
+                       S.task_off.as<uint32_t>(), G, (unsigned)p.seg, tb.lshift, tb.nbins, len_off, len_cursor, S.tasks.as<uint4>(),
+                       S.task_cnt.as<uint32_t>(), hot_a, hot_b, ctl + CTL_HOT, (uint32_t)cap);
     PM_HIP(ctx, hipGetLastError());
     return PM_OK;
 }
 
 template <class C, bool TABLE>
 static int accumulate(pm_ctx *ctx, MsmSet &S, const BucketPlan &p, const void *points) {
-    int per_cu = 0, cus = 0;
-    PM_HIP(ctx, hipOccupancyMaxActiveBlocksPerMultiprocessor(&per_cu, (const void *)k_accumulate<C, TABLE>, 128, 0));
-    PM_HIP(ctx, hipDeviceGetAttribute(&cus, hipDeviceAttributeMultiprocessorCount, ctx->device));
-    size_t blocks = (size_t)(per_cu > 0 ? per_cu : 1) * (size_t)(cus > 0 ? cus : 1);
+    unsigned &resident = ctx->msm.resident_blocks[C::ID][TABLE ? 1 : 0];
+    if (!resident) {
+        int per_cu = 0, cus = 0;
+        PM_HIP(ctx, hipOccupancyMaxActiveBlocksPerMultiprocessor(&per_cu, (const void *)k_accumulate<C, TABLE>, 128, 0));
+        PM_HIP(ctx, hipDeviceGetAttribute(&cus, hipDeviceAttributeMultiprocessorCount, ctx->device));
+        resident = (unsigned)(per_cu > 0 ? per_cu : 1) * (unsigned)(cus > 0 ? cus : 1);
+    }
+    size_t blocks = resident;
     if (blocks > (p.max_tasks + 127) / 128) blocks = (p.max_tasks + 127) / 128;
     hipLaunchKernelGGL((k_accumulate<C, TABLE>), dim3((unsigned)blocks), dim3(128), 0, ctx->stream, S.sorted.as<uint32_t>(),
-                       S.task_off.as<uint32_t>(), S.tasks.as<uint4>(), points, S.partials.as<XYZZ<C>>(), p.NB, ctx->msm.len_bins.as<uint32_t>());
+                       S.task_off.as<uint32_t>(), S.tasks.as<uint4>(), points, S.partials.as<XYZZ<C>>(), p.NB, set_ctl(S, p) + CTL_TICKET);
     PM_HIP(ctx, hipGetLastError());
     return PM_OK;
 }
@@ -1045,13 +1077,14 @@
     PM_HIP(ctx, ws.digits.reserve(p.E * 4));
     uint32_t *counts = S.counts.as<uint32_t>(), *cursor = counts + p.NB, *digits = ws.digits.as<uint32_t>();
     const unsigned nbuckets = (unsigned)p.NB1;
-    PM_HIP(ctx, hipMemsetAsync(counts, 0, 2 * p.NB * 4, ctx->stream));
+    PM_TRY(clear_counters(ctx, S, p));
     hipLaunchKernelGGL(k_digits<C>, dim3((unsigned)((p.len + 255) / 256)), dim3(256), 0, ctx->stream, d_scalars, d_bases, digits, p.len, p.c, p.nwin);
     PM_HIP(ctx, hipGetLastError());
     const size_t lds = (size_t)nbuckets * 4;
-    if (lds > 48 * 1024) {
+    if (lds > 48 * 1024 && lds > ws.hist_lds) {
         PM_HIP(ctx, hipFuncSetAttribute((const void *)k_hist, hipFuncAttributeMaxDynamicSharedMemorySize, (int)lds));
         PM_HIP(ctx, hipFuncSetAttribute((const void *)k_scatter, hipFuncAttributeMaxDynamicSharedMemorySize, (int)lds));
+        ws.hist_lds = lds;
     }
     hipLaunchKernelGGL(k_hist, dim3(p.nchunks, p.nwin), dim3(1024), lds, ctx->stream, digits, counts, p.len, p.chunk, nbuckets);
     PM_HIP(ctx, hipGetLastError());
@@ -1064,7 +1097,7 @@
 
 struct SortBuffers {
     uint16_t *keys;
-    uint32_t *vals, *region_count, *region_off, *region_cursor;
+    uint32_t *vals, *region_off;
 };
 
 template <class P, unsigned NWIN = 10>
@@ -1079,33 +1112,33 @@
     const BlockScanShape bsh = block_scan_shape(pblocks, p.regions);
     PM_HIP(ctx, ctx->msm.block_cnt.reserve(((size_t)pblocks + bsh.G) * p.regions * 4));
     uint32_t *block_cnt = ctx->msm.block_cnt.as<uint32_t>(), *block_partial = block_cnt + (size_t)pblocks * p.regions;
-    PM_HIP(ctx, hipMemsetAsync(b.region_count, 0, (size_t)p.regions * 4, st));
     hipLaunchKernelGGL((k_tbl_count<P, NWIN>), dim3(pblocks), dim3(p.pbd), 0, st, d_scalars, inf, p.len, p.regions, block_cnt, p.win_buckets,
                        p.narrow_buckets);
     hipLaunchKernelGGL(k_block_sums, dim3(bsh.G), dim3(1024), 0, st, block_cnt, pblocks, p.regions, bsh, block_partial);
-    hipLaunchKernelGGL(k_block_offsets, dim3(bsh.G), dim3(1024), 0, st, block_cnt, pblocks, p.regions, bsh, block_partial, b.region_count);
-    hipLaunchKernelGGL(k_region_offsets, dim3(1), dim3(1024), 0, st, b.region_count, b.region_off, b.region_cursor, p.regions);
-    PM_HIP(ctx, hipFuncSetAttribute((const void *)k_tbl_partition<P, NWIN>, hipFuncAttributeMaxDynamicSharedMemorySize, (int)p.plds));
+    hipLaunchKernelGGL(k_block_offsets, dim3(bsh.G), dim3(1024), 0, st, block_cnt, pblocks, p.regions, bsh, block_partial, b.region_off);
+    size_t &plds_set = ctx->msm.partition_lds[std::is_same<P, BlsFrP>::value ? 0 : 1][NWIN];
+    if (p.plds > plds_set) {
+        PM_HIP(ctx, hipFuncSetAttribute((const void *)k_tbl_partition<P, NWIN>, hipFuncAttributeMaxDynamicSharedMemorySize, (int)p.plds));
+        plds_set = p.plds;
+    }
     hipLaunchKernelGGL((k_tbl_partition<P, NWIN>), dim3(pblocks), dim3(p.pbd), p.plds, st, d_scalars, inf, p.len, p.regions, b.region_off, block_cnt,
                        p.wide ? (size_t)0 : tb.stride, tb.base_index, b.keys, b.vals, p.win_buckets, p.narrow_buckets);
     PM_HIP(ctx, hipGetLastError());
     return PM_OK;
 }
 
-constexpr unsigned SUB_BINS = 128, FIN_BINS = 256, FIN_BITS = 8;
 
 static int sort_three_levels(pm_ctx *ctx, MsmSet &S, const BucketPlan &p, const SortBuffers &b) {
     MsmWorkspace &ws = ctx->msm;
     hipStream_t st = ctx->stream;
     const unsigned nsub = p.regions * SUB_BINS, chunk = 1u << RS_CHUNK_LOG;
-    PM_HIP(ctx, ws.sub.reserve((3 * (size_t)nsub + 4) * 4));
+    PM_HIP(ctx, ws.sub.reserve((2 * (size_t)nsub + 4) * 4));
     PM_HIP(ctx, ws.digits2.reserve(p.keys_bytes + p.E * 4 + 128));
     uint32_t *counts = S.counts.as<uint32_t>(), *cursor = counts + p.NB;
-    uint32_t *sub_count = ws.sub.as<uint32_t>(), *sub_off = sub_count + nsub, *sub_cursor = sub_off + nsub + 1;
+    uint32_t *sub_count = set_ctl(S, p) + CTL_SUB_COUNT, *sub_off = ws.sub.as<uint32_t>(), *sub_cursor = sub_off + nsub + 1;
     uint16_t *keys2 = (uint16_t *)ws.digits2.p;
     uint32_t *vals2 = (uint32_t *)((uint8_t *)ws.digits2.p + p.keys_bytes);
     const unsigned sblocks = (unsigned)((p.E + chunk - 1) / chunk), stblocks = (unsigned)((p.E + ST_CHUNK - 1) / ST_CHUNK);
-    PM_HIP(ctx, hipMemsetAsync(sub_count, 0, (size_t)nsub * 4, st));
     hipLaunchKernelGGL(k_hist_small, dim3(sblocks), dim3(1024), 0, st, b.keys, b.region_off, p.regions, FIN_BITS, SUB_BINS, chunk, sub_count);
     PM_HIP(ctx, hipGetLastError());
     hipLaunchKernelGGL(k_scan_small, dim3(1), dim3(1024), 0, st, sub_count, sub_off, sub_cursor, nsub);
@@ -1143,14 +1176,12 @@
 static int sort_tables(pm_ctx *ctx, MsmSet &S, const BucketPlan &p, const MsmTables &tb, const Fp<typename C::FrP> *d_scalars) {
     MsmWorkspace &ws = ctx->msm;
     PM_HIP(ctx, ws.digits.reserve(p.keys_bytes + p.E * 4 + 128));
-    PM_HIP(ctx, ws.region.reserve((3 * (size_t)p.regions + 4) * 4));
+    PM_HIP(ctx, ws.region.reserve(((size_t)p.regions + 1) * 4));
     SortBuffers b;
     b.keys = (uint16_t *)ws.digits.p;
     b.vals = (uint32_t *)((uint8_t *)ws.digits.p + p.keys_bytes);
-    b.region_count = ws.region.as<uint32_t>();
-    b.region_off = b.region_count + p.regions;
-    b.region_cursor = b.region_off + p.regions + 1;
-    PM_HIP(ctx, hipMemsetAsync(S.counts.as<uint32_t>(), 0, 2 * p.NB * 4, ctx->stream));
+    b.region_off = ws.region.as<uint32_t>();
+    PM_TRY(clear_counters(ctx, S, p));
     PM_TRY((sort_first_level<typename C::FrP>(ctx, p, tb, d_scalars, b)));
     return p.lo_buckets == (1u << LO_BITS) ? sort_three_levels(ctx, S, p, b) : sort_one_region(ctx, S, p, b);
 }
diff --git a/polymath_amd/csrc/ntt.hip b/polymath_amd/csrc/ntt.hip
--- a/polymath_amd/csrc/ntt.hip
+++ b/polymath_amd/csrc/ntt.hip
@@ -408,13 +408,18 @@
 }
 
 template <class C>
-int ntt_run(pm_ctx *ctx, Fp<typename C::FrP> *d, unsigned log_n, bool inv_dir) {
+int ntt_run(pm_ctx *ctx, Fp<typename C::FrP> *d, unsigned log_n, bool inv_dir, const Fp<typename C::FrP> *src) {
     typedef typename C::FrP P;
     typedef Fp<P> Fr;
     if (log_n > (unsigned)C::TWO_ADICITY) return PM_ERR_DOMAIN_TOO_LARGE;
+    const size_t n = (size_t)1 << log_n;
+    if (src == d) src = nullptr;
+    if (src && !(log_n && ntt_l28_domain(log_n))) {
+        PM_HIP(ctx, hipMemcpyAsync(d, src, n * sizeof(Fr), hipMemcpyDeviceToDevice, ctx->stream));
+        src = nullptr;
+    }
     if (log_n == 0) return PM_OK;
     StageTimer timer(ctx, T_NTT);
-    const size_t n = (size_t)1 << log_n;
     TwiddleCache *slot = nullptr;
     PM_TRY(twiddles_slot<C>(ctx, log_n, &slot));
     const DevBuf &twb = inv_dir ? slot->inv_int : slot->fwd_int;
@@ -452,9 +457,9 @@
                 const dim3 grid((unsigned)(n >> (ns + log_cols)));
                 const size_t lds = ((size_t)1 << (ns + log_cols)) * RR::N * 4;
                 if (small)
-                    hipLaunchKernelGGL((k_ntt_first_pass28<P, RR, 256>), grid, dim3(256), lds, ctx->stream, (const Fr *)d, tmp, tw28, log_n, ns, log_cols, pair_stages);
+                    hipLaunchKernelGGL((k_ntt_first_pass28<P, RR, 256>), grid, dim3(256), lds, ctx->stream, src ? src : (const Fr *)d, tmp, tw28, log_n, ns, log_cols, pair_stages);
                 else
-                    hipLaunchKernelGGL((k_ntt_first_pass28<P, RR, 512>), grid, dim3(512), lds, ctx->stream, (const Fr *)d, tmp, tw28, log_n, ns, log_cols, pair_stages);
+                    hipLaunchKernelGGL((k_ntt_first_pass28<P, RR, 512>), grid, dim3(512), lds, ctx->stream, src ? src : (const Fr *)d, tmp, tw28, log_n, ns, log_cols, pair_stages);
             } else {
                 if (s0 < log_cols) log_cols = s0;
                 const dim3 grid((unsigned)(n >> (ns + log_cols)));
@@ -494,7 +499,7 @@
 
 template int twiddles_get<BlsCurve>(pm_ctx *, unsigned, bool, const Fp<BlsFrP> **);
 template int twiddles_get<BnCurve>(pm_ctx *, unsigned, bool, const Fp<BnFrP> **);
-template int ntt_run<BlsCurve>(pm_ctx *, Fp<BlsFrP> *, unsigned, bool);
-template int ntt_run<BnCurve>(pm_ctx *, Fp<BnFrP> *, unsigned, bool);
-
-}
+template int ntt_run<BlsCurve>(pm_ctx *, Fp<BlsFrP> *, unsigned, bool, const Fp<BlsFrP> *);
+template int ntt_run<BnCurve>(pm_ctx *, Fp<BnFrP> *, unsigned, bool, const Fp<BnFrP> *);
+
+}
diff --git a/polymath_amd/csrc/prove.hip b/polymath_amd/csrc/prove.hip
--- a/polymath_amd/csrc/prove.hip
+++ b/polymath_amd/csrc/prove.hip
@@ -457,9 +457,7 @@
         hipLaunchKernelGGL(k_check_sap<P>, dim3(nblk(n)), dim3(256), 0, st, ue, we, n, flags);
         PM_HIP(ctx, hipGetLastError());
     }
-    PM_HIP(ctx, hipMemcpyAsync(u, ue, n * sizeof(Fr), hipMemcpyDeviceToDevice, st));
-    PM_HIP(ctx, hipMemcpyAsync(wv, we, n * sizeof(Fr), hipMemcpyDeviceToDevice, st));
-    PM_TRY(ntt_run<C>(ctx, u, pk->log_n, true));
+    PM_TRY(ntt_run<C>(ctx, u, pk->log_n, true, ue));
     const bool overlap = ctx->opt.v[PM_OPT_MSM_OVERLAP] != 0;
     pm_ctx *const aux_ctx = overlap ? ctx_aux(ctx) : nullptr;
     int st_a = PM_OK;
@@ -494,7 +492,7 @@
             if (!helper.pending) a_early = false;
         }
     }
-    PM_TRY(ntt_run<C>(ctx, wv, pk->log_n, true));
+    PM_TRY(ntt_run<C>(ctx, wv, pk->log_n, true, we));
     if (2 * m0 <= 16 && pk->log_n >= 1) {
         const Fr *winv = nullptr;
         PM_TRY(twiddles_get<C>(ctx, pk->log_n, true, &winv));
```
